# kimkyeonghun/MSA

Measured on AMD Instinct MI355X. Metric: train-step samples/sec, higher is better.
Workload: dtype bf16; 1 GPU; MMBertForPretraining train step, 3 passes S=50/550/550, 12-layer d=768 heads=12 vocab=30522, T=50 A=500 V=500, dropout on, AdamW; per_gpu_batch=16, global_batch=16, parallelism=dp1, scores_dtype=bf16, mlm_backward=labelled rows only (exact: unlabelled rows have zero CE gradient), deterministic=True

## Files before the change

### include/mmbert_hip.h

```cpp
#ifndef MMBERT_HIP_H
#define MMBERT_HIP_H
#include <stddef.h>
#include <stdint.h>

#ifdef __cplusplus
extern "C" {
#endif

typedef struct ihipStream_t* mmbert_stream_t;

#define MMBERT_EPI_BIAS 1
#define MMBERT_EPI_GELU 2
#define MMBERT_EPI_RESID 4
#define MMBERT_EPI_GELU_BWD 8
#define MMBERT_EPI_OUT_F32 16

int mmbert_gemm_nt(mmbert_stream_t stream, const void* A, int lda, const void* B, int ldb, void* C, int ldc,
                   int M, int N, int K, int epi, const float* bias, const void* R, int ldr, void* aux, int ldaux,
                   const void* U, int ldu, float alpha, const float* alpha_dev,
                   uint32_t drop_stream, uint32_t drop_thr16, float drop_scale, int* tile_queue);

int mmbert_gemm_nt_splitk(mmbert_stream_t stream, const void* A, int lda, const void* B, int ldb, void* C, int ldc,
                          int M, int N, int K, void* workspace, const void* R, int ldr);
size_t mmbert_gemm_nt_splitk_workspace(int M, int N, int K);

void mmbert_gemm_nt_force(int mode);
int mmbert_gemm_nt_describe(int M, int N, int K, int epi, int with_queue, int* out);
void mmbert_gemm_tn_force_splits(int splits);
void mmbert_gemm_tn_force_one_launch(int on);

size_t mmbert_gemm_tn_workspace(int M, int N, int K, int* splits_out);
int mmbert_gemm_tn(mmbert_stream_t stream, const void* A, int lda, const void* B, int ldb, float* W, int ldw,
                   int M, int N, int K, int accumulate, float alpha, const float* alpha_dev, void* slab, float* bias_out);
size_t mmbert_gemm_tn_grouped_workspace(int nprob, const int* N, const int* K, int M, int* splits_out);
int mmbert_gemm_tn_grouped(mmbert_stream_t stream, int nprob, const void* const* A, const int* lda, const void* const* B, const int* ldb,
                           float* const* W, float* const* bias, const int* N, const int* K, int M,
                           int accumulate, float alpha, const float* alpha_dev, void* slab);
int mmbert_gemm_tn_grouped_rows(mmbert_stream_t stream, int nprob, const void* const* A, const int* lda, const void* const* B, const int* ldb,
                                float* const* W, float* const* bias, const int* N, const int* K, const int* M,
                                int accumulate, const int* accumulate_each, float alpha, const float* alpha_dev, void* slab);

int mmbert_colsum(mmbert_stream_t stream, const void* X, int ldx, int M, int N, float* out, float alpha, const float* alpha_dev);

uint32_t mmbert_rng_stream(uint64_t seed, uint32_t site);
uint32_t mmbert_dropout_thr16(float p);
int mmbert_dropout_mask(mmbert_stream_t stream, uint8_t* out, size_t n, uint32_t rng_stream, uint32_t thr16);

int mmbert_mlm_mask(mmbert_stream_t stream, int64_t* ids, int64_t* labels, size_t n, uint32_t rng_stream, uint32_t select_thr16,
                    uint32_t replace_thr16, int64_t special0, int64_t special1, int64_t special2, int64_t mask_id);

int mmbert_ln_fwd(mmbert_stream_t stream, const void* x, int ldx, const int* in_rows, void* y, int ldy, const int* out_rows,
                  int M, int H, const float* gamma, const float* beta, float eps, float* mean, float* rstd,
                  uint32_t dstream, uint32_t dthr, float dscale, int drop_row0);
int mmbert_ln_bwd(mmbert_stream_t stream, const void* dy, int lddy, const int* dy_rows, const void* x, int ldx, const int* x_rows,
                  const float* mean, const float* rstd, const float* gamma, int M, int H,
                  void* dx, int lddx, const int* dx_rows, void* dx2, int lddx2, float* dgamma, float* dbeta, float* dbias2,
                  uint32_t post_stream, uint32_t post_thr, float post_scale,
                  uint32_t pre_stream, uint32_t pre_thr, float pre_scale,
                  float* partial_ws , const int* drop_rows,
                  int defer_reduce ,
                  int dy_row_limit );
size_t mmbert_ln_bwd_workspace(int M, int H);
int mmbert_ln_bwd_reduce(mmbert_stream_t stream, int items, const float* const* partial_ws, float* const* dgamma, float* const* dbeta,
                         float* const* dbias2, int M, int H);
int mmbert_ln_bwd_reduce_rows(mmbert_stream_t stream, int items, const float* const* partial_ws, float* const* dgamma, float* const* dbeta,
                              float* const* dbias2, const int* M, int H);

int mmbert_embed_gather(mmbert_stream_t stream, const int64_t* ids, const int64_t* tts, const float* word, const float* type,
                        const float* pos, int n, int T, int H, int V, void* out, int ldo);
int mmbert_embed_scatter(mmbert_stream_t stream, const int64_t* ids, const int64_t* tts, const void* d, int ldd, int n, int T, int H, int V,
                         float* gword, float* gtype, float* gpos, float* type_slab);

int mmbert_pair_proj_fwd(mmbert_stream_t stream, const void* feat, int feat_f64, int B, int P, int D, const float* W, const float* bias, int H,
                         void* out, int ldo, int T);
int mmbert_pair_proj_bwd(mmbert_stream_t stream, const void* feat, int feat_f64, int B, int P, int D, const void* J, const void* dJ, int ld, int T,
                         float* dW, float* db, int H, void* workspace );
size_t mmbert_pair_proj_bwd_workspace(int B, int P, int D, int H);

int mmbert_attn_tile_rows(int which);
int mmbert_attn_kv_len(mmbert_stream_t stream, const float* key_bias, const int* bias_start, const int* seq_len, int nseq, int* kv_len);
int mmbert_attn_fwd(mmbert_stream_t stream, const void* qkv, void* ctx, float* lse, const float* key_bias, const int* bias_start, int H, int heads,
                    const int* seq_start, const int* seq_len, const unsigned* elem_base, const int* tile_seq, const int* tile_r0, int ntiles,
                    uint32_t dstream, uint32_t dthr, float dscale, const int* kv_len, const int* tile_qshift, const int* tile_qend);
int mmbert_attn_fwd_first(mmbert_stream_t stream, const void* qkv, void* ctx, const float* key_bias, const int* bias_start, int H, int heads,
                          const int* seq_start, const int* seq_len, const int* q_row, int nseq, const int* kv_len);
int mmbert_attn_probs_first(mmbert_stream_t stream, const void* qkv, float* probs, int ld, const float* key_bias, const int* bias_start, int H, int heads,
                            const int* seq_start, const int* seq_len, const int* q_row, int nseq, const int* kv_len );
int mmbert_attn_bwd(mmbert_stream_t stream, const void* qkv, const void* ctx, const void* dctx, void* dqkv, const float* lse, float* delta,
                    const float* key_bias, const int* bias_start, int H, int heads, const int* seq_start, const int* seq_len, const unsigned* elem_base,
                    const int* qtile_seq, const int* qtile_r0, int nqtiles,
                    const int* tile_seq, const int* tile_r0, int ntiles,
                    uint32_t dstream, uint32_t dthr, float dscale, const int* kv_len,
                    const int* qtile_qshift, const int* qtile_qend, int split,
                    const int* q_limit);
int mmbert_attn_q_limit(mmbert_stream_t stream, const int* rows, int n, const int* seq_start, int nseq, int* q_limit);
int mmbert_attn_dropout_mask(mmbert_stream_t stream, uint8_t* out, int S, unsigned elem_base, int head, uint32_t rng_stream, uint32_t thr16);

int mmbert_ce_fwd(mmbert_stream_t stream, const void* logits, int ldv, int V, const int64_t* labels, int M,
                  const int* seg_bounds, int nseg, float* inv_count, float* loss_sum, float* row_lse,
                  int logits_f32 ,
                  float* row_loss );
int mmbert_ce_bwd(mmbert_stream_t stream, const void* logits, int ldv, int V, const int64_t* labels, int M,
                  const int* seg_bounds, int nseg, const float* inv_count, const float* gscale, const float* row_lse, void* dlogits, int ldd,
                  const int* rows , int nrows,
                  int logits_f32 );
int mmbert_vocab_topk(mmbert_stream_t stream, const void* logits, int ldv, int V, int M, int logits_f32, int k,
                      const int64_t* labels ,
                      int32_t* top_ids , float* top_logprob , float* row_lse ,
                      float* label_logprob , int32_t* label_rank );
int mmbert_split_rows(mmbert_stream_t stream, const int64_t* row_seq, const int64_t* row_pos, const int* start_a, const int* start_b,
                      const int* valid, int mode, int M, int rows_a, int64_t* perm, int64_t* inv, const int* rank,
                      int* perm32 , int* inv32);

int mmbert_split_layout(mmbert_stream_t stream, const int* seq_len, const int* valid, int nseq, int tile_rows, int xs, int nf_max, int nq_max,
                        int* out);

int mmbert_prologue(mmbert_stream_t stream, int nseg, const void* const* seg_ptr, const long long* seg_stride_b, const long long* seg_stride_p,
                    const int* seg_dtype, const int* seg_pass, const int* seg_offset, const int* seg_len,
                    int npass, const int* pass_len, int B, const int64_t* labels, int vocab,
                    float* key_bias, int* kv_len, int* valid, int* seq_cnt, int* idx, int* words, int* rank, float* key_bias_perm);

int mmbert_rows_to_block(mmbert_stream_t stream, const int64_t* ids, const void* rows, int rows_bf16, int ldr, int n, int H,
                         const int64_t* uni, int U, int V, float* block);

int mmbert_pack_i64(mmbert_stream_t stream, int nseg, const int64_t* const* src, const long long* dst_offset, const long long* count,
                    const long long* fill, int64_t* out);

int mmbert_active_rows(mmbert_stream_t stream, const int64_t* labels, int M, int V, int* idx, int* count);

int mmbert_heads_gate_fwd(mmbert_stream_t stream, const float* P, const float* Apre, const float* const* vw3, const float* const* vb3, int B, int H, float* g, float* C);
int mmbert_heads_loss_fwd(mmbert_stream_t stream, const float* P, const float* XP, const float* rel, const int64_t* ap, const float* lo, const float* sent,
                          int B, int H, float beta, int tanh_lo, float* out5, float* dXP, float* dPc, float* drel, float* dlo, float* nce_part,
                          const float* mlm, int nmlm, float alpha, float* loss_out , float* aux_out );
int mmbert_heads_scale(mmbert_stream_t stream, float* x, size_t n, const float* s);
int mmbert_heads_seed(mmbert_stream_t stream, const float* src, size_t n, const float* s, float* dst, float* zero, size_t nzero, float* dmlm, int nmlm, float coef);
int mmbert_heads_gate_bwd(mmbert_stream_t stream, const float* dC, const float* P, const float* Apre, const float* g, const float* const* vw3, const float* dPc,
                          int B, int H, float* dP, float* dApre, float* E, float* dg);
int mmbert_heads_tanh(mmbert_stream_t stream, float* x, size_t n);
int mmbert_heads_tanh_bwd(mmbert_stream_t stream, const float* dP, const float* P, float* dpre, size_t n);
int mmbert_heads_colsum(mmbert_stream_t stream, int nseg, const float* const* src, float* const* dst, const int* rows, const int* cols, const int* ld);

typedef struct {
    int B, H, tanh_lo, nmlm;
    float alpha, beta;
    const float* first; const void* y; const int64_t* first_rows; int ldy, ncls;
    const int64_t* ap; const int64_t* ap2; const float* sent; const float* mlm;
    const float *Wp, *bp, *Wal, *bal, *Wsr, *bsr, *Wat, *bat, *vw[3], *vb[3], *Wc1, *bc1, *Wc2, *bc2, *Wq[3], *bq[3];
    float *loss, *aux, *out5, *logits, *t_rel, *rel;
    float* ws;
    const float* dloss; float* dfirst; float* dmlm;
    float *gWp, *gbp, *gWal, *gbal, *gWat, *gbat, *gvw[3], *gvb[3], *gWc1, *gbc1, *gWc2, *gbc2, *gWq[3], *gbq[3];
    unsigned* sync;
    const int64_t* sent_cls; int64_t* pred;
} mmbert_heads_step;
int mmbert_heads_step_struct_size(void);
size_t mmbert_heads_step_workspace(int B, int H);
int mmbert_heads_step_fwd(mmbert_stream_t stream, const mmbert_heads_step* p);
int mmbert_heads_step_bwd(mmbert_stream_t stream, const mmbert_heads_step* p);
int mmbert_heads_step_fwd_levels(mmbert_stream_t stream, const mmbert_heads_step* p, int lo, int hi);
int mmbert_heads_step_bwd_levels(mmbert_stream_t stream, const mmbert_heads_step* p, int lo, int hi);
int mmbert_heads_predict(mmbert_stream_t stream, const mmbert_heads_step* p);
int mmbert_heads_step_outputs(int B, int H, size_t* pooled_offset, size_t* fused_offset);
int mmbert_heads_step_dmlm(mmbert_stream_t stream, const mmbert_heads_step* p);

typedef struct { const float* X; const float* W; int ldx, ldw, inner, row0, rows, w_inner_major; } mmbert_skinny_src;
typedef struct { float* Y; const float* bias; int ldy, M, N, nsrc, act, accumulate; mmbert_skinny_src src[4]; } mmbert_skinny_op;
typedef struct { const float* dY; const float* X; float* dW; float* db; int ldy, ldx, ldw, M, N, K; } mmbert_skinny_wgrad_op;
int mmbert_skinny_mm(mmbert_stream_t stream, int nops, const mmbert_skinny_op* ops);
size_t mmbert_skinny_mm_workspace(int nops, const mmbert_skinny_op* ops);
int mmbert_skinny_mm_ordered(mmbert_stream_t stream, int nops, const mmbert_skinny_op* ops, void* workspace);
int mmbert_skinny_wgrad(mmbert_stream_t stream, int nops, const mmbert_skinny_wgrad_op* ops);

typedef struct { uint32_t stream, thr16; float scale; } mmbert_drop;
typedef struct {
    const float* key_bias; const int* bias_start; const int* seq_start; const int* seq_len; const unsigned* elem_base;
    const int* ftile_seq; const int* ftile_r0; const int* ftile_qshift; const int* ftile_qend;
    const int* qtile_seq; const int* qtile_r0; const int* qtile_qshift; const int* qtile_qend;
    const int* tile_seq; const int* tile_r0;
    const int* kv_len;
    int nftiles, nqtiles, ntiles, split, heads, pad_;
} mmbert_attn_layout;
typedef struct {
    const void* x;
    const void* Wqkv; const void* Wo; const void* W1; const void* W2;
    const float* bqkv; const float* bo; const float* b1; const float* b2; const float* ln1_g; const float* ln1_b; const float* ln2_g; const float* ln2_b;
    void* qkv; void* actx; float* lse; void* z1; void* y1; float* m1; float* r1; void* u ; void* g; void* z2; void* y2; float* m2; float* r2;
    const int* y2_rows;
    int* tile_queue;
    mmbert_drop att, h1, h2;
    int rows, H, I, ldx, ldy2; float ln_eps;
} mmbert_layer_fwd_args;
typedef struct {
    const void* dy; const int* dy_rows;
    const void* z2; const float* m2; const float* r2; const float* ln2_g; float* g_ln2_g; float* g_ln2_b; float* ln2_ws;
    const void* z1; const float* m1; const float* r1; const float* ln1_g; float* g_ln1_g; float* g_ln1_b; float* ln1_ws;
    const void* u; const void* qkv; const void* actx; const float* lse;
    const void* W2T; const void* W1T; const void* WoT; const void* WqkvT;
    void* dz2; void* dz2d ; void* du; void* dy1; void* dz1; void* dz1d ; void* dctx; void* dqkv; float* delta; void* dx;
    int* tile_queue;
    mmbert_drop att, h1, h2;
    int rows, H, I, lddy;
} mmbert_layer_bwd_args;
int mmbert_layer_fwd(mmbert_stream_t stream, const mmbert_attn_layout* layout, const mmbert_layer_fwd_args* a);
int mmbert_layer_bwd(mmbert_stream_t stream, const mmbert_attn_layout* layout, const mmbert_layer_bwd_args* a);
int mmbert_layer_struct_sizes(int* out );

void mmbert_set_deterministic(int on);
int mmbert_get_deterministic(void);
int mmbert_id_runs_sum_rows(mmbert_stream_t stream, const void* src, int src_bf16, int lds, const int64_t* ids, int n,
                            int H, int V, const int64_t* uni, int U, float* dst, int ldd);

int mmbert_adamw(mmbert_stream_t stream, float* p, float* g, float* m, float* v, void* p_bf16, const uint8_t* flags, size_t n,
                 double lr, double beta1, double beta2, double eps, double wd, int step, double gscale, int mode, int zero_grad);

int mmbert_adamw_devscale(mmbert_stream_t stream, float* p, float* g, float* m, float* v, void* p_bf16, const uint8_t* flags, size_t n,
                          double lr, double beta1, double beta2, double eps, double wd, int step, const float* coef, int mode, int zero_grad);

#define MMBERT_ADAMW_MAX_GROUPS 255
#define MMBERT_ADAMW_MAX_SLOTS 64
int mmbert_adamw_grouped(mmbert_stream_t stream, float* p, float* g, float* m, float* v, void* p_bf16, const uint8_t* flags,
                         const uint8_t* group_of_block, size_t n, const double* hyper, int ngroups, int step, double gscale,
                         const float* coef, int mode, int zero_grad);

#define MMBERT_GRAD_NORM_WORKSPACE 8192
int mmbert_grad_norm(mmbert_stream_t stream, const float* g, size_t n, const int64_t* segs, int nseg, double norm_type, double max_norm,
                     double gscale, void* workspace, float* out);
int mmbert_grad_scale(mmbert_stream_t stream, float* g, size_t n, const int64_t* segs, int nseg, const float* coef);

int mmbert_gelu_bwd(mmbert_stream_t stream, const void* dy, const void* u, void* du, size_t n);

int mmbert_cast_f32_bf16(mmbert_stream_t stream, const float* x, void* y, size_t n);
int mmbert_cast_bf16_f32(mmbert_stream_t stream, const void* x, float* y, size_t n);
int mmbert_transpose_cast(mmbert_stream_t stream, const float* src, void* dst, const void* descs, int ndesc, int total_tiles);
int mmbert_compact_rows(mmbert_stream_t stream, const int* rows32, const int64_t* rows64, int n, const int64_t* extra, int nextra, const int64_t* map,
                        int64_t* out64, int* out32);
int mmbert_compact_rows_inv(mmbert_stream_t stream, const int* rows32, const int64_t* rows64, int n, const int64_t* extra, int nextra, const int64_t* map,
                            int64_t* out64, int* out32, int64_t* inv_stamp, unsigned stamp);
int mmbert_scatter_rows_zero(mmbert_stream_t stream, int nseg, const void* const* src, void* const* dst, const long long* src_pitch,
                             const long long* dst_pitch, const int* row_bytes, const int64_t* inv_stamp, unsigned stamp, int nlist, int nrows);
int mmbert_gather_rows(mmbert_stream_t stream, int nseg, const void* const* src, void* const* dst, const long long* src_pitch, const long long* dst_pitch,
                       const int* row_bytes, const int* idx, int nrows);
int mmbert_transpose_bf16(mmbert_stream_t stream, const void* src, void* dst, const void* descs, int ndesc, int total_tiles);

#ifdef __cplusplus
}
#endif
#endif
```

### msa_amd/_lib.py

```python
from __future__ import annotations

import ctypes as C
import os

HERE = os.path.dirname(os.path.abspath(__file__))
LIB_PATH = os.environ.get("MMBERT_LIB_PATH") or os.path.join(HERE, "libmmbert_hip.so")

P, I, F, D, U32, SZ, U64 = C.c_void_p, C.c_int, C.c_float, C.c_double, C.c_uint32, C.c_size_t, C.c_uint64

SIGNATURES = {
    "mmbert_gemm_nt": (I, [P, P, I, P, I, P, I, I, I, I, I, P, P, I, P, I, P, I, F, P, U32, U32, F, P]),
    "mmbert_gemm_nt_force": (None, [I]),
    "mmbert_gemm_nt_describe": (I, [I, I, I, I, I, P]),
    "mmbert_gemm_nt_splitk": (I, [P, P, I, P, I, P, I, I, I, I, P, P, I]),
    "mmbert_gemm_nt_splitk_workspace": (SZ, [I, I, I]),
    "mmbert_gemm_tn_force_splits": (None, [I]),
    "mmbert_gemm_tn_force_one_launch": (None, [I]),
    "mmbert_gemm_tn_workspace": (SZ, [I, I, I, P]),
    "mmbert_gemm_tn": (I, [P, P, I, P, I, P, I, I, I, I, I, F, P, P, P]),
    "mmbert_gemm_tn_grouped_workspace": (SZ, [I, P, P, I, P]),
    "mmbert_gemm_tn_grouped": (I, [P, I, P, P, P, P, P, P, P, P, I, I, F, P, P]),
    "mmbert_gemm_tn_grouped_rows": (I, [P, I, P, P, P, P, P, P, P, P, P, I, P, F, P, P]),
    "mmbert_colsum": (I, [P, P, I, I, I, P, F, P]),
    "mmbert_rng_stream": (U32, [U64, U32]),
    "mmbert_dropout_thr16": (U32, [F]),
    "mmbert_dropout_mask": (I, [P, P, SZ, U32, U32]),
    "mmbert_mlm_mask": (I, [P, P, P, SZ, U32, U32, U32, C.c_int64, C.c_int64, C.c_int64, C.c_int64]),
    "mmbert_ln_fwd": (I, [P, P, I, P, P, I, P, I, I, P, P, F, P, P, U32, U32, F, I]),
    "mmbert_ln_bwd": (I, [P, P, I, P, P, I, P, P, P, P, I, I, P, I, P, P, I, P, P, P, U32, U32, F, U32, U32, F, P, P, I, I]),
    "mmbert_ln_bwd_reduce": (I, [P, I, P, P, P, P, I, I]),
    "mmbert_ln_bwd_reduce_rows": (I, [P, I, P, P, P, P, P, I]),
    "mmbert_ln_bwd_workspace": (SZ, [I, I]),
    "mmbert_embed_gather": (I, [P, P, P, P, P, P, I, I, I, I, P, I]),
    "mmbert_embed_scatter": (I, [P, P, P, P, I, I, I, I, I, P, P, P, P]),
    "mmbert_pair_proj_fwd": (I, [P, P, I, I, I, I, P, P, I, P, I, I]),
    "mmbert_pair_proj_bwd": (I, [P, P, I, I, I, I, P, P, I, I, P, P, I, P]),
    "mmbert_pair_proj_bwd_workspace": (SZ, [I, I, I, I]),
    "mmbert_attn_tile_rows": (I, [I]),
    "mmbert_attn_kv_len": (I, [P, P, P, P, I, P]),
    "mmbert_attn_fwd": (I, [P, P, P, P, P, P, I, I, P, P, P, P, P, I, U32, U32, F, P, P, P]),
    "mmbert_attn_fwd_first": (I, [P, P, P, P, P, I, I, P, P, P, I, P]),
    "mmbert_attn_probs_first": (I, [P, P, P, I, P, P, I, I, P, P, P, I, P]),
    "mmbert_attn_bwd": (I, [P, P, P, P, P, P, P, P, P, I, I, P, P, P, P, P, I, P, P, I, U32, U32, F, P, P, P, I, P]),
    "mmbert_attn_q_limit": (I, [P, P, I, P, I, P]),
    "mmbert_attn_dropout_mask": (I, [P, P, I, C.c_uint, I, U32, U32]),
    "mmbert_ce_fwd": (I, [P, P, I, I, P, I, P, I, P, P, P, I, P]),
    "mmbert_ce_bwd": (I, [P, P, I, I, P, I, P, I, P, P, P, P, I, P, I, I]),
    "mmbert_vocab_topk": (I, [P, P, I, I, I, I, I, P, P, P, P, P, P]),
    "mmbert_active_rows": (I, [P, P, I, I, P, P]),
    "mmbert_prologue": (I, [P, I, P, P, P, P, P, P, P, I, P, I, P, I, P, P, P, P, P, P, P, P]),
    "mmbert_split_rows": (I, [P, P, P, P, P, P, I, I, I, P, P, P, P, P]),
    "mmbert_heads_gate_fwd": (I, [P, P, P, P, P, I, I, P, P]),
    "mmbert_heads_loss_fwd": (I, [P, P, P, P, P, P, P, I, I, F, I, P, P, P, P, P, P, P, I, F, P, P]),
    "mmbert_heads_scale": (I, [P, P, SZ, P]),
    "mmbert_heads_seed": (I, [P, P, SZ, P, P, P, SZ, P, I, F]),
    "mmbert_heads_gate_bwd": (I, [P, P, P, P, P, P, P, I, I, P, P, P, P]),
    "mmbert_heads_tanh": (I, [P, P, SZ]),
    "mmbert_heads_tanh_bwd": (I, [P, P, P, P, SZ]),
    "mmbert_heads_colsum": (I, [P, I, P, P, P, P, P]),
    "mmbert_skinny_mm": (I, [P, I, P]),
    "mmbert_skinny_mm_workspace": (SZ, [I, P]),
    "mmbert_skinny_mm_ordered": (I, [P, I, P, P]),
    "mmbert_heads_step_struct_size": (I, []),
    "mmbert_heads_step_workspace": (SZ, [I, I]),
    "mmbert_heads_step_fwd": (I, [P, P]),
    "mmbert_heads_step_bwd": (I, [P, P]),
    "mmbert_heads_step_fwd_levels": (I, [P, P, I, I]),
    "mmbert_heads_step_bwd_levels": (I, [P, P, I, I]),
    "mmbert_heads_step_dmlm": (I, [P, P]),
    "mmbert_heads_predict": (I, [P, P]),
    "mmbert_heads_step_outputs": (I, [I, I, P, P]),
    "mmbert_layer_fwd": (I, [P, P, P]),
    "mmbert_layer_bwd": (I, [P, P, P]),
    "mmbert_layer_struct_sizes": (I, [P]),
    "mmbert_set_deterministic": (None, [I]),
    "mmbert_get_deterministic": (I, []),
    "mmbert_id_runs_sum_rows": (I, [P, P, I, I, P, I, I, I, P, I, P, I]),
    "mmbert_skinny_wgrad": (I, [P, I, P]),
    "mmbert_adamw": (I, [P, P, P, P, P, P, P, SZ, D, D, D, D, D, I, D, I, I]),
    "mmbert_adamw_devscale": (I, [P, P, P, P, P, P, P, SZ, D, D, D, D, D, I, P, I, I]),
    "mmbert_adamw_grouped": (I, [P, P, P, P, P, P, P, P, SZ, P, I, I, D, P, I, I]),
    "mmbert_grad_norm": (I, [P, P, SZ, P, I, D, D, D, P, P]),
    "mmbert_grad_scale": (I, [P, P, SZ, P, I, P]),
    "mmbert_gelu_bwd": (I, [P, P, P, P, SZ]),
    "mmbert_cast_f32_bf16": (I, [P, P, P, SZ]),
    "mmbert_cast_bf16_f32": (I, [P, P, P, SZ]),
    "mmbert_transpose_cast": (I, [P, P, P, P, I, I]),
    "mmbert_transpose_bf16": (I, [P, P, P, P, I, I]),
    "mmbert_gather_rows": (I, [P, I, P, P, P, P, P, P, I]),
    "mmbert_compact_rows": (I, [P, P, P, I, P, I, P, P, P]),
    "mmbert_compact_rows_inv": (I, [P, P, P, I, P, I, P, P, P, P, C.c_uint]),
    "mmbert_scatter_rows_zero": (I, [P, I, P, P, P, P, P, P, C.c_uint, I, I]),
    "mmbert_pack_i64": (I, [P, I, P, P, P, P, P]),
    "mmbert_rows_to_block": (I, [P, P, P, I, I, I, I, P, I, I, P]),
    "mmbert_split_layout": (I, [P, P, P, I, I, I, I, I, P]),
}

_lib = None


def load() -> C.CDLL:
    global _lib
    if _lib is not None:
        return _lib
    if not os.path.exists(LIB_PATH):
        raise RuntimeError(
            f"{LIB_PATH} not found: the MI355X kernels are not built and there is no CPU fallback. "
            "Run `python -m msa_amd.build` (needs hipcc) first.")
    lib = C.CDLL(LIB_PATH)
    for name, (res, args) in SIGNATURES.items():
        fn = getattr(lib, name)
        fn.restype = res
        fn.argtypes = args
    _lib = lib
    return lib


def check(code: int, what: str) -> None:
    if code != 0:
        raise RuntimeError(f"{what} failed with code {code} "
                           f"({'invalid argument' if code < 0 else 'hipError_t'})")
```

### msa_amd/csrc/attention.hip

```cpp
#include <cstdlib>
#include "common.h"
#include <type_traits>

#define LOG2E 1.4426950408889634f
#define LN2 0.6931471805599453f

struct AttnArgs {
    const bf16_t* qkv; int ld_qkv;
    bf16_t* ctx;
    const bf16_t* dctx;
    bf16_t* dqkv;
    float* lse;
    float* delta;
    const float* key_bias;
    const int* bias_start;
    const int* kv_len;
    const int* seq_start; const int* seq_len; const unsigned* elem_base;
    const int* tile_seq; const int* tile_r0;
    const int* tile_qshift; const int* tile_qend; int split;
    const int* q_limit;
    int H, heads;
    float scale;
    uint32_t dstream, dthr; float dscale;
    int head_fast;
// ... 799 lines not shown

    for (int k0 = grp; k0 < Skv; k0 += 256) {
        bf16x8 kf[8];
        float b[8];
#pragma unroll
        for (int u = 0; u < 8; ++u) {
            const int k = min(k0 + 32 * u, Skv - 1);
            kf[u] = *(const bf16x8*)(kbase + (size_t)k * a.ld_qkv);
            b[u] = bbase[k];
        }
        float s[8];
#pragma unroll
        for (int u = 0; u < 8; ++u) {
            float d = 0.f;
#pragma unroll
            for (int j = 0; j < 8; ++j) d = __builtin_fmaf(q[j], bf2f(kf[u][j]), d);
            d += __shfl_xor(d, 1, 64); d += __shfl_xor(d, 2, 64); d += __shfl_xor(d, 4, 64);
            const int k = k0 + 32 * u;
            s[u] = k < Skv ? d + b[u] : -INFINITY;
            if (c == 0 && k < Skv && k < a.ld) sc[k] = s[u];
        }
        const float mnew = fmaxf(fmaxf(fmaxf(fmaxf(s[0], s[1]), fmaxf(s[2], s[3])), fmaxf(fmaxf(s[4], s[5]), fmaxf(s[6], s[7]))), st.m);
        st.l *= __builtin_amdgcn_exp2f((st.m - mnew) * LOG2E);
        st.m = mnew;
#pragma unroll
        for (int u = 0; u < 8; ++u) st.l += __builtin_amdgcn_exp2f((s[u] - mnew) * LOG2E);
    }
#pragma unroll
    for (int off = 8; off < 64; off <<= 1) {
        ApState o2;
        o2.m = __shfl_xor(st.m, off, 64); o2.l = __shfl_xor(st.l, off, 64);
        ap_merge(st, o2);
    }
    if (lane == 0) { part[2 * wave] = st.m; part[2 * wave + 1] = st.l; }
    __syncthreads();
    ApState tot;
    tot.m = part[0]; tot.l = part[1];
#pragma unroll
    for (int w = 1; w < 4; ++w) {
        ApState o2;
        o2.m = part[2 * w]; o2.l = part[2 * w + 1];
        ap_merge(tot, o2);
    }
    const float inv = 1.0f / tot.l;
    const int nk = min(Skv, a.ld);
    for (int k = threadIdx.x; k < a.ld; k += 256)
        prow[k] = k < nk ? __builtin_amdgcn_exp2f((sc[k] - tot.m) * LOG2E) * inv : 0.f;
}

__global__ void attn_mask_kernel(uint8_t* out, int S, unsigned elem_base, int head, uint32_t stream, uint32_t thr) {
    const int Spad = (S + 3) & ~3;
    for (int e = blockIdx.x * blockDim.x + threadIdx.x; e < S * S; e += gridDim.x * blockDim.x) {
        const int i = e / S, j = e % S;
        out[e] = mmb_keep(stream, (uint64_t)elem_base + (uint64_t)(head * S + i) * Spad + j, thr) ? 1 : 0;
    }
}

__global__ void attn_kv_len_kernel(const float* __restrict__ key_bias, const int* __restrict__ bias_start, const int* __restrict__ seq_len, int nseq, int* __restrict__ out) {
    const int s = blockIdx.x;
    if (s >= nseq) return;
    const int S = seq_len[s];
    const float* b = key_bias + bias_start[s];
    int last = -1;
    for (int k = threadIdx.x; k < S; k += 64)
        if (b[k] > -10000.0f) last = k;
#pragma unroll
    for (int o = 32; o > 0; o >>= 1) last = max(last, __shfl_xor(last, o, 64));
    if (threadIdx.x == 0) out[s] = last < 0 ? S : last + 1;
}

__global__ void attn_q_limit_kernel(const int* __restrict__ rows, int n, const int* __restrict__ seq_start, int nseq, int* __restrict__ out) {
    const int i = blockIdx.x * blockDim.x + threadIdx.x;
    if (i >= n) return;
    const int r = rows[i];
    int lo = 0, hi = nseq - 1;
    while (lo < hi) {
        const int mid = (lo + hi + 1) >> 1;
        if (seq_start[mid] <= r) lo = mid; else hi = mid - 1;
    }
    atomicMax(out + lo, r - seq_start[lo] + 1);
}
__global__ __launch_bounds__(256) void attn_q_limit_wg_kernel(const int* __restrict__ rows, int n, const int* __restrict__ seq_start, int nseq,
                                                              int* __restrict__ out) {
    __shared__ int lim[1024], st[1024];
    for (int s = threadIdx.x; s < nseq; s += 256) { lim[s] = 0; st[s] = seq_start[s]; }
    __syncthreads();
    for (int i = threadIdx.x; i < n; i += 256) {
        const int r = rows[i];
        int lo = 0, hi = nseq - 1;
        while (lo < hi) {
            const int mid = (lo + hi + 1) >> 1;
            if (st[mid] <= r) lo = mid; else hi = mid - 1;
        }
        atomicMax(&lim[lo], r - st[lo] + 1);
    }
    __syncthreads();
    for (int s = threadIdx.x; s < nseq; s += 256) out[s] = lim[s];
}

extern "C" {

static int fill_args(AttnArgs& a, const void* qkv, int H, int heads, const float* key_bias, const int* bias_start, const int* seq_start, const int* seq_len,
                     const unsigned* elem_base, const int* tile_seq, const int* tile_r0, float* lse,
                     uint32_t dstream, uint32_t dthr, float dscale, const int* kv_len) {
    if (heads <= 0 || H != heads * 64) return -1;
    a.qkv = (const bf16_t*)qkv; a.ld_qkv = 3 * H; a.H = H; a.heads = heads; a.key_bias = key_bias; a.bias_start = bias_start;
    a.seq_start = seq_start; a.seq_len = seq_len; a.elem_base = elem_base; a.tile_seq = tile_seq; a.tile_r0 = tile_r0;
    a.lse = lse; a.scale = 0.125f; a.dstream = dstream; a.dthr = dthr; a.dscale = dscale;
    a.ctx = nullptr; a.dctx = nullptr; a.dqkv = nullptr; a.delta = nullptr; a.kv_len = kv_len;
    a.tile_qshift = nullptr; a.tile_qend = nullptr; a.split = 0; a.q_limit = nullptr;
    a.head_fast = 1;
    return 0;
}

int mmbert_attn_fwd(hipStream_t stream, const void* qkv, void* ctx, float* lse, const float* key_bias, const int* bias_start, int H, int heads,
                    const int* seq_start, const int* seq_len, const unsigned* elem_base, const int* tile_seq, const int* tile_r0, int ntiles,
                    uint32_t dstream, uint32_t dthr, float dscale, const int* kv_len, const int* tile_qshift, const int* tile_qend) {
    if (ntiles <= 0) return 0;
    if ((tile_qshift == nullptr) != (tile_qend == nullptr)) return -1;
    AttnArgs a;
    if (fill_args(a, qkv, H, heads, key_bias, bias_start, seq_start, seq_len, elem_base, tile_seq, tile_r0, lse, dstream, dthr, dscale, kv_len)) return -1;
    a.ctx = (bf16_t*)ctx; a.tile_qshift = tile_qshift; a.tile_qend = tile_qend;
    if (ntiles > 65535) a.head_fast = 0;
    constexpr int extra_lds = 0;
    if (dthr) hipLaunchKernelGGL(attn_fwd_kernel<true>, a.head_fast ? dim3(heads, ntiles) : dim3(ntiles, heads), dim3(256), extra_lds, stream, a);
    else hipLaunchKernelGGL(attn_fwd_kernel<false>, a.head_fast ? dim3(heads, ntiles) : dim3(ntiles, heads), dim3(256), extra_lds, stream, a);
    MMB_CHECK_LAUNCH();
    return 0;
}

int mmbert_attn_fwd_first(hipStream_t stream, const void* qkv, void* ctx, const float* key_bias, const int* bias_start, int H, int heads,
                          const int* seq_start, const int* seq_len, const int* q_row, int nseq, const int* kv_len) {
    if (nseq <= 0) return 0;
    if (heads <= 0 || H != heads * 64 || nseq > 65535 || !qkv || !ctx || !key_bias || !bias_start || !seq_start || !seq_len || !q_row) return -1;
    AttnFirstArgs a;
    a.qkv = (const bf16_t*)qkv; a.ld_qkv = 3 * H; a.ctx = (bf16_t*)ctx; a.key_bias = key_bias; a.bias_start = bias_start; a.kv_len = kv_len;
    a.seq_start = seq_start; a.seq_len = seq_len; a.q_row = q_row; a.H = H; a.scale = 0.125f;
    hipLaunchKernelGGL(attn_fwd_first_kernel, dim3(heads, nseq), dim3(256), 0, stream, a);
    MMB_CHECK_LAUNCH();
    return 0;
}

int mmbert_attn_probs_first(hipStream_t stream, const void* qkv, float* probs, int ld, const float* key_bias, const int* bias_start, int H, int heads,
                            const int* seq_start, const int* seq_len, const int* q_row, int nseq, const int* kv_len) {
    if (nseq <= 0) return 0;
    if (heads <= 0 || H != heads * 64 || nseq > 65535 || ld < 1 || !qkv || !probs || !key_bias || !bias_start || !seq_start || !seq_len || !q_row) return -1;
    if (APF_LDS_BYTES(ld) > APF_LDS_MAX) return -1;
    AttnProbsArgs a;
    a.qkv = (const bf16_t*)qkv; a.ld_qkv = 3 * H; a.probs = probs; a.ld = ld; a.key_bias = key_bias; a.bias_start = bias_start; a.kv_len = kv_len;
    a.seq_start = seq_start; a.seq_len = seq_len; a.q_row = q_row; a.H = H; a.heads = heads; a.scale = 0.125f;
    hipLaunchKernelGGL(attn_probs_first_kernel, dim3(heads, nseq), dim3(256), APF_LDS_BYTES(ld), stream, a);
    MMB_CHECK_LAUNCH();
    return 0;
}

int mmbert_attn_bwd(hipStream_t stream, const void* qkv, const void* ctx, const void* dctx, void* dqkv, const float* lse, float* delta,
                    const float* key_bias, const int* bias_start, int H, int heads, const int* seq_start, const int* seq_len, const unsigned* elem_base,
                    const int* qtile_seq, const int* qtile_r0, int nqtiles, const int* tile_seq, const int* tile_r0, int ntiles,
                    uint32_t dstream, uint32_t dthr, float dscale, const int* kv_len, const int* qtile_qshift, const int* qtile_qend, int split,
                    const int* q_limit) {
    if (ntiles <= 0 || nqtiles <= 0) return 0;
    if ((qtile_qshift == nullptr) != (qtile_qend == nullptr) || (split && !kv_len)) return -1;
    AttnArgs a;
    if (fill_args(a, qkv, H, heads, key_bias, bias_start, seq_start, seq_len, elem_base, tile_seq, tile_r0, (float*)lse, dstream, dthr, dscale, kv_len)) return -1;
    a.ctx = (bf16_t*)ctx; a.dctx = (const bf16_t*)dctx; a.dqkv = (bf16_t*)dqkv; a.delta = delta; a.q_limit = q_limit;
    {
        AttnArgs q = a;
        q.tile_seq = qtile_seq; q.tile_r0 = qtile_r0; q.tile_qshift = qtile_qshift; q.tile_qend = qtile_qend;
        if (nqtiles > 65535) q.head_fast = 0;
        if (dthr) hipLaunchKernelGGL(attn_bwd_dq_kernel<true>, q.head_fast ? dim3(heads, nqtiles) : dim3(nqtiles, heads), dim3(256), 0, stream, q);
        else hipLaunchKernelGGL(attn_bwd_dq_kernel<false>, q.head_fast ? dim3(heads, nqtiles) : dim3(nqtiles, heads), dim3(256), 0, stream, q);
        MMB_CHECK_LAUNCH();
    }
    a.split = split;
    if (ntiles > 65535) a.head_fast = 0;
    if (dthr) hipLaunchKernelGGL(attn_bwd_dkv_kernel<true>, a.head_fast ? dim3(heads, ntiles) : dim3(ntiles, heads), dim3(256), 0, stream, a);
    else hipLaunchKernelGGL(attn_bwd_dkv_kernel<false>, a.head_fast ? dim3(heads, ntiles) : dim3(ntiles, heads), dim3(256), 0, stream, a);
    MMB_CHECK_LAUNCH();
    return 0;
}
// ... 38 lines not shown
```

### msa_amd/csrc/common.h

```cpp
#pragma once
#include <hip/hip_runtime.h>
#include <stdint.h>

#if defined(MMB_EXP_NOMFMA) || defined(MMB_EXP_ALOADS) || defined(MMB_EXP_NOBLOADS) || defined(MMB_EXP_EXEC0) || defined(MMB_EXP_WAVEA) || \
    defined(MMB_EXP_NOFRAGS) || defined(MMB_AB_FREE_HASH)
#error "MMB_EXP_* / MMB_AB_* ablation switches are not part of the product sources (see git tag r3-gemm-ablations)"
#endif

typedef __bf16 bf16_t;
typedef __attribute__((ext_vector_type(8))) __bf16 bf16x8;
typedef __attribute__((ext_vector_type(4))) __bf16 bf16x4;
typedef __attribute__((ext_vector_type(2))) __bf16 bf16x2;
typedef __attribute__((ext_vector_type(4))) short s16x4;
typedef __attribute__((ext_vector_type(4))) float f32x4;
typedef __attribute__((ext_vector_type(16))) float f32x16;

#define MMB_CHECK_LAUNCH() do { hipError_t e_ = hipGetLastError(); if (e_ != hipSuccess) return (int)e_; } while (0)

#include <atomic>
static inline int mmb_allow_lds(const void* fn, int bytes, std::atomic<unsigned long long>& done) {
    int dev = 0;
    if (hipGetDevice(&dev) != hipSuccess) return (int)hipErrorInvalidDevice;
    const unsigned long long bit = 1ull << (dev & 63);
    if (done.load(std::memory_order_acquire) & bit) return 0;
// ... 77 lines not shown

__device__ __forceinline__ float mmb_clamp_abs12(float x) { return __builtin_amdgcn_fmed3f(fabsf(x), 0.0f, 12.0f); }
__device__ __forceinline__ float mmb_relu(float x) { float r; asm("v_max_f32 %0, 0, %1" : "=v"(r) : "v"(x)); return r; }
__device__ __forceinline__ float gelu_erf(float x) {
    const float a = mmb_clamp_abs12(x);
    float q = 0.000488118665642307f;
    q = fmaf(q, a, -0.007198809871008205f);
    q = fmaf(q, a, 0.05214680078704519f);
    q = fmaf(q, a, 0.4595957249475095f);
    q = fmaf(q, a, 1.1510005681479196f);
    const float t = __builtin_amdgcn_exp2f(fmaf(-a, q, -1.0f));
    return fmaf(-a, t, mmb_relu(x));
}
__device__ __forceinline__ float gelu_erf_grad(float x) {
    const float a = mmb_clamp_abs12(x);
    float w = -0.00016849001371319273f;
    w = fmaf(w, a, 0.002318365387269111f);
    w = fmaf(w, a, -0.013920757956130972f);
    w = fmaf(w, a, 0.04993439894451681f);
    w = fmaf(w, a, -0.1258212077485634f);
    w = fmaf(w, a, 0.2479567789223165f);
    w = fmaf(w, a, -0.7976617799265314f);
    w = fmaf(w, a, 0.49999600551278855f);
    const float g = __builtin_amdgcn_exp2f(-0.72134752044448170f * a * a) * w;
    return x > 0.0f ? 1.0f - g : g;
}

__device__ __forceinline__ mmb_f2 gelu_erf2(mmb_f2 x) {
    const mmb_f2 a = {mmb_clamp_abs12(x.x), mmb_clamp_abs12(x.y)};
    mmb_f2 q = (mmb_f2){0.000488118665642307f, 0.000488118665642307f};
    q = q * a + (mmb_f2){-0.007198809871008205f, -0.007198809871008205f};
    q = q * a + (mmb_f2){0.05214680078704519f, 0.05214680078704519f};
    q = q * a + (mmb_f2){0.4595957249475095f, 0.4595957249475095f};
    q = q * a + (mmb_f2){1.1510005681479196f, 1.1510005681479196f};
    const mmb_f2 e = -a * q + (mmb_f2){-1.0f, -1.0f};
    const mmb_f2 t = {__builtin_amdgcn_exp2f(e.x), __builtin_amdgcn_exp2f(e.y)};
    const mmb_f2 r = {mmb_relu(x.x), mmb_relu(x.y)};
    return -a * t + r;
}
__device__ __forceinline__ mmb_f2 gelu_erf_grad2(mmb_f2 x) {
    const mmb_f2 a = {mmb_clamp_abs12(x.x), mmb_clamp_abs12(x.y)};
    mmb_f2 w = (mmb_f2){-0.00016849001371319273f, -0.00016849001371319273f};
    w = w * a + (mmb_f2){0.002318365387269111f, 0.002318365387269111f};
    w = w * a + (mmb_f2){-0.013920757956130972f, -0.013920757956130972f};
    w = w * a + (mmb_f2){0.04993439894451681f, 0.04993439894451681f};
    w = w * a + (mmb_f2){-0.1258212077485634f, -0.1258212077485634f};
    w = w * a + (mmb_f2){0.2479567789223165f, 0.2479567789223165f};
    w = w * a + (mmb_f2){-0.7976617799265314f, -0.7976617799265314f};
    w = w * a + (mmb_f2){0.49999600551278855f, 0.49999600551278855f};
    const mmb_f2 e = ((mmb_f2){-0.72134752044448170f, -0.72134752044448170f} * a) * a;
    const mmb_f2 g = (mmb_f2){__builtin_amdgcn_exp2f(e.x), __builtin_amdgcn_exp2f(e.y)} * w;
    const mmb_f2 og = (mmb_f2){1.0f, 1.0f} - g;
    return (mmb_f2){x.x > 0.0f ? og.x : g.x, x.y > 0.0f ? og.y : g.y};
}

__device__ __forceinline__ void gelu_erf4(mmb_f2& x0, mmb_f2& x1) {
    const mmb_f2 a0 = {mmb_clamp_abs12(x0.x), mmb_clamp_abs12(x0.y)}, a1 = {mmb_clamp_abs12(x1.x), mmb_clamp_abs12(x1.y)};
    mmb_f2 q0 = (mmb_f2){0.000488118665642307f, 0.000488118665642307f}, q1 = q0;
    q0 = q0 * a0 + (mmb_f2){-0.007198809871008205f, -0.007198809871008205f}; q1 = q1 * a1 + (mmb_f2){-0.007198809871008205f, -0.007198809871008205f};
    q0 = q0 * a0 + (mmb_f2){0.05214680078704519f, 0.05214680078704519f};    q1 = q1 * a1 + (mmb_f2){0.05214680078704519f, 0.05214680078704519f};
    q0 = q0 * a0 + (mmb_f2){0.4595957249475095f, 0.4595957249475095f};      q1 = q1 * a1 + (mmb_f2){0.4595957249475095f, 0.4595957249475095f};
    q0 = q0 * a0 + (mmb_f2){1.1510005681479196f, 1.1510005681479196f};      q1 = q1 * a1 + (mmb_f2){1.1510005681479196f, 1.1510005681479196f};
    const mmb_f2 e0 = -a0 * q0 + (mmb_f2){-1.0f, -1.0f}, e1 = -a1 * q1 + (mmb_f2){-1.0f, -1.0f};
    const mmb_f2 r0 = {mmb_relu(x0.x), mmb_relu(x0.y)}, r1 = {mmb_relu(x1.x), mmb_relu(x1.y)};
    const mmb_f2 t0 = {__builtin_amdgcn_exp2f(e0.x), __builtin_amdgcn_exp2f(e0.y)}, t1 = {__builtin_amdgcn_exp2f(e1.x), __builtin_amdgcn_exp2f(e1.y)};
    x0 = -a0 * t0 + r0;
    x1 = -a1 * t1 + r1;
}
__device__ __forceinline__ void gelu_erf_grad4(mmb_f2 x0, mmb_f2 x1, mmb_f2& d0, mmb_f2& d1) {
    const mmb_f2 a0 = {mmb_clamp_abs12(x0.x), mmb_clamp_abs12(x0.y)}, a1 = {mmb_clamp_abs12(x1.x), mmb_clamp_abs12(x1.y)};
    mmb_f2 w0 = (mmb_f2){-0.00016849001371319273f, -0.00016849001371319273f}, w1 = w0;
#define MMB_W_STEP(C) w0 = w0 * a0 + (mmb_f2){C, C}; w1 = w1 * a1 + (mmb_f2){C, C};
    MMB_W_STEP(0.002318365387269111f) MMB_W_STEP(-0.013920757956130972f) MMB_W_STEP(0.04993439894451681f) MMB_W_STEP(-0.1258212077485634f)
    MMB_W_STEP(0.2479567789223165f) MMB_W_STEP(-0.7976617799265314f) MMB_W_STEP(0.49999600551278855f)
#undef MMB_W_STEP
    const mmb_f2 k = {-0.72134752044448170f, -0.72134752044448170f};
    const mmb_f2 e0 = (k * a0) * a0, e1 = (k * a1) * a1;
    const mmb_f2 t0 = {__builtin_amdgcn_exp2f(e0.x), __builtin_amdgcn_exp2f(e0.y)}, t1 = {__builtin_amdgcn_exp2f(e1.x), __builtin_amdgcn_exp2f(e1.y)};
    const mmb_f2 g0 = t0 * w0, g1 = t1 * w1;
    const mmb_f2 o0 = (mmb_f2){1.0f, 1.0f} - g0, o1 = (mmb_f2){1.0f, 1.0f} - g1;
    d0 = (mmb_f2){x0.x > 0.0f ? o0.x : g0.x, x0.y > 0.0f ? o0.y : g0.y};
    d1 = (mmb_f2){x1.x > 0.0f ? o1.x : g1.x, x1.y > 0.0f ? o1.y : g1.y};
}
```

### msa_amd/csrc/rowwise.hip

```cpp
#include "common.h"
#include <cstring>

std::atomic<int> g_mmb_deterministic{0};

__global__ void split_rows_kernel(const int64_t* __restrict__ row_seq, const int64_t* __restrict__ row_pos, const int* __restrict__ start_a,
                                  const int* __restrict__ start_b, const int* __restrict__ valid, int mode, int M, int rows_a,
                                  int64_t* __restrict__ perm, int64_t* __restrict__ inv, const int* __restrict__ rank,
                                  int* __restrict__ perm32, int* __restrict__ inv32) {
    const int i = blockIdx.x * blockDim.x + threadIdx.x;
    if (i >= M) return;
    const int s = (int)row_seq[i], p = rank ? rank[i] : (int)row_pos[i], v = valid[s];
    int n = rows_a;
    bool own = false;
    if (p < v) { n = start_a[s] + p; own = true; }
    else if (mode == 0) { n = start_b[s] + p - v; own = true; }
    else if (mode == 1) { n = start_b[s]; own = p == v; }
    inv[i] = n;
    if (inv32) inv32[i] = n;
    if (own) { perm[n] = i; if (perm32) perm32[n] = i; }
}

#define SL_MAXSEQ 1024
__global__ __launch_bounds__(1024) void split_layout_kernel(const int* __restrict__ lens, const int* __restrict__ valid, int nseq, int rows, int xs,
                                                            int nf_max, int nq_max, int* __restrict__ out) {
// ... 811 lines not shown
            for (int i = 0; i < 4; ++i) av[i] = bf2f(st[u].j[i]) > 0.f ? bf2f(st[u].d[i]) : 0.f;
            float fv[PAIR_NT];
#pragma unroll
            for (int j = 0; j < PAIR_NT; ++j) fv[j] = st[u].f[j];
            load(st[u], r + 16 + 4 * u + g);
#pragma unroll
            for (int j = 0; j < PAIR_NT; ++j) {
                if (j >= njt) continue;
#pragma unroll
                for (int i = 0; i < 4; ++i) acc[j][i] = __builtin_amdgcn_mfma_f32_16x16x4f32(av[i], fv[j], acc[j][i], 0, 0, 0);
            }
        }
    }
    if (wave) {
#pragma unroll
        for (int j = 0; j < PAIR_NT; ++j)
#pragma unroll
            for (int i = 0; i < 4; ++i)
#pragma unroll
                for (int q = 0; q < 4; ++q) red[wave - 1][(j * 4 + i) * 4 + q][lane] = acc[j][i][q];
    }
    __syncthreads();
    if (wave == 0) {
        const int W1 = a.D + 1;
        float* out = a.slab + (size_t)s * a.H * W1;
#pragma unroll
        for (int j = 0; j < PAIR_NT; ++j) {
            const int k = (jt0 + j) * 16 + c;
#pragma unroll
            for (int i = 0; i < 4; ++i)
#pragma unroll
                for (int q = 0; q < 4; ++q) {
                    const int e = (j * 4 + i) * 4 + q;
                    const float v = ((acc[j][i][q] + red[0][e][lane]) + red[1][e][lane]) + red[2][e][lane];
                    const int h = hb + 4 * (4 * g + q) + i;
                    if (j < njt && k < W1 && h < a.H) out[(size_t)h * W1 + k] = v;
                }
        }
    }
#endif
}

__global__ void pair_wgrad_reduce_kernel(const float* __restrict__ slab, int S, int H, int D, float* __restrict__ dW, float* __restrict__ db) {
    const int i = blockIdx.x * blockDim.x + threadIdx.x;
    const int W1 = D + 1;
    if (i >= H * W1) return;
    float t = 0.f;
    int s_ = 0;
    for (; s_ + 8 <= S; s_ += 8) {
        float v[8];
#pragma unroll
        for (int u = 0; u < 8; ++u) v[u] = slab[(size_t)(s_ + u) * H * W1 + i];
#pragma unroll
        for (int u = 0; u < 8; ++u) t += v[u];
    }
    for (; s_ < S; ++s_) t += slab[(size_t)s_ * H * W1 + i];
    const int h = i / W1, k = i - h * W1;
    if (k < D) dW[(size_t)h * D + k] += t; else db[h] += t;
}

__global__ __launch_bounds__(1024) void active_rows_kernel(const int64_t* __restrict__ labels, int M, int V, int* __restrict__ idx, int* __restrict__ count) {
    __shared__ int wsum[16];
    __shared__ int base;
    const int tid = threadIdx.x, lane = tid & 63, w = tid >> 6;
    if (tid == 0) base = 0;
    __syncthreads();
    for (int i0 = 0; i0 < M; i0 += 1024) {
        const int i = i0 + tid;
        const bool act = i < M && labels[i] >= 0 && labels[i] < V;
        const unsigned long long bal = __ballot(act);
        const int before = __popcll(bal & ((1ull << lane) - 1ull));
        if (lane == 0) wsum[w] = __popcll(bal);
        __syncthreads();
        int off = base;
        for (int q = 0; q < w; ++q) off += wsum[q];
        if (act) idx[off + before] = i;
        __syncthreads();
        if (tid == 0) { int t = 0; for (int q = 0; q < 16; ++q) t += wsum[q]; base += t; }
        __syncthreads();
    }
    if (tid == 0) *count = base;
}

__global__ void ce_count_kernel(const int64_t* __restrict__ labels, int M, int V, const int* __restrict__ seg_bounds, int nseg,
                                float* __restrict__ inv_count, float* __restrict__ loss_sum) {
    __shared__ int cnt[4];
    if (threadIdx.x < 4) cnt[threadIdx.x] = 0;
    __syncthreads();
    const int b1 = nseg > 1 ? seg_bounds[1] : 0x7fffffff, b2 = nseg > 2 ? seg_bounds[2] : 0x7fffffff, b3 = nseg > 3 ? seg_bounds[3] : 0x7fffffff;
    int c[4] = {0, 0, 0, 0};
    for (int i0 = threadIdx.x; i0 < M; i0 += (int)blockDim.x * 8) {
        int64_t lab[8];
#pragma unroll
        for (int u = 0; u < 8; ++u) lab[u] = labels[min(i0 + u * (int)blockDim.x, M - 1)];
#pragma unroll
        for (int u = 0; u < 8; ++u) {
            const int i = i0 + u * (int)blockDim.x;
            const int ok = (i < M && lab[u] >= 0 && lab[u] < V) ? 1 : 0;
            const int sg = (i >= b1 ? 1 : 0) + (i >= b2 ? 1 : 0) + (i >= b3 ? 1 : 0);
#pragma unroll
            for (int q = 0; q < 4; ++q) c[q] += (sg == q) ? ok : 0;
        }
    }
#pragma unroll
    for (int q = 0; q < 4; ++q) if (c[q]) atomicAdd(&cnt[q], c[q]);
    __syncthreads();
    if (threadIdx.x < nseg) {
        inv_count[threadIdx.x] = 1.0f / (float)max(cnt[threadIdx.x], 1);
        loss_sum[threadIdx.x] = 0.f;
    }
}

__global__ __launch_bounds__(1024) void ce_loss_sum_ordered_kernel(const float* __restrict__ row_loss, int M, const int* __restrict__ seg_bounds, int nseg,
                                                                   float* __restrict__ loss_sum) {
    __shared__ float red[4][1024];
    const int b1 = nseg > 1 ? seg_bounds[1] : 0x7fffffff, b2 = nseg > 2 ? seg_bounds[2] : 0x7fffffff, b3 = nseg > 3 ? seg_bounds[3] : 0x7fffffff;
    float c[4] = {0.f, 0.f, 0.f, 0.f};
    for (int i0 = threadIdx.x; i0 < M; i0 += 1024 * 8) {
        float v[8];
#pragma unroll
        for (int u = 0; u < 8; ++u) v[u] = row_loss[min(i0 + u * 1024, M - 1)];
#pragma unroll
        for (int u = 0; u < 8; ++u) {
            const int i = i0 + u * 1024;
            const int sg = (i >= b1 ? 1 : 0) + (i >= b2 ? 1 : 0) + (i >= b3 ? 1 : 0);
            const float x = i < M ? v[u] : 0.f;
#pragma unroll
            for (int q = 0; q < 4; ++q) c[q] += (sg == q) ? x : 0.f;
        }
    }
#pragma unroll
    for (int q = 0; q < 4; ++q) red[q][threadIdx.x] = c[q];
    __syncthreads();
    for (int w = 512; w > 0; w >>= 1) {
        if ((int)threadIdx.x < w) {
#pragma unroll
            for (int q = 0; q < 4; ++q) red[q][threadIdx.x] += red[q][threadIdx.x + w];
        }
        __syncthreads();
    }
    if ((int)threadIdx.x < nseg) loss_sum[threadIdx.x] = red[threadIdx.x][0];
}

#define RUNS_MAXN 8192
__global__ __launch_bounds__(1024) void id_runs_sum_rows_kernel(const void* __restrict__ src, int src_bf16, int lds, const int64_t* __restrict__ ids,
                                                                int n, int H, int V, const int64_t* __restrict__ uni, int U,
                                                                float* __restrict__ dst, int ldd) {
    __shared__ int list[RUNS_MAXN];
    __shared__ float red[1024 * 4];
    __shared__ int s_count, s_earlier;
    const int i0 = blockIdx.x, tid = threadIdx.x, nthr = blockDim.x;
    const long long key = ids[i0];
    if (key <= 0 || key >= V) return;
    if (tid == 0) { s_count = 0; s_earlier = 0; }
    __syncthreads();
    int earlier = 0;
    for (int j = tid; j < i0; j += nthr) earlier |= (ids[j] == key) ? 1 : 0;
    if (earlier) s_earlier = 1;
    __syncthreads();
    if (s_earlier) return;
    long long dr = key;
    if (uni) {
        int lo = 0, hi = U - 1;
        while (lo < hi) { const int mid = (lo + hi) >> 1; if (uni[mid] < key) lo = mid + 1; else hi = mid; }
        if (U <= 0 || uni[lo] != key) return;
        dr = lo;
    }
    if (tid < 64) {
        int count = 0;
        for (int base = i0; base < n; base += 64) {
            const int j = base + tid;
            const bool hit = j < n && ids[j] == key;
            const unsigned long long m = __ballot(hit);
            if (hit) list[count + __popcll(m & ((1ull << tid) - 1ull))] = j;
            count += __popcll(m);
        }
        if (tid == 0) s_count = count;
    }
    __syncthreads();
    const int cnt = s_count;
    const int CT = H >> 2, G = nthr / CT;
    const int g = tid / CT, c = tid - g * CT;
    float a[4] = {0.f, 0.f, 0.f, 0.f};
    if (g < G) {
#pragma unroll 4
        for (int k = g; k < cnt; k += G) {
            const size_t r = (size_t)list[k];
            if (src_bf16) {
                const bf16x4 x = *(const bf16x4*)((const bf16_t*)src + r * lds + 4 * c);
#pragma unroll
                for (int q = 0; q < 4; ++q) a[q] += bf2f(x[q]);
            } else {
                const float4 x = *(const float4*)((const float*)src + r * lds + 4 * c);
                a[0] += x.x; a[1] += x.y; a[2] += x.z; a[3] += x.w;
            }
        }
#pragma unroll
        for (int q = 0; q < 4; ++q) red[(g * CT + c) * 4 + q] = a[q];
    }
    __syncthreads();
    if (g == 0) {
        float4* d = (float4*)(dst + (size_t)dr * ldd + 4 * c);
        float4 o = *d;
        float t[4] = {0.f, 0.f, 0.f, 0.f};
        for (int gg = 0; gg < G; ++gg)
#pragma unroll
            for (int q = 0; q < 4; ++q) t[q] += red[(gg * CT + c) * 4 + q];
        o.x += t[0]; o.y += t[1]; o.z += t[2]; o.w += t[3];
        *d = o;
    }
}

__global__ void embed_type_fold_kernel(const float* __restrict__ slab, int T, int H, float* __restrict__ gtype) {
    const int e = blockIdx.x * blockDim.x + threadIdx.x;
    if (e >= 2 * H) return;
    float t = 0.f;
    for (int p = 0; p < T; ++p) t += slab[(size_t)p * 2 * H + e];
    gtype[e] += t;
}

#define CE_MAXC 16
template <int MODE, bool F32>
__global__ __launch_bounds__(256) void ce_row_kernel(const void* __restrict__ logits_, int ldv, int V, const int64_t* __restrict__ labels,
                                                     const int* __restrict__ seg_bounds, int nseg, const float* __restrict__ inv_count,
                                                     float* __restrict__ loss_sum, float* __restrict__ row_lse, const float* __restrict__ gscale,
                                                     bf16_t* __restrict__ dlogits, int ldd, const int* __restrict__ rows, float* __restrict__ row_loss) {
    __shared__ float red[4];
    __shared__ float lab_logit;
    const int i = rows ? rows[blockIdx.x] : blockIdx.x;
    const int64_t lab = labels[i];
    const int tid = threadIdx.x, lane = tid & 63, w = tid >> 6;
    const int nchunk = ldv >> 3;
    if (lab < 0 || lab >= V) {
        if (MODE == 0) { if (tid == 0) { row_lse[i] = 0.f; if (row_loss) row_loss[i] = 0.f; } }
        else {
            bf16_t* drow = dlogits + (size_t)(rows ? blockIdx.x : i) * ldd;
            const bf16x8 z = {0, 0, 0, 0, 0, 0, 0, 0};
            for (int c = tid; c < nchunk; c += 256) *(bf16x8*)(drow + c * 8) = z;
        }
        return;
    }
    int s = 0;
    while (s + 1 < nseg && i >= seg_bounds[s + 1]) ++s;
    bf16x8 v[CE_MAXC];
    if constexpr (F32) {
        const float* row = (const float*)logits_ + (size_t)i * ldv;
#pragma unroll
        for (int c = 0; c < CE_MAXC; ++c) {
            const int ch = c * 256 + tid;
            if (ch < nchunk) {
                const float4 lo = *(const float4*)(row + ch * 8), hi = *(const float4*)(row + ch * 8 + 4);
                v[c] = (bf16x8){f2bf(lo.x), f2bf(lo.y), f2bf(lo.z), f2bf(lo.w), f2bf(hi.x), f2bf(hi.y), f2bf(hi.z), f2bf(hi.w)};
            }
        }
    } else {
        const bf16_t* row = (const bf16_t*)logits_ + (size_t)i * ldv;
#pragma unroll
        for (int c = 0; c < CE_MAXC; ++c) {
            const int ch = c * 256 + tid;
            if (ch < nchunk) v[c] = *(const bf16x8*)(row + ch * 8);
        }
    }
    if (MODE == 0) {
        float mx = -INFINITY;
#pragma unroll
        for (int c = 0; c < CE_MAXC; ++c) {
            const int ch = c * 256 + tid;
            if (ch < nchunk) {
#pragma unroll
                for (int r = 0; r < 8; ++r) if (ch * 8 + r < V) mx = fmaxf(mx, bf2f(v[c][r]));
            }
        }
        mx = wave_max(mx);
        if (lane == 0) red[w] = mx;
        __syncthreads();
        mx = fmaxf(fmaxf(red[0], red[1]), fmaxf(red[2], red[3]));
        __syncthreads();
        float se = 0.f;
#pragma unroll
        for (int c = 0; c < CE_MAXC; ++c) {
            const int ch = c * 256 + tid;
            if (ch < nchunk) {
#pragma unroll
                for (int r = 0; r < 8; ++r) if (ch * 8 + r < V) se += __expf(bf2f(v[c][r]) - mx);
                if ((int)(lab >> 3) == ch) lab_logit = bf2f(v[c][lab & 7]);
            }
        }
        se = wave_sum(se);
        if (lane == 0) red[w] = se;
        __syncthreads();
        if (tid == 0) {
            const float lse = mx + __logf(red[0] + red[1] + red[2] + red[3]);
            row_lse[i] = lse;
            if (row_loss) row_loss[i] = (lse - lab_logit) * inv_count[s];
            else atomicAdd(loss_sum + s, (lse - lab_logit) * inv_count[s]);
        }
    } else {
        const float lse = row_lse[i];
        const float scale = inv_count[s] * gscale[s];
        bf16_t* drow = dlogits + (size_t)(rows ? blockIdx.x : i) * ldd;
#pragma unroll
        for (int c = 0; c < CE_MAXC; ++c) {
            const int ch = c * 256 + tid;
            if (ch < nchunk) {
                bf16x8 o;
#pragma unroll
                for (int r = 0; r < 8; ++r) {
                    const int col = ch * 8 + r;
                    float pr = col < V ? __expf(bf2f(v[c][r]) - lse) : 0.f;
                    if (col == (int)lab) pr -= 1.0f;
                    o[r] = f2bf(pr * scale);
                }
                *(bf16x8*)(drow + ch * 8) = o;
            }
        }
    }
}

typedef uint32_t vt_u32x4 __attribute__((ext_vector_type(4)));

__device__ __forceinline__ uint32_t vt_key(uint32_t h) {
    const uint32_t neg = (uint32_t)((int32_t)h >> 31);
    return h ^ ((neg & 0x7FFF0000u) | 0x80000000u);
}
__device__ __forceinline__ float vt_value(uint32_t word) {
    const uint32_t kk = word & 0xFFFF0000u;
    return __builtin_bit_cast(float, (kk & 0x80000000u) ? (kk ^ 0x80000000u) : (kk ^ 0xFFFF0000u));
}
__device__ __forceinline__ uint32_t vt_wave_max(uint32_t v) {
#pragma unroll
    for (int o = 32; o > 0; o >>= 1) v = max(v, (uint32_t)__shfl_xor((int)v, o, 64));
    return v;
}
template <bool COUNT>
__device__ __forceinline__ uint32_t vt_scan(const uint32_t (&e)[CE_MAXC * 8], uint32_t prev, uint32_t lab_word, int& above) {
    uint32_t best = 0u;
#pragma unroll
    for (int n = 0; n < CE_MAXC * 8; ++n) {
        best = max(best, e[n] - prev);
        if (COUNT) above += e[n] > lab_word ? 1 : 0;
    }
    const uint32_t word = best + prev;
    return word < prev ? word : 0u;
}

template <bool F32>
__global__ __launch_bounds__(256) void vocab_topk_kernel(const void* __restrict__ logits_, int ldv, int V, int k, const int64_t* __restrict__ labels,
                                                         int32_t* __restrict__ top_ids, float* __restrict__ top_logprob, float* __restrict__ row_lse,
                                                         float* __restrict__ label_logprob, int32_t* __restrict__ label_rank) {
    __shared__ float red[4];
    __shared__ float lab_logit;
    __shared__ int red_above[4];
    __shared__ uint32_t red_word[2][4];
    const int i = blockIdx.x;
    const int tid = threadIdx.x, lane = tid & 63, w = tid >> 6;
    const int nchunk = (V + 7) >> 3;
    const int64_t lab = labels ? labels[i] : -1;
    const bool has_lab = lab >= 0 && lab < V;
    const int lab_chunk = has_lab ? (int)(lab >> 3) : -1;
    bf16x8 v[CE_MAXC];
    if constexpr (F32) {
        const float* row = (const float*)logits_ + (size_t)i * ldv;
#pragma unroll
        for (int c = 0; c < CE_MAXC; ++c) {
            const int ch = c * 256 + tid;
            if (ch < nchunk) {
                const float4 lo = *(const float4*)(row + ch * 8), hi = *(const float4*)(row + ch * 8 + 4);
                v[c] = (bf16x8){f2bf(lo.x), f2bf(lo.y), f2bf(lo.z), f2bf(lo.w), f2bf(hi.x), f2bf(hi.y), f2bf(hi.z), f2bf(hi.w)};
            }
        }
    } else {
        const bf16_t* row = (const bf16_t*)logits_ + (size_t)i * ldv;
#pragma unroll
        for (int c = 0; c < CE_MAXC; ++c) {
            const int ch = c * 256 + tid;
            if (ch < nchunk) v[c] = *(const bf16x8*)(row + ch * 8);
        }
    }
    float mx = -INFINITY;
#pragma unroll
    for (int c = 0; c < CE_MAXC; ++c) {
        const int ch = c * 256 + tid;
        if (ch < nchunk) {
#pragma unroll
            for (int r = 0; r < 8; ++r) if (ch * 8 + r < V) mx = fmaxf(mx, bf2f(v[c][r]));
        }
    }
    mx = wave_max(mx);
    if (lane == 0) red[w] = mx;
    __syncthreads();
    mx = fmaxf(fmaxf(red[0], red[1]), fmaxf(red[2], red[3]));
    __syncthreads();
    float se = 0.f;
    {
#pragma clang fp reassociate(off)
#pragma unroll
        for (int c = 0; c < CE_MAXC; ++c) {
            const int ch = c * 256 + tid;
// ... 793 lines not shown
    if (mmb_deterministic() && (gword != nullptr || type_slab == nullptr)) return -4;
    constexpr int slices = 1;
    hipLaunchKernelGGL(embed_scatter_kernel, dim3(T < n ? T : n, slices), dim3(256), 0, stream, ids, tts, (const bf16_t*)d, ldd, n, T, H, V, gword, gtype, gpos, type_slab);
    MMB_CHECK_LAUNCH();
    if (type_slab) {
        hipLaunchKernelGGL(embed_type_fold_kernel, dim3((2 * H + 255) / 256), dim3(256), 0, stream, type_slab, T < n ? T : n, H, gtype);
        MMB_CHECK_LAUNCH();
    }
    return 0;
}

int mmbert_pair_proj_fwd(hipStream_t stream, const void* feat, int feat_f64, int B, int P, int D, const float* W, const float* bias, int H,
                         void* out, int ldo, int T) {
    const int n = B * P;
    if (n <= 0) return 0;
    if (D < 1 || H < 1) return -1;
    const int KC = D < 128 ? (D + 3) & ~3 : 128;
    const int pitch = KC + ((18 - (KC & 15)) & 15);
    const int ops_lds = 192 * pitch * (int)sizeof(float), out_lds = 64 * 136 * (int)sizeof(bf16_t);
    const int lds = ops_lds > out_lds ? ops_lds : out_lds;
    return feat_f64 ? pair_proj_fwd_launch(stream, (const double*)feat, n, P, D, W, bias, H, out, ldo, T, KC, pitch, lds)
                    : pair_proj_fwd_launch(stream, (const float*)feat, n, P, D, W, bias, H, out, ldo, T, KC, pitch, lds);
}

static void pair_bwd_split(int n, int D, int H, int* rows_per_wg, int* S) {
    const int htiles = (H + 63) / 64, zt = ((D + 1 + 15) / 16 + PAIR_NT - 1) / PAIR_NT;
    int want = (mmb_device_cus() + htiles * zt - 1) / (htiles * zt);
    if (want < 1) want = 1;
    int rp = ((n + want - 1) / want + 63) / 64 * 64;
    if (rp < 64) rp = 64;
    *rows_per_wg = rp;
    *S = (n + rp - 1) / rp;
}
size_t mmbert_pair_proj_bwd_workspace(int B, int P, int D, int H) {
    if (B <= 0 || P <= 0 || D < 1 || H < 1) return 0;
    int rp, S;
    pair_bwd_split(B * P, D, H, &rp, &S);
    return (size_t)S * H * (D + 1) * sizeof(float);
}

int mmbert_pair_proj_bwd(hipStream_t stream, const void* feat, int feat_f64, int B, int P, int D, const void* J, const void* dJ, int ld, int T,
                         float* dW, float* db, int H, void* workspace) {
    const int n = B * P;
    if (n <= 0) return 0;
    if (!workspace || (H & 7) || (ld & 7) || D < 1) return -1;
    PairBwdArgs a = {};
    a.feat = feat; a.J = (const bf16_t*)J; a.dJ = (const bf16_t*)dJ; a.slab = (float*)workspace;
    a.n = n; a.P = P; a.D = D; a.T = T; a.H = H; a.ld = ld;
    int S;
    pair_bwd_split(n, D, H, &a.rows_per_wg, &S);
    a.ntiles = (D + 1 + 15) / 16;
    const dim3 grid((H + 63) / 64, S, (a.ntiles + PAIR_NT - 1) / PAIR_NT);
    if (feat_f64) hipLaunchKernelGGL(pair_wgrad_kernel<double>, grid, dim3(256), 0, stream, a);
    else hipLaunchKernelGGL(pair_wgrad_kernel<float>, grid, dim3(256), 0, stream, a);
    MMB_CHECK_LAUNCH();
    hipLaunchKernelGGL(pair_wgrad_reduce_kernel, dim3((H * (D + 1) + 255) / 256), dim3(256), 0, stream, (const float*)workspace, S, H, D, dW, db);
    MMB_CHECK_LAUNCH();
    return 0;
}

int mmbert_ce_fwd(hipStream_t stream, const void* logits, int ldv, int V, const int64_t* labels, int M,
                  const int* seg_bounds, int nseg, float* inv_count, float* loss_sum, float* row_lse, int logits_f32, float* row_loss) {
    if (M <= 0) return 0;
    if (nseg < 1 || nseg > 4 || (ldv & 7) || ldv > CE_MAXC * 256 * 8 || V > ldv) return -1;
    const bool det = mmb_deterministic();
    if (det && !row_loss) return -4;
    if (!det) row_loss = nullptr;
    hipLaunchKernelGGL(ce_count_kernel, dim3(1), dim3(1024), 0, stream, labels, M, V, seg_bounds, nseg, inv_count, loss_sum);
    MMB_CHECK_LAUNCH();
    if (logits_f32)
        hipLaunchKernelGGL((ce_row_kernel<0, true>), dim3(M), dim3(256), 0, stream, logits, ldv, V, labels, seg_bounds, nseg, inv_count, loss_sum,
                           row_lse, (const float*)nullptr, (bf16_t*)nullptr, 0, (const int*)nullptr, row_loss);
    else
        hipLaunchKernelGGL((ce_row_kernel<0, false>), dim3(M), dim3(256), 0, stream, logits, ldv, V, labels, seg_bounds, nseg, inv_count, loss_sum,
                           row_lse, (const float*)nullptr, (bf16_t*)nullptr, 0, (const int*)nullptr, row_loss);
    MMB_CHECK_LAUNCH();
    if (det) {
        hipLaunchKernelGGL(ce_loss_sum_ordered_kernel, dim3(1), dim3(1024), 0, stream, (const float*)row_loss, M, seg_bounds, nseg, loss_sum);
        MMB_CHECK_LAUNCH();
    }
    return 0;
}

int mmbert_vocab_topk(hipStream_t stream, const void* logits, int ldv, int V, int M, int logits_f32, int k, const int64_t* labels,
                      int32_t* top_ids, float* top_logprob, float* row_lse, float* label_logprob, int32_t* label_rank) {
    if (M < 0 || V < 1 || V > CE_MAXC * 256 * 8 || k < 1 || k > 8 || k > V || (ldv & 7) || ldv < V) return -1;
    if (M == 0) return 0;
    if (!logits || !top_ids || !top_logprob || !row_lse) return -1;
    if (labels ? (!label_logprob || !label_rank) : (label_logprob || label_rank)) return -1;
    if (logits_f32)
        hipLaunchKernelGGL(vocab_topk_kernel<true>, dim3(M), dim3(256), 0, stream, logits, ldv, V, k, labels, top_ids, top_logprob, row_lse,
                           label_logprob, label_rank);
    else
        hipLaunchKernelGGL(vocab_topk_kernel<false>, dim3(M), dim3(256), 0, stream, logits, ldv, V, k, labels, top_ids, top_logprob, row_lse,
                           label_logprob, label_rank);
    MMB_CHECK_LAUNCH();
    return 0;
}

void mmbert_set_deterministic(int on) { g_mmb_deterministic.store(on != 0); }
int mmbert_get_deterministic(void) { return g_mmb_deterministic.load(); }

int mmbert_id_runs_sum_rows(hipStream_t stream, const void* src, int src_bf16, int lds, const int64_t* ids, int n,
                            int H, int V, const int64_t* uni, int U, float* dst, int ldd) {
    if (n <= 0) return 0;
    if ((H & 3) || H > 4096 || n > RUNS_MAXN || (lds & 3) || (ldd & 3) || !src || !ids || !dst) return -1;
    const int CT = H >> 2;
    int G = 1024 / CT; if (G > 8) G = 8; if (G < 1) G = 1;
    int threads = G * CT; if (threads < 64) threads = 64;
    hipLaunchKernelGGL(id_runs_sum_rows_kernel, dim3(n), dim3(threads), 0, stream, src, src_bf16, lds, ids, n, H, V, uni, U, dst, ldd);
    MMB_CHECK_LAUNCH();
    return 0;
}

int mmbert_ce_bwd(hipStream_t stream, const void* logits, int ldv, int V, const int64_t* labels, int M,
                  const int* seg_bounds, int nseg, const float* inv_count, const float* gscale, const float* row_lse, void* dlogits, int ldd,
                  const int* rows, int nrows, int logits_f32) {
    if (M <= 0 || (rows && nrows <= 0)) return 0;
    if (nseg < 1 || nseg > 4 || (ldv & 7) || (ldd & 7) || ldv > CE_MAXC * 256 * 8 || V > ldv) return -1;
    if (logits_f32)
        hipLaunchKernelGGL((ce_row_kernel<1, true>), dim3(rows ? nrows : M), dim3(256), 0, stream, logits, ldv, V, labels, seg_bounds, nseg, inv_count,
                           (float*)nullptr, (float*)row_lse, gscale, (bf16_t*)dlogits, ldd, rows, (float*)nullptr);
    else
        hipLaunchKernelGGL((ce_row_kernel<1, false>), dim3(rows ? nrows : M), dim3(256), 0, stream, logits, ldv, V, labels, seg_bounds, nseg, inv_count,
                           (float*)nullptr, (float*)row_lse, gscale, (bf16_t*)dlogits, ldd, rows, (float*)nullptr);
    MMB_CHECK_LAUNCH();
    return 0;
}

int mmbert_split_rows(hipStream_t stream, const int64_t* row_seq, const int64_t* row_pos, const int* start_a, const int* start_b, const int* valid,
                      int mode, int M, int rows_a, int64_t* perm, int64_t* inv, const int* rank, int* perm32, int* inv32) {
    if (M <= 0) return 0;
    if (mode < 0 || mode > 2) return -1;
    hipLaunchKernelGGL(split_rows_kernel, dim3((M + 255) / 256), dim3(256), 0, stream, row_seq, row_pos, start_a, start_b, valid, mode, M, rows_a, perm, inv, rank,
                       perm32, inv32);
    MMB_CHECK_LAUNCH();
    return 0;
}

int mmbert_split_layout(hipStream_t stream, const int* seq_len, const int* valid, int nseq, int tile_rows, int xs, int nf_max, int nq_max, int* out) {
    if (nseq <= 0) return 0;
    if (nseq > SL_MAXSEQ || tile_rows <= 0 || xs <= 0 || !out) return -1;
    hipLaunchKernelGGL(split_layout_kernel, dim3(1), dim3(1024), 0, stream, seq_len, valid, nseq, tile_rows, xs, nf_max, nq_max, out);
    MMB_CHECK_LAUNCH();
    return 0;
}

int mmbert_prologue(hipStream_t stream, int nseg, const void* const* seg_ptr, const long long* seg_stride_b, const long long* seg_stride_p,
                    const int* seg_dtype, const int* seg_pass, const int* seg_offset, const int* seg_len,
                    int npass, const int* pass_len, int B, const int64_t* labels, int vocab,
                    float* key_bias, int* kv_len, int* valid, int* seq_cnt, int* idx, int* words, int* rank, float* key_bias_perm) {
    if (npass <= 0 || B <= 0) return 0;
    if (nseg < 0 || nseg > PRO_MAXSEG || npass > PRO_MAXPASS || ((rank == nullptr) != (key_bias_perm == nullptr))) return -1;
    PrologueArgs a = {};
    for (int q = 0; q < nseg; ++q) {
        if (seg_dtype[q] < 0 || seg_dtype[q] > 6 || seg_pass[q] < 0 || seg_pass[q] >= npass) return -1;
        a.seg[q].ptr = (const char*)seg_ptr[q]; a.seg[q].sb = seg_stride_b[q]; a.seg[q].sp = seg_stride_p[q];
        a.seg[q].dtype = seg_dtype[q]; a.seg[q].pass = seg_pass[q]; a.seg[q].offset = seg_offset[q]; a.seg[q].len = seg_len[q];
    }
    int row = 0, slot = 0;
    for (int p = 0; p < npass; ++p) {
        a.pass_len[p] = pass_len[p]; a.pass_row0[p] = row; a.pass_bias0[p] = slot;
        row += B * pass_len[p]; slot += B * ((pass_len[p] + 127) & ~127);
    }
    a.nseg = nseg; a.npass = npass; a.B = B; a.vocab = vocab; a.labels = labels;
    a.key_bias = key_bias; a.kv_len = kv_len; a.valid = valid; a.seq_cnt = seq_cnt; a.idx = idx; a.words = words;
// ... 144 lines not shown
    return 0;
}

__global__ void compact_rows_kernel(const int* __restrict__ a32, const int64_t* __restrict__ a64, int n, const int64_t* __restrict__ extra, int nextra,
                                    const int64_t* __restrict__ map, int64_t* __restrict__ out64, int* __restrict__ out32,
                                    long long* __restrict__ inv_stamp, long long stamp_hi) {
    const int i = blockIdx.x * blockDim.x + threadIdx.x;
    if (i >= n + nextra) return;
    int64_t r = i < n ? (a32 ? (int64_t)a32[i] : a64[i]) : extra[i - n];
    if (map) r = map[r];
    out64[i] = r;
    out32[i] = (int)r;
    if (inv_stamp) inv_stamp[r] = stamp_hi | (long long)i;
}
static int compact_rows_launch(hipStream_t stream, const int* rows32, const int64_t* rows64, int n, const int64_t* extra, int nextra, const int64_t* map,
                               int64_t* out64, int* out32, long long* inv_stamp, unsigned stamp) {
    if (n < 0 || nextra < 0 || (n > 0 && !rows32 && !rows64) || (nextra > 0 && !extra)) return -1;
    if (n + nextra == 0) return 0;
    hipLaunchKernelGGL(compact_rows_kernel, dim3((n + nextra + 255) / 256), dim3(256), 0, stream, rows32, rows64, n, extra, nextra, map, out64, out32,
                       inv_stamp, (long long)((unsigned long long)stamp << 32));
    MMB_CHECK_LAUNCH();
    return 0;
}
int mmbert_compact_rows(hipStream_t stream, const int* rows32, const int64_t* rows64, int n, const int64_t* extra, int nextra, const int64_t* map,
                        int64_t* out64, int* out32) {
    return compact_rows_launch(stream, rows32, rows64, n, extra, nextra, map, out64, out32, nullptr, 0u);
}
int mmbert_compact_rows_inv(hipStream_t stream, const int* rows32, const int64_t* rows64, int n, const int64_t* extra, int nextra, const int64_t* map,
                            int64_t* out64, int* out32, int64_t* inv_stamp, unsigned stamp) {
    if (!inv_stamp || stamp == 0u) return -1;
    return compact_rows_launch(stream, rows32, rows64, n, extra, nextra, map, out64, out32, (long long*)inv_stamp, stamp);
}

struct ScatterSeg { const char* src; char* dst; long long src_pitch, dst_pitch; int row_bytes; };
struct ScatterArgs { ScatterSeg s[4]; };
__global__ __launch_bounds__(256) void scatter_rows_zero_kernel(const ScatterArgs a, const long long* __restrict__ inv_stamp, long long stamp_hi, int nlist) {
    const ScatterSeg s = a.s[blockIdx.y];
    const int r = blockIdx.x;
    const long long v = inv_stamp[r];
    const int i = (int)(v & 0xffffffffll);
    const bool hit = (v & ~0xffffffffll) == stamp_hi && i < nlist;
    char* dst = s.dst + (long long)r * s.dst_pitch;
    const char* src = s.src + (long long)(hit ? i : 0) * s.src_pitch;
    for (int b = threadIdx.x * 16; b < s.row_bytes; b += 256 * 16) {
        uint4 x = {0u, 0u, 0u, 0u};
        if (hit) x = *(const uint4*)(src + b);
        *(uint4*)(dst + b) = x;
    }
}
int mmbert_scatter_rows_zero(hipStream_t stream, int nseg, const void* const* src, void* const* dst, const long long* src_pitch, const long long* dst_pitch,
                             const int* row_bytes, const int64_t* inv_stamp, unsigned stamp, int nlist, int nrows) {
    if (nseg <= 0 || nrows <= 0) return 0;
    if (nseg > 4 || !inv_stamp || stamp == 0u || nlist < 0) return -1;
    ScatterArgs a = {};
    for (int k = 0; k < nseg; ++k) {
        if (!dst[k] || (nlist > 0 && !src[k]) || row_bytes[k] <= 0 || ((row_bytes[k] | src_pitch[k] | dst_pitch[k]) & 15) ||
            (((uintptr_t)src[k] | (uintptr_t)dst[k]) & 15)) return -1;
        a.s[k].src = (const char*)src[k]; a.s[k].dst = (char*)dst[k]; a.s[k].src_pitch = src_pitch[k]; a.s[k].dst_pitch = dst_pitch[k];
        a.s[k].row_bytes = row_bytes[k];
    }
    hipLaunchKernelGGL(scatter_rows_zero_kernel, dim3(nrows, nseg), dim3(256), 0, stream, a, (const long long*)inv_stamp,
                       (long long)((unsigned long long)stamp << 32), nlist);
    MMB_CHECK_LAUNCH();
    return 0;
}

int mmbert_gather_rows(hipStream_t stream, int nseg, const void* const* src, void* const* dst, const long long* src_pitch, const long long* dst_pitch,
                       const int* row_bytes, const int* idx, int nrows) {
    if (nseg <= 0 || nrows <= 0) return 0;
    if (nseg > 12) return -1;
    GatherArgs a = {};
    for (int k = 0; k < nseg; ++k) {
        if (!src[k] || !dst[k] || row_bytes[k] <= 0 || (row_bytes[k] & 3) || (src_pitch[k] & 3) || (dst_pitch[k] & 3) ||
            ((uintptr_t)src[k] & 3) || ((uintptr_t)dst[k] & 3)) return -1;
        a.s[k].src = (const char*)src[k]; a.s[k].dst = (char*)dst[k]; a.s[k].src_pitch = src_pitch[k]; a.s[k].dst_pitch = dst_pitch[k];
        a.s[k].row_bytes = row_bytes[k];
        a.s[k].vec16 = !((row_bytes[k] | src_pitch[k] | dst_pitch[k]) & 15) && !(((uintptr_t)src[k] | (uintptr_t)dst[k]) & 15);
    }
    hipLaunchKernelGGL(gather_rows_kernel, dim3(nrows, nseg), dim3(256), 0, stream, a, idx);
    MMB_CHECK_LAUNCH();
    return 0;
}

int mmbert_rows_to_block(hipStream_t stream, const int64_t* ids, const void* rows, int rows_bf16, int ldr, int n, int H,
                         const int64_t* uni, int U, int V, float* block) {
    if (n <= 0 || U <= 0) return 0;
    if (!ids || !rows || !uni || !block || H <= 0 || ldr < H) return -1;
    hipLaunchKernelGGL(rows_to_block_kernel, dim3(n), dim3(256), 0, stream, ids, rows, rows_bf16, ldr, n, H, uni, U, V, block);
    MMB_CHECK_LAUNCH();
    return 0;
}

int mmbert_pack_i64(hipStream_t stream, int nseg, const int64_t* const* src, const long long* dst_offset, const long long* count,
                    const long long* fill, int64_t* out) {
    if (nseg <= 0) return 0;
    if (nseg > 12 || !out) return -1;
    PackArgs a = {};
    long long most = 0;
    for (int k = 0; k < nseg; ++k) {
        if (count[k] < 0 || dst_offset[k] < 0) return -1;
        a.s[k].src = src[k]; a.s[k].dst0 = dst_offset[k]; a.s[k].n = count[k]; a.s[k].fill = fill[k];
        most = count[k] > most ? count[k] : most;
    }
    if (most == 0) return 0;
    hipLaunchKernelGGL(pack_i64_kernel, dim3(grid_for((size_t)most, 256, 256), nseg), dim3(256), 0, stream, a, out);
    MMB_CHECK_LAUNCH();
    return 0;
}

int mmbert_mlm_mask(hipStream_t stream, int64_t* ids, int64_t* labels, size_t n, uint32_t rng_stream, uint32_t select_thr16,
                    uint32_t replace_thr16, int64_t special0, int64_t special1, int64_t special2, int64_t mask_id) {
    if (n == 0) return 0;
    if (n >= ((size_t)1 << 32) || select_thr16 > 65536u || replace_thr16 > 65536u) return -1;
    hipLaunchKernelGGL(mlm_mask_kernel, dim3(grid_for(n, 256, 1024)), dim3(256), 0, stream, ids, labels, n, rng_stream, select_thr16,
                       replace_thr16, special0, special1, special2, mask_id);
    MMB_CHECK_LAUNCH();
    return 0;
}

int mmbert_dropout_mask(hipStream_t stream, uint8_t* out, size_t n, uint32_t rng_stream, uint32_t thr16) {
    if (n == 0) return 0;
    hipLaunchKernelGGL(dropout_mask_kernel, dim3(grid_for(n, 256, 4096)), dim3(256), 0, stream, out, n, rng_stream, thr16);
    MMB_CHECK_LAUNCH();
    return 0;
}

}
```

### msa_amd/model.py

```python
from __future__ import annotations

import json
import os
from typing import Optional

import contextlib

import torch
import torch.nn as nn
import torch.nn.functional as F

from . import ops
from .flat import FlatParams

MODALITY_DIMS = {"mosi": (47, 74), "mosei": (35, 74), "ur_funny": (371, 81)}
LN_EPS_JOINT = 1e-5
MASK_NEG = -10000.0


class MMBertConfig:

    def __init__(self, vocab_size=30522, hidden_size=768, num_hidden_layers=12, num_attention_heads=12,
                 intermediate_size=3072, max_position_embeddings=512, type_vocab_size=2,
                 hidden_dropout_prob=0.1, attention_probs_dropout_prob=0.1, layer_norm_eps=1e-12,
# ... 323 lines not shown
                    saved.append((x, qkv, actx, lse, z1, m1, r1, y1, u, g, z2, m2, r2, d_att, d_h1, d_h2))
                x = y2
            return x, saved
        for i in range(nl):
            lw = top._lw[i]
            d_att, d_h1, d_h2 = (ops.make_drop(pa, seed, 8 * i), ops.make_drop(ph, seed, 8 * i + 1), ops.make_drop(ph, seed, 8 * i + 2))
            qkv = ops.gemm_nt(x, lw["Wqkv"], bias=lw["bqkv"])
            actx, lse = ops.attn_fwd(qkv, key_bias, layout, H, drop=d_att, kv_len=kv_len)
            if probe is not None:
                probe(i, qkv)
            z1 = ops.gemm_nt(actx, lw["Wo"], bias=lw["bo"], resid=x, drop=d_h1)
            y1, m1, r1 = ops.ln_fwd(z1, lw["ln1_g"], lw["ln1_b"], cfg.layer_norm_eps, stats=keep)
            u = torch.empty((x.shape[0], cfg.intermediate_size), device=x.device, dtype=torch.bfloat16) if keep else None
            g = ops.gemm_nt(y1, lw["W1"], bias=lw["b1"], gelu=True, aux=u)
            z2 = ops.gemm_nt(g, lw["W2"], bias=lw["b2"], resid=y1, drop=d_h2)
            last = i == L - 1 and y_out is not None
            y2, m2, r2 = ops.ln_fwd(z2, lw["ln2_g"], lw["ln2_b"], cfg.layer_norm_eps, stats=keep,
                                    out=y_out if last else None, out_rows=y_rows if last else None)
            if keep:
                saved.append((x, qkv, actx, lse, z1, m1, r1, y1, u, g, z2, m2, r2, d_att, d_h1, d_h2))
            x = y2
            if top.debug_hidden is not None:
                top.debug_hidden.setdefault("_layers_packed", []).append(None if last else y2.detach())
        return x, saved

    @staticmethod
    def run_top_first(top, x, layout, key_bias, kv_len, q_rows, probe=None):
        cfg = top.config
        H = cfg.hidden_size
        lw = top._lw[cfg.num_hidden_layers - 1]
        qkv = ops.gemm_nt(x, lw["Wqkv"], bias=lw["bqkv"])
        actx = ops.attn_fwd_first(qkv, key_bias, layout, H, q_rows, kv_len=kv_len)
        if probe is not None:
            probe(cfg.num_hidden_layers - 1, qkv)
        del qkv
        xr = ops.gather_rows([x], q_rows)[0]
        z1 = ops.gemm_nt(actx, lw["Wo"], bias=lw["bo"], resid=xr)
        y1, _, _ = ops.ln_fwd(z1, lw["ln1_g"], lw["ln1_b"], cfg.layer_norm_eps, stats=False)
        g = ops.gemm_nt(y1, lw["W1"], bias=lw["b1"], gelu=True)
        z2 = ops.gemm_nt(g, lw["W2"], bias=lw["b2"], resid=y1)
        y2, _, _ = ops.ln_fwd(z2, lw["ln2_g"], lw["ln2_b"], cfg.layer_norm_eps, stats=False)
        return y2

    @staticmethod
    def run_backward(top, layout, key_bias, kv_len, saved, dy, dy_rows, top_rows, compact=None, lnd=None):
        H = top.config.hidden_size
        L = top.config.num_hidden_layers
        top._flat.grads_dirty = True
        top._flat.attach_lazy()
        top._flat.wait_transposes()
        _join_wgrads(top)
        _join_heads(top)
        M_all = saved[0][0].shape[0]
        ra = layout.rows_a if getattr(layout, "split", False) else M_all
        if dy is not None and dy_rows is None and ra < dy.shape[0]:
            dy = dy[:ra]
        own_lnd = lnd is None
        if own_lnd:
            lnd = ops.LnDeferred(2 * L)
        pair_wgrads, held = getattr(top, "pair_wgrads", True), None
        dw = getattr(top, "defer_wgrads", None)
        if dw is None and _DEFER_ENV:
            dw = _DEFER_ENV != "0"
        if dw is None:
            dw = _auto_defer_wgrads(H, top.config.intermediate_size, L, x_dev=saved[0][0].device, rows=ra)
        defer_wgrads, deferred = (top.grad_hook is None and bool(dw)), []
        composite_bwd = getattr(top, "composite_layers", True) and ops.launches_unwrapped()
        AL = tq = None
        for i in reversed(range(L)):
            lw = top._lw[i]
            saved_i = saved[i]
            saved[i] = None
            if ra < M_all:
                saved_i = tuple(t[:ra] if torch.is_tensor(t) else t for t in saved_i)
            x, qkv, actx, lse, z1, m1, r1, y1, u, g, z2, m2, r2, d_att, d_h1, d_h2 = saved_i
            if i == L - 1 and (top_rows is not None or compact is not None):
                R = None
                R32 = None
                if compact is not None:
                    rows_l, rows_f, dy_c = compact
                    rinv = top.__dict__.get("_row_inverse")
                    if rinv is None or rinv.table.numel() < M_all or rinv.table.device != rows_f.device:
                        rinv = top.__dict__["_row_inverse"] = ops.RowInverse(M_all, rows_f.device)
                    R, R32 = ops.compact_rows(rows_l, rows_f, layout.inv if getattr(layout, "split", False) else None, inverse=rinv)
                elif top_rows is not None:
                    Ro = _EncoderFn._sparse_rows(top_rows, None, ra)
                    if Ro is not None:
                        R = layout.inv.index_select(0, Ro) if getattr(layout, "split", False) else Ro
                        src_rows = Ro if dy_rows is not None else R
                        (dy_c,) = ops.gather_rows([dy], src_rows.int())
                if R is not None:
                    dy = _EncoderFn._last_layer_sparse(top, lw, layout, key_bias, kv_len, saved_i, dy_c, R, H, ra, R32, lnd,
                                                       rinv if compact is not None else None, deferred if defer_wgrads else None)
                    if top.grad_hook is not None:
                        lnd.flush()
                    dy_rows = None
                    top._layer_grads_done(i)
                    continue
                if compact is not None:
                    raise RuntimeError("compact output gradient without the sparse top-layer path")
            if composite_bwd:
                dev, bf = z2.device, torch.bfloat16
                I_ = top.config.intermediate_size
                if AL is None:
                    AL = ops.attn_layout_struct(key_bias, layout, backward=True)
                    if kv_len is not None and not getattr(layout, "split", False):
                        AL.kv_len = kv_len.data_ptr()
                    tq = ops._tile_queue(dev)
                dz2, dz1, dy1, dctx, dx_ = (torch.empty((ra, H), device=dev, dtype=bf) for _ in range(5))
                dz2d = torch.empty((ra, H), device=dev, dtype=bf) if d_h2[1] else None
                dz1d = torch.empty((ra, H), device=dev, dtype=bf) if d_h1[1] else None
                du, dqkv = torch.empty((ra, I_), device=dev, dtype=bf), torch.empty((ra, 3 * H), device=dev, dtype=bf)
                delta = torch.empty((ra, layout.heads), device=dev, dtype=torch.float32)
                lnd.reserve(2, ra, H, dev)
                ws2 = lnd.slot(ra, H, dev, lw["g_ln2_g"], lw["g_ln2_b"], None)
                ws1 = lnd.slot(ra, H, dev, lw["g_ln1_g"], lw["g_ln1_b"], None)
                b = lw.get("_bwd_args")
                if b is None:
                    b = lw["_bwd_args"] = ops._LayerBwd()
                    for n in ("W2T", "W1T", "WoT", "WqkvT", "ln2_g", "ln1_g", "g_ln2_g", "g_ln2_b", "g_ln1_g", "g_ln1_b"):
                        assert lw[n].is_contiguous()
                        setattr(b, n, lw[n].data_ptr())
                    b.H, b.I = H, I_
                b.dy, b.lddy, b.dy_rows, b.rows = dy.data_ptr(), dy.stride(0), ops._ptr(dy_rows), ra
                b.z2, b.m2, b.r2, b.ln2_ws, b.z1, b.m1, b.r1, b.ln1_ws = z2.data_ptr(), m2.data_ptr(), r2.data_ptr(), ws2, z1.data_ptr(), m1.data_ptr(), r1.data_ptr(), ws1
                b.u, b.qkv, b.actx, b.lse = u.data_ptr(), qkv.data_ptr(), actx.data_ptr(), lse.data_ptr()
                b.dz2, b.dz2d, b.du, b.dy1, b.dz1, b.dz1d = dz2.data_ptr(), ops._ptr(dz2d), du.data_ptr(), dy1.data_ptr(), dz1.data_ptr(), ops._ptr(dz1d)
                b.dctx, b.dqkv, b.delta, b.dx, b.tile_queue = dctx.data_ptr(), dqkv.data_ptr(), delta.data_ptr(), dx_.data_ptr(), tq
                ops._set_drop(b.att, d_att); ops._set_drop(b.h1, d_h1); ops._set_drop(b.h2, d_h2)
                ops.layer_bwd(AL, b)
                dy_rows = None
                dy = dx_
                if dz2d is None:
                    dz2d = dz2
                if dz1d is None:
                    dz1d = dz1
            else:
              dz2d = torch.empty((ra, H), device=z2.device, dtype=torch.bfloat16) if d_h2[1] else None
              dz2 = ops.ln_bwd(dy, z2, m2, r2, lw["ln2_g"], lw["g_ln2_g"], lw["g_ln2_b"], dx2=dz2d, pre_drop=d_h2, deferred=lnd, dy_rows=dy_rows)
              dy_rows = None
              if dz2d is None:
                  dz2d = dz2
              du = ops.gemm_nt(dz2d, lw["W2T"], gelu_bwd_u=u)
              dy1 = ops.gemm_nt(du, lw["W1T"], resid=dz2)
              dz1d = torch.empty((ra, H), device=z2.device, dtype=torch.bfloat16) if d_h1[1] else None
              dz1 = ops.ln_bwd(dy1, z1, m1, r1, lw["ln1_g"], lw["g_ln1_g"], lw["g_ln1_b"], dx2=dz1d, pre_drop=d_h1, deferred=lnd)
              if dz1d is None:
                  dz1d = dz1
              dctx = ops.gemm_nt(dz1d, lw["WoT"])
              dqkv = ops.attn_bwd(qkv, actx, dctx, lse, key_bias, layout, H, drop=d_att, kv_len=kv_len)
              dy = ops.gemm_nt(dqkv, lw["WqkvT"], resid=dz1)
            probs = [(du, y1, lw["g_W1"], lw["g_b1"]), (dz2d, g, lw["g_W2"], lw["g_b2"]),
                     (dqkv, x, lw["g_Wqkv"], lw["g_bqkv"]), (dz1d, actx, lw["g_Wo"], lw["g_bo"])]
            if defer_wgrads:
                deferred.extend(probs)
                top._layer_grads_done(i)
                continue
            if pair_wgrads:
                if held is None and i > 0:
                    held = (i, probs)
                    continue
                if held is not None:
                    _wgrad(top, held[1] + probs)
                    if top.grad_hook is not None:
                        lnd.flush()
                    top._layer_grads_done(held[0])
                    held = None
                else:
                    _wgrad(top, probs)
            else:
                _wgrad(top, probs)
            if top.grad_hook is not None:
                lnd.flush()
            top._layer_grads_done(i)
        if own_lnd:
            lnd.flush()
        _flush_late_wgrads(top, deferred, deferred=defer_wgrads)
        return dy

    @staticmethod
    def _sparse_rows(top_rows, layout, ra):
        (idx, host, ev), first = top_rows
        n = _active_row_count(top_rows[0])
        r = n + first.numel()
        if 4 * r > ra or int(host[1]) != 0:
            return None
        R = torch.cat((idx[:n].long(), first))
        if layout is not None and getattr(layout, "split", False):
            R = layout.inv.index_select(0, R)
        return R

    @staticmethod
    def _last_layer_sparse(top, lw, layout, key_bias, kv_len, saved_i, dy_c, R, H, ra, R32=None, lnd=None, rinv=None, deferred=None):
        cfg = top.config
        x, qkv, actx, lse, z1, m1, r1, y1, u, g, z2, m2, r2, d_att, d_h1, d_h2 = saved_i
        if R32 is None:
            R32 = R.int()
        m2_c, r2_c, u_c, m1_c, r1_c, y1_c, g_c, actx_c = ops.gather_rows([m2, r2, u, m1, r1, y1, g, actx], R32)
        dy = dy_c
        dz2d_c = torch.empty_like(dy_c) if d_h2[1] else None
        dz2_c = ops.ln_bwd(dy_c, z2, m2_c, r2_c, lw["ln2_g"], lw["g_ln2_g"], lw["g_ln2_b"], x_rows=R32, dx2=dz2d_c, pre_drop=d_h2,
                           drop_rows=R32, deferred=lnd)
        if dz2d_c is None:
            dz2d_c = dz2_c
        du_c = ops.gemm_nt(dz2d_c, lw["W2T"], gelu_bwd_u=u_c)
        dy1_c = ops.gemm_nt_splitk(du_c, lw["W1T"], resid=dz2_c) if du_c.shape[0] <= 1024 else ops.gemm_nt(du_c, lw["W1T"], resid=dz2_c)
        dz1d_c = torch.empty_like(dy_c) if d_h1[1] else None
        dz1_c = ops.ln_bwd(dy1_c, z1, m1_c, r1_c, lw["ln1_g"], lw["g_ln1_g"], lw["g_ln1_b"], x_rows=R32, dx2=dz1d_c, pre_drop=d_h1,
                           drop_rows=R32, deferred=lnd)
        if dz1d_c is None:
            dz1d_c = dz1_c
        dctx_c = ops.gemm_nt(dz1d_c, lw["WoT"])
        if rinv is not None:
            dctx, dz1 = ops.scatter_rows_zero([dctx_c, dz1_c], rinv, ra)
        else:
            dctx = torch.zeros((ra, H), device=dy.device, dtype=torch.bfloat16)
            dctx.index_copy_(0, R, dctx_c)
        qlim = ops.attn_q_limit(R32, layout) if getattr(top, "top_layer_query_limit", True) else None
        dqkv = ops.attn_bwd(qkv, actx, dctx, lse, key_bias, layout, H, drop=d_att, kv_len=kv_len, q_limit=qlim)
        if rinv is None:
            dz1 = torch.zeros((ra, H), device=dy.device, dtype=torch.bfloat16)
            dz1.index_copy_(0, R, dz1_c)
        out = ops.gemm_nt(dqkv, lw["WqkvT"], resid=dz1)
        few = [(du_c, y1_c, lw["g_W1"], lw["g_b1"]), (dz2d_c, g_c, lw["g_W2"], lw["g_b2"]), (dz1d_c, actx_c, lw["g_Wo"], lw["g_bo"])]
        if deferred is not None and getattr(top, "late_wgrads", True):
            deferred.append((dqkv, x, lw["g_Wqkv"], lw["g_bqkv"]))
            for q in few:
                _late_wgrad(top, q, True)
        else:
            _wgrad(top, few)
            _wgrad(top, [(dqkv, x, lw["g_Wqkv"], lw["g_bqkv"])])
        return out


def _trunk_static(plan, B, T, lens, joff, dev):
    key = ("trunk_static", T, tuple(sorted(joff.items())))
    st = plan.get(key)
    if st is None:
        jrows = {}
        for k, lo in joff.items():
            b = torch.arange(B, dtype=torch.int32)[:, None] * lens[k] + torch.arange(T, dtype=torch.int32)[None, :] + lo
            jrows[k] = b.reshape(-1).to(dev)
        groups, k = [], 0
        while k < len(lens):
            k1 = k
            while k1 + 1 < len(lens) and ((k1 + 1) in joff) == (k in joff):
                k1 += 1
            groups.append((k in joff, k, k1 + 1, torch.cat([jrows[q] for q in range(k, k1 + 1)]) if k in joff else None))
            k = k1 + 1
        st = plan[key] = dict(jrows=jrows, groups=groups, arange=torch.arange(len(lens) * B * T, dtype=torch.int32, device=dev))
    return st


class _Trunk:
    __slots__ = ("ids", "tts", "B", "T", "lens", "pair_info", "feats", "feat_versions", "plan", "layout", "split", "key_bias", "kv_len", "seed", "top_rows",
                 "d_emb", "d_joint", "infer", "late_split", "compact", "J_pre", "predict", "attention", "dense")


class _TrunkFn(torch.autograd.Function):

    @staticmethod
    def forward(ctx, anchor, top, t):
        cfg, w = top.config, top._w
        H = cfg.hidden_size
        B, T, lens, plan, split = t.B, t.T, t.lens, t.plan, t.split
        bounds, tokens = plan["bounds"], plan["layout"].tokens
        dev = t.ids.device
        keep = ctx.needs_input_grad[0] and not t.predict
        late = t.layout
        npass = len(lens)
        joint = [k for k in range(npass) if t.pair_info[k] is not None]
        joff, jtot = {}, 0
        for k in joint:
            joff[k] = jtot
            jtot += B * lens[k]
        early = split is not None and not t.late_split and not t.infer
        dropped = split is not None and getattr(split, "dropped", False)
        Mx = split.rows_packed if early else tokens
        pad = 1 if (early and dropped) else 0
        pre = t.J_pre
        t.J_pre = None
        if pre is not None and pre[0].shape[0] == jtot:
            buf = torch.empty((Mx + pad, H), device=dev, dtype=torch.bfloat16)
            X, J = buf[:Mx], pre[0]
        else:
            pre = None
            buf = torch.empty((Mx + pad + jtot, H), device=dev, dtype=torch.bfloat16)
            X, J = buf[:Mx], buf[Mx + pad:]
        st = _trunk_static(plan, B, T, lens, joff, dev)
        e0 = ops.embed_gather(t.ids, t.tts, w["word"], w["type"], w["pos"], T)
        mean0 = torch.empty(npass * B * T, device=dev, dtype=torch.float32)
        rstd0 = torch.empty_like(mean0)
        for is_joint, k0, k1, jr in st["groups"]:
            rows = slice(k0 * B * T, k1 * B * T)
            if is_joint:
                out, orows = J, jr
            elif early:
                out, orows = X, split.inv32[bounds[k0]:bounds[k1]]
            else:
                out, orows = X[bounds[k0]:bounds[k1]], None
            ops.ln_fwd(e0[rows], w["emb_ln_g"], w["emb_ln_b"], cfg.layer_norm_eps, out=out, out_rows=orows, drop=t.d_emb, drop_row0=k0 * B * T,
                       stats=(mean0[rows], rstd0[rows]))
        jstats = {}
        for n, k in enumerate(joint):
            S = lens[k]
            Jk = J[joff[k]:joff[k] + B * S]
            off = T
            if pre is not None:
                torch.cuda.current_stream().wait_event(pre[1][n])
            else:
                for feat, which in zip(t.feats[k], t.pair_info[k][1]):
                    ops.pair_proj_fwd(feat, w[which + "_w"], w[which + "_b"], Jk, T, seq_len=S, offset=off)
                    off += feat.shape[1]
            if early:
                out, orows = X, split.inv32[bounds[k]:bounds[k + 1]]
            else:
                out, orows = X[bounds[k]:bounds[k + 1]], None
            _, m_, r_ = ops.ln_fwd(Jk, w["joint_ln_g"], w["joint_ln_b"], LN_EPS_JOINT, out=out, out_rows=orows, drop=t.d_joint[k])
            jstats[k] = (m_, r_)
        if top.debug_hidden is not None:
            e1 = torch.cat([(J[joff[k]:joff[k] + B * lens[k]].view(B, lens[k], H)[:, :T].reshape(B * T, H) if k in joff else
                             (torch.cat((X, X.new_zeros((1, H)))).index_select(0, split.inv[bounds[k]:bounds[k + 1]]) if early else X[bounds[k]:bounds[k + 1]]))
                            for k in range(npass)])
            xo = torch.cat((X, X.new_zeros((1, H)))).index_select(0, split.inv) if early else X
            top.debug_hidden.update(emb=e1.detach().clone(), x=xo.detach().clone())
            top.debug_hidden.pop("_layers_packed", None)
        if late is not None:
            split = t.split = late()
            t.layout = None
            dropped = split is not None and getattr(split, "dropped", False)
        x = X
        if split is not None and not early:
            x = X.index_select(0, split.perm)
        layout = split if split is not None else plan["layout"]
        y_out = y_rows = None
        if split is not None and not t.infer:
            y_out = (torch.zeros if dropped else torch.empty)((tokens, H), device=dev, dtype=torch.bfloat16)
            y_rows = split.perm32
        if t.predict and not t.dense:
# ... 11 lines not shown
            return _EncoderFn.run_top_first(top, y, layout, t.key_bias, kvl, q_rows, probe=probe)
        y, saved = _EncoderFn.run_forward(top, x, layout, t.key_bias, t.seed, None if split is not None else t.kv_len, keep, y_out, y_rows,
                                          train=False if t.predict else None)
        if split is not None and t.infer:
            y = y.index_select(0, split.inv)
        ctx.top, ctx.t, ctx.saved, ctx.joff, ctx.early = top, t, saved, joff, early
        if keep:
            ctx.save_for_backward(e0, mean0, rstd0, J, *[x_ for k in joint for x_ in jstats[k]])
        return y

    @staticmethod
    def backward(ctx, dy):
        top, t = ctx.top, ctx.t
        cfg, w = top.config, top._w
        H = cfg.hidden_size
        e0, mean0, rstd0, J, *js = ctx.saved_tensors
        B, T, lens, plan, split = t.B, t.T, t.lens, t.plan, t.split
        bounds = plan["bounds"]
        st = _trunk_static(plan, B, T, lens, ctx.joff, e0.device)
        npass = len(lens)
        layout = split if split is not None else plan["layout"]
        compact, t.compact = t.compact, None
        if not any(q[2] is w["g_word_pad"] for q in _late_pending(top)):
            top._flat.settle([w["g_word_pad"]])
        lnd = top._shared_lnd()
        if top.head_grad_hook is not None:
            lnd.flush()
            top.head_grad_hook()
        dy_rows = None
        if compact is None:
            dy = dy.contiguous()
            if split is not None:
                dy_rows = split.perm32[:split.rows_a]
        dx = _EncoderFn.run_backward(top, layout, t.key_bias, None if split is not None else t.kv_len, ctx.saved, dy, dy_rows, t.top_rows,
                                     compact, lnd)
        ctx.saved = None
        top._flat.settle([w["g_word_pad"]])
        if split is not None:
            top.last_backward_row_fraction = float(split.rows_a) / split.tokens
        ra = dx.shape[0]
        inv32 = split.inv32 if split is not None else None
        limit = ra if split is not None else 0
        dJ = torch.empty_like(J)
        de0 = torch.empty_like(e0)
        joint = sorted(ctx.joff)
        for n, k in enumerate(joint):
            S = lens[k]
            lo = ctx.joff[k]
            m_, r_ = js[2 * n], js[2 * n + 1]
            if split is not None:
                ops.ln_bwd(dx, J[lo:lo + B * S], m_, r_, w["joint_ln_g"], w["g_joint_ln_g"], w["g_joint_ln_b"], dx=dJ[lo:lo + B * S],
                           dy_rows=inv32[bounds[k]:bounds[k + 1]], dy_row_limit=limit, post_drop=t.d_joint[k], deferred=lnd)
            else:
                ops.ln_bwd(dx[bounds[k]:bounds[k + 1]], J[lo:lo + B * S], m_, r_, w["joint_ln_g"], w["g_joint_ln_g"], w["g_joint_ln_b"],
                           dx=dJ[lo:lo + B * S], post_drop=t.d_joint[k], deferred=lnd)
        for n, k in enumerate(joint):
            S = lens[k]
            lo = ctx.joff[k]
            off = T
            _check_unchanged(t.feats[k], t.feat_versions[k])
            for feat, which in zip(t.feats[k], t.pair_info[k][1]):
                ops.pair_proj_bwd(feat, J[lo:lo + B * S], dJ[lo:lo + B * S], T, w["g_" + which + "_w"], w["g_" + which + "_b"], seq_len=S, offset=off)
                off += feat.shape[1]
        for is_joint, k0, k1, jr in st["groups"]:
            rows = slice(k0 * B * T, k1 * B * T)
            kw = dict(dx=de0[rows], post_drop=t.d_emb, drop_rows=st["arange"][rows] if t.d_emb[1] else None, deferred=lnd)
            if is_joint:
                ops.ln_bwd(dJ, e0[rows], mean0[rows], rstd0[rows], w["emb_ln_g"], w["g_emb_ln_g"], w["g_emb_ln_b"], dy_rows=jr, **kw)
            elif split is not None:
                ops.ln_bwd(dx, e0[rows], mean0[rows], rstd0[rows], w["emb_ln_g"], w["g_emb_ln_g"], w["g_emb_ln_b"],
                           dy_rows=inv32[bounds[k0]:bounds[k1]], dy_row_limit=limit, **kw)
            else:
                ops.ln_bwd(dx[bounds[k0]:bounds[k1]], e0[rows], mean0[rows], rstd0[rows], w["emb_ln_g"], w["g_emb_ln_g"], w["g_emb_ln_b"], **kw)
        lnd.flush()
        _join_wgrads(top)
        if top.defer_embed_rows:
            ops.embed_scatter(t.ids, t.tts, de0, T, None, w["g_type"], w["g_pos"], vocab=cfg.vocab_size)
            top.__dict__.setdefault("_deferred_embed_rows", []).append((t.ids, de0))
        else:
            ops.embed_scatter(t.ids, t.tts, de0, T, w["g_word"], w["g_type"], w["g_pos"])
        return None, None, None


def mlm_active_rows(labels, vocab, first=None):
    idx, cnt = ops.active_rows(labels, vocab)
    dup = (labels.index_select(0, first) != -100).sum().to(torch.int32).view(1) if first is not None else torch.zeros_like(cnt)
    bad = ((labels != -100) & ((labels < 0) | (labels >= vocab))).sum().to(torch.int32).view(1)
    host = torch.empty(3, dtype=torch.int32, pin_memory=True)
    host.copy_(torch.cat((cnt, dup, bad)), non_blocking=True)
    ev = torch.cuda.Event()
    ev.record()
    return idx, host, ev


def _active_row_count(rows) -> int:
    _idx, host, ev = rows
    ev.synchronize()
    if int(host[2]) != 0:
        raise IndexError(f"masked_labels: {int(host[2])} label(s) are neither -100 nor in [0, vocab_size) -- Target out of bounds")
    return int(host[0])


_ones = {}


class _ScalarLoss(torch.Tensor):

    def mean(self, *args, **kwargs):
        if self.dim() == 0 and not args and not kwargs:
            return self
        return super().mean(*args, **kwargs)

    def backward(self, gradient=None, retain_graph=None, create_graph=False, inputs=None):
        if gradient is None and not create_graph:
            with torch._C.DisableTorchFunctionSubclass():
                if self.dim() == 0:
                    if self._backward_hooks or self.retains_grad or self.grad_fn is None:
                        gradient = torch.ones((), dtype=self.dtype, device=self.device)
                    else:
                        key = (self.dtype, self.device)
                        gradient = _ones.get(key)
                        if gradient is None:
                            gradient = _ones[key] = torch.ones((), dtype=self.dtype, device=self.device)
        return torch.autograd.backward(self, gradient, retain_graph, create_graph, inputs=inputs)


def _scalar_loss(loss):
    return loss.as_subclass(_ScalarLoss) if (torch.is_tensor(loss) and loss.dim() == 0 and type(loss) is torch.Tensor) else loss


_dummies = {}


def _zero_dummy(M, H, dtype, device):
    key = (dtype, str(device))
    z = _dummies.get(key)
    if z is None:
        z = _dummies[key] = torch.zeros((1, 1), dtype=dtype, device=device)
    return z.expand(M, H)


class _MLMHeadFn(torch.autograd.Function):

    @staticmethod
    def forward(ctx, y, anchor, top, labels, seg_bounds_host, seg_bounds, want_scores, rows=None, first_rows=None, trunk=None, leave_rows=False):
        cfg, w = top.config, top._w
        ctx.trunk = trunk
        M, H = y.shape
        V, Vp = cfg.vocab_size, top._flat.vpad
        keep = ctx.needs_input_grad[0]
        y = y.contiguous()
        ctx.compact = False
        ctx.first_rows = first_rows
        first = None
        if first_rows is not None:
            if leave_rows:
                first = torch.empty((first_rows.numel(), H), device=y.device, dtype=torch.float32)
            else:
                first = y.index_select(0, first_rows).float()
        if (not want_scores) and keep and rows is not None and getattr(top, "sparse_mlm_backward", True):
            idx_all, host, ev = rows
            n = _active_row_count(rows)
            if 0 < n and 2 * n <= M:
                sel32 = idx_all[:n]
                sel = sel32.long()
                y_c = y.index_select(0, sel)
                pre_c = torch.empty_like(y_c)
                t0_c = ops.gemm_nt(y_c, w["Wt"], bias=w["bt"], gelu=True, aux=pre_c)
                t_c, mean_c, rstd_c = ops.ln_fwd(t0_c, w["mlm_ln_g"], w["mlm_ln_b"], cfg.layer_norm_eps, stats=True)
                logits_c = ops.gemm_nt(t_c, w["word_h"], bias=w["pred_bias"])
                labels_c = labels.index_select(0, sel)
                nseg = len(seg_bounds_host) - 1
                bounds_c = torch.searchsorted(sel32, seg_bounds.to(sel32.dtype)).to(torch.int32)
                loss, inv, lse = ops.ce_fwd(logits_c, V, labels_c, bounds_c, nseg)
                ctx.top, ctx.nseg, ctx.compact, ctx.M = top, nseg, True, M
                ctx.set_materialize_grads(False)
                ctx.save_for_backward(y_c, pre_c, t0_c, mean_c, rstd_c, t_c, logits_c, labels_c, bounds_c, inv, lse, sel)
                return loss, None, first
        pre = torch.empty_like(y) if keep else None
        t0 = ops.gemm_nt(y, w["Wt"], bias=w["bt"], gelu=True, aux=pre)
        t, mean, rstd = ops.ln_fwd(t0, w["mlm_ln_g"], w["mlm_ln_b"], cfg.layer_norm_eps, stats=keep)
        f32_scores = want_scores and getattr(top, "scores_dtype", torch.bfloat16) == torch.float32
        logits = ops.gemm_nt(t, w["word_h"], bias=w["pred_bias"], out_f32=f32_scores)
        nseg = len(seg_bounds_host) - 1
        loss, inv, lse = ops.ce_fwd(logits, V, labels, seg_bounds, nseg)
        ctx.top, ctx.nseg, ctx.keep_logits, ctx.M = top, nseg, want_scores, M
        ctx.set_materialize_grads(False)
        ctx.rows = None
        if keep and getattr(top, "sparse_mlm_backward", True):
            ctx.rows = rows if rows is not None else mlm_active_rows(labels, V)
        if keep:
            ctx.save_for_backward(y, pre, t0, mean, rstd, t, logits, labels, seg_bounds, inv, lse)
        out_logits = logits if want_scores else None
        if out_logits is not None:
            ctx.mark_non_differentiable(out_logits)
        return loss, out_logits, first

    @staticmethod
    def backward(ctx, dloss, _unused, dfirst=None):
        t = ctx.trunk
        nf = t.top_rows[1].numel() if (t is not None and t.top_rows is not None and dfirst is not None) else 0
        res = _MLMHeadFn._backward(ctx, dloss, extra_rows=nf)
        _join_heads(ctx.top)
        nones = (None,) * 10
        if isinstance(res, tuple):
            sel, dy_all = res
            n = sel.numel()
            dyl = dy_all[:n]
            if nf and _MLMHeadFn._compact_ok(ctx, t, n, dfirst):
                first = t.top_rows[1]
                df = dfirst if dfirst.shape[0] == first.numel() else dfirst.view(-1, first.numel(), dfirst.shape[1]).sum(0)
                dy_all[n:].copy_(df)
                t.compact = (sel, first, dy_all)
                return (_zero_dummy(ctx.M, dyl.shape[1], dyl.dtype, dyl.device),) + nones
            dy = torch.zeros((ctx.M, dyl.shape[1]), device=dyl.device, dtype=dyl.dtype)
            if n:
                dy.index_copy_(0, sel.long(), dyl)
        else:
            dy = res
        if dfirst is not None:
            if dy is None:
                dy = torch.zeros((ctx.M, dfirst.shape[1]), device=dfirst.device, dtype=torch.bfloat16)
            dy.index_add_(0, ctx.first_rows, dfirst.to(dy.dtype))
        return (dy,) + nones

    @staticmethod
    def _compact_ok(ctx, t, n, dfirst):
        (idx, host, ev), first = t.top_rows
        ra = t.split.rows_a if t.split is not None else t.plan["layout"].tokens
        if ctx.first_rows is None or (ctx.first_rows.numel() % first.numel()) != 0:
            return False
        return 4 * (n + first.numel()) <= ra and int(host[1]) == 0 and n == _active_row_count(t.top_rows[0])

    @staticmethod
    def _few_rows_backward(top, dl, t_c, t0_c, pre_c, y_c, mean_c, rstd_c, lnd, late, extra_rows):
        w = top._w
        n = dl.shape[0]
        _late_wgrad(top, (dl, t_c, w["g_word_pad"], w["g_pred_bias"]), late)
        dt = ops.gemm_nt_splitk(dl, w["wordT"])
        dt0 = ops.ln_bwd(dt, t0_c, mean_c, rstd_c, w["mlm_ln_g"], w["g_mlm_ln_g"], w["g_mlm_ln_b"], deferred=lnd)
        dpre = ops.gelu_bwd(dt0, pre_c)
        _late_wgrad(top, (dpre, y_c, w["g_Wt"], w["g_bt"]), late)
        dy_all = torch.empty((n + extra_rows, y_c.shape[1]), device=y_c.device, dtype=torch.bfloat16)
        ops.gemm_nt(dpre, w["WtT"], out=dy_all[:n])
        return dy_all

    @staticmethod
    def _backward(ctx, dloss, extra_rows=0):
        w = ctx.top._w
        V = ctx.top.config.vocab_size
        if dloss is None:
            return None
        ctx.top._flat.grads_dirty = True
        ctx.top._flat.attach_lazy()
        ctx.top._flat.wait_transposes()
        gs = dloss.contiguous().float()
        lnd = ctx.top._shared_lnd() if (ctx.trunk is not None and ctx.needs_input_grad[0]) else None
        late = (ctx.trunk is not None and ctx.needs_input_grad[0] and ctx.top.grad_hook is None and ctx.top.head_grad_hook is None
                and getattr(ctx.top, "late_wgrads", True))
        if ctx.top.__dict__.get("_late_wgrads"):
            _flush_late_wgrads(ctx.top)
        if ctx.compact:
            y_c, pre_c, t0_c, mean_c, rstd_c, t_c, logits_c, labels_c, bounds_c, inv, lse, sel = ctx.saved_tensors
            dl = ops.ce_bwd(logits_c, V, labels_c, bounds_c, ctx.nseg, inv, gs, lse, logits_c)
            return sel, _MLMHeadFn._few_rows_backward(ctx.top, dl, t_c, t0_c, pre_c, y_c, mean_c, rstd_c, lnd, late, extra_rows)
        y, pre, t0, mean, rstd, t, logits, labels, seg_bounds, inv, lse = ctx.saved_tensors
        M = y.shape[0]
        if ctx.rows is not None:
# ... 191 lines not shown

    def _stage_labels(self, passes, label_parts):
        pk = self._pack_inputs(passes, label_parts)
        if pk is not None:
            return pk[2], pk[:2]
        ids = passes[0]["ids"]
        side = self._prologue_stream(ids) if label_parts[0].is_cuda else None
        with (torch.cuda.stream(side) if side is not None else contextlib.nullcontext()):
            labels = torch.cat([l.reshape(-1) for l in label_parts]) if len(label_parts) > 1 else label_parts[0].reshape(-1)
            labels = labels.to(device=ids.device, dtype=torch.long)
        if side is not None:
            labels.record_stream(torch.cuda.current_stream())
        return labels, None

    def _encode(self, passes, labels=None, want_rows=False, rowset=False, packed=None, predict=False, attention=None):
        bert = self._bert()
        dev = passes[0]["ids"].device
        self._ensure_ready(dev)
        if not predict:
            lnd = self.__dict__.get("_lnd")
            if lnd is not None and lnd.items and torch.is_grad_enabled():
                lnd.drop()
            self._drop_leftovers()
        B, T = passes[0]["ids"].shape
        cfg = self.config
        if T > cfg.max_position_embeddings:
            raise ValueError("text length exceeds max_position_embeddings")
        seed = 0 if predict else self._next_seed()
        je = bert.jointEmbeddings
        rowset = bool(rowset and labels is not None and torch.is_grad_enabled() and getattr(self, "skip_padded_backward", True)
                      and getattr(self, "skip_masked_keys", True))
        segs, lens, pair_info = [], [], []
        side = None if predict else self._prologue_stream(passes[0]["ids"])
        with (torch.cuda.stream(side) if side is not None else contextlib.nullcontext()):
            for k, p in enumerate(passes):
                segs.append((self._mask2d(p["mask"], False, dev), k, 0))
                if p.get("pair") is not None:
                    pairs = p["pair"] if isinstance(p["pair"], (tuple, list)) else (p["pair"],)
                    pmasks = p["pair_mask"] if isinstance(p["pair_mask"], (tuple, list)) else (p["pair_mask"],)
                    off = T
                    for f, pm in zip(pairs, pmasks):
                        segs.append((self._mask2d(pm, True, dev), k, off))
                        off += f.shape[1]
                    lens.append(off)
                    pair_info.append((pairs, tuple(je.which(f) for f in pairs)))
                else:
                    lens.append(T)
                    pair_info.append(None)
        plan = self._plan(lens, B, dev)
        if side is None:
            pro = ops.prologue(segs, lens, B, labels, cfg.vocab_size, dev, rowset=rowset)
            nseq = pro.nseq
            host = torch.empty(nseq + 3, dtype=torch.int32, pin_memory=True)
            host.copy_(pro.words, non_blocking=True)
            ev = torch.cuda.Event()
            ev.record()
        else:
            main = torch.cuda.current_stream()
            k = self._pro_calls = getattr(self, "_pro_calls", 0) + 1
            marks = self.__dict__.setdefault("_pro_marks", {})
            if (k - 1) % 2 in marks:
                side.wait_event(marks[(k - 1) % 2])
            nf, ni = ops.prologue_sizes(lens, B, rowset)
            sets = self.__dict__.setdefault("_pro_bufs", {})
            bufs = sets.get(k % 2)
            if bufs is None or bufs[0].numel() < nf or bufs[1].numel() < ni or bufs[0].device != dev:
                bufs = sets[k % 2] = (torch.empty(nf, device=dev, dtype=torch.float32), torch.empty(ni, device=dev, dtype=torch.int32))
                side.wait_stream(main)
            with torch.cuda.stream(side):
                pro = ops.prologue(segs, lens, B, labels, cfg.vocab_size, dev, bufs=bufs, rowset=rowset)
                nseq = pro.nseq
                host = torch.empty(nseq + 3, dtype=torch.int32, pin_memory=True)
                host.copy_(pro.words, non_blocking=True)
                ev = torch.cuda.Event()
                ev.record()
            mark = torch.cuda.Event()
            mark.record(main)
            marks[k % 2] = mark
            main.wait_event(ev)
        key_bias = pro.key_bias
        if not predict:
            self._last_valid_dev = pro.valid
        rows = (pro.idx, host[nseq:], ev) if want_rows else None
        kv_len = pro.kv_len if getattr(self, "skip_masked_keys", True) else None
        infer = (predict or ((not self.training) and (not torch.is_grad_enabled()))) and getattr(self, "dedupe_masked_rows", True)
        if not predict:
            self.last_backward_row_fraction = 1.0
        pending = None
        if kv_len is not None:
            if infer:
                pending = self._request_lengths(plan, kv_len, labels, True, (pair_info, B, T))
            elif labels is not None and torch.is_grad_enabled() and getattr(self, "skip_padded_backward", True):
                pending = (host[:nseq], None, ev)
        if packed is not None:
            ids, tts = packed
        else:
            ids = torch.cat([p["ids"].reshape(-1).long() for p in passes])
            tts = torch.cat([(p["tt"].reshape(-1).long() if p.get("tt") is not None else torch.zeros(B * T, dtype=torch.long, device=dev)) for p in passes])
        if self.embed_ids_hook is not None and torch.is_grad_enabled():
            if packed is not None or side is None:
                early_ids = ids
            else:
                with torch.cuda.stream(side):
                    early_ids = torch.cat([p["ids"].reshape(-1).long() for p in passes])
            self.embed_ids_hook(early_ids, side)
        p_emb = cfg.hidden_dropout_prob if (self.training and not predict) else 0.0
        p_joint = je.dropout_prob if (self.training and je.training and not predict) else 0.0
        t = _Trunk()
        t.compact = None
        t.predict = bool(predict)
        t.dense = predict == "dense"
        t.attention = attention if predict else None
        t.ids, t.tts, t.B, t.T, t.lens, t.pair_info, t.plan = ids, tts, B, T, lens, pair_info, plan
        t.feats = [None if info is None else tuple(_pair_features(f, dev) for f in info[0]) for info in pair_info]
        t.feat_versions = [None if fs is None else tuple(f._version for f in fs) for fs in t.feats]
        t.J_pre = None
        if getattr(self, "pairs_side_stream", True) and dev.type == "cuda" and any(info is not None for info in pair_info):
            w_ = self._w
            jtot = sum(B * lens[k] for k in range(len(lens)) if pair_info[k] is not None)
            J = torch.empty((jtot, cfg.hidden_size), device=dev, dtype=torch.bfloat16)
            evs, lo = [], 0
            main = torch.cuda.current_stream()
            for n, k in enumerate(k for k in range(len(lens)) if pair_info[k] is not None):
                S = lens[k]
                s_ = ops.side_stream("pairs%d" % n, dev)
                s_.wait_stream(main)
                with torch.cuda.stream(s_):
                    off = T
                    for feat, which in zip(t.feats[k], pair_info[k][1]):
                        ops.pair_proj_fwd(feat, w_[which + "_w"], w_[which + "_b"], J[lo:lo + B * S], T, seq_len=S, offset=off)
                        off += feat.shape[1]
                    evs.append(s_.record_event())
                lo += B * S
            t.J_pre = (J, evs)
        t.key_bias, t.kv_len, t.seed, t.infer = key_bias, kv_len, seed, infer
        t.d_emb = ops.make_drop(p_emb, seed, 1000)
        t.d_joint = [ops.make_drop(p_joint, seed, 1001 + k) for k in range(len(lens))]
        t.top_rows = (rows, plan["first"]) if (rows is not None and getattr(self, "sparse_top_layer_backward", True)) else None
        drop = (not infer) and labels is not None and not getattr(self, "return_scores", True)
        rank = pro.rank
        on_device = pending is not None and not infer and not drop and getattr(self, "device_split_layout", True) and len(lens) * B <= 1024
        t.late_split = side is None and not on_device
        t.split = None
        get_split = lambda: self._split_layout(plan, kv_len, pending, infer, drop, rank)
        if not t.late_split:
            t.split = get_split()
            get_split = None
        t.layout = get_split
        y = _TrunkFn.apply(bert.embeddings.LayerNorm.weight, self, t)
        split = t.split
        if predict:
            return y, plan, lens, rows, None
        if self.debug_hidden is not None:
            packed = self.debug_hidden.pop("_layers_packed", [])
            if split is not None:
                pad = getattr(split, "dropped", False)
                packed = [None if q is None else (torch.cat((q, q.new_zeros((1, q.shape[1])))) if pad else q).index_select(0, split.inv) for q in packed]
            self.debug_hidden["layers"] = [y.detach() if q is None else q for q in packed]
        return y, plan, lens, rows, t

    def _request_lengths(self, plan, kv_len, labels, infer=False, pairs=None):
        assert infer
        pair_info, B, T = pairs
        keep, bad = [], torch.zeros((), dtype=torch.int64, device=kv_len.device)
        for k, info in enumerate(pair_info):
            kv = kv_len[k * B:(k + 1) * B]
            if info is None:
                keep.append(torch.full_like(kv, T))
                continue
            kv = kv.clamp(min=T)
            keep.append(kv)
            off = T
            for f in info[0]:
                pos = off + torch.arange(f.shape[1], device=kv.device)[None, :]
                bad = bad + ((pos >= kv[:, None].long()) & (f.to(kv.device) != 0).any(-1)).sum()
                off += f.shape[1]
        kv_len = torch.cat(keep)
        host = torch.empty(kv_len.numel() + 1, dtype=torch.int32, pin_memory=True)
        host.copy_(torch.cat((kv_len, bad.to(torch.int32).view(1))), non_blocking=True)
        ev = torch.cuda.Event()
        ev.record()
        return host[:-1], host[-1:], ev

    def _split_layout(self, plan, kv_len, pending, infer=False, drop=False, rank=None):
        if pending is None:
            return None
        lay = plan["layout"]
        valid_host, flag, ev = pending
        if not infer and not drop and getattr(self, "device_split_layout", True) and len(lay.lens) <= 1024:
            lay2 = ops.DeviceSplitLayout(lay, self._last_valid_dev, kv_len.device, rank=rank, words=(valid_host, ev))
            return lay2
        ev.synchronize()
        if flag is not None and int(flag[0]) != 0:
            return None
        valid = valid_host.numpy().copy()
        if rank is None and int(valid.sum()) > 0.97 * lay.tokens:
            return None
        if infer:
            return ops.SplitLayout(lay, valid, kv_len.device, dedupe=True)
        self.last_backward_row_fraction = float(valid.sum()) / lay.tokens
        lay2 = ops.SplitLayout(lay, valid, kv_len.device, drop=drop, rank=rank)
        lay2.dropped = drop
        return lay2

class MMBertModel(_GpuModelBase):

    def __init__(self, config, _owner=None):
        super().__init__()
        self.config = config
        holder = _make_bert_holder(config)
        self.embeddings, self.encoder, self.pooler = holder.embeddings, holder.encoder, holder.pooler
        self._init_runtime()
        self._owner = _owner
        _hf_init(self, config.initializer_range)

    def set_joint_embeddings(self, dataset):
        self.dataset = dataset
        self.jointEmbeddings = JointEmbeddings(self.config.hidden_size, 0.5, dataset)
        dev = self.embeddings.word_embeddings.weight.device
        self.jointEmbeddings.to(dev)
# ... 283 lines not shown
        logits_out = torch.tanh(lo) if tanh_lo else lo
        ctx.mark_non_differentiable(t_rel, rel, logits_out)
        ctx.set_materialize_grads(False)
        ctx.mark_non_differentiable(aux)
        return loss, aux, logits_out, t_rel, rel

    @staticmethod
    def backward(ctx, d, *_unused):
        if d is None:
            return None, None, None, None, None
        first, P, Apre, g, Cc, T, seeds = ctx.saved_tensors
        top, B = ctx.top, ctx.B
        H = P.shape[1]
        pool, al, at = top.bert.pooler.dense, top.cls.align, top.attn
        vs3 = (top.vt, top.vv, top.vs)
        c1, c2 = top.classifier1_1, top.classifier1_2
        qs = (top.cpc_zt.net, top.cpc_zv.net, top.cpc_za.net)
        n = 3 * B * H
        dev = first.device
        d1 = d.reshape(1).float().contiguous()
        coef = (ctx.alpha / ctx.nmlm) if ctx.nmlm else 0.0
        dfirst, dmlm = _HeadsFn._backward_chain(ctx, top, first, P, Apre, g, Cc, T, seeds, d1, ctx.nmlm, coef)
        return dfirst, None, None, None, dmlm

    @staticmethod
    def _backward_chain(ctx, top, first, P, Apre, g, Cc, T, seeds, d1, nmlm, coef):
        B = ctx.B
        H = P.shape[1]
        pool, al, at = top.bert.pooler.dense, top.cls.align, top.attn
        vs3 = (top.vt, top.vv, top.vs)
        c1, c2 = top.classifier1_1, top.classifier1_2
        qs = (top.cpc_zt.net, top.cpc_zv.net, top.cpc_za.net)
        n = 3 * B * H
        seeds, zb, dmlm = ops.heads_seed(seeds, d1, 7 * B * H, nmlm, coef)
        dXP, dPc = seeds[:n].view(3, B, H), seeds[n:2 * n].view(3 * B, H)
        dlo, drel = seeds[2 * n:2 * n + B].view(B, 1), seeds[2 * n + B:].view(2 * B, 2)
        dT, dC, dfirst = zb[:B * H].view(B, H), zb[B * H:4 * B * H].view(B, 3 * H), zb[4 * B * H:].view(3 * B, H)
        ops.skinny_mm([(dT, None, 0, False, [(dXP[0], qs[0].weight, 1, 0), (dXP[1], qs[1].weight, 1, 0), (dXP[2], qs[2].weight, 1, 0),
                                            (dlo, c2.weight, 1, 0)])])
        ops.skinny_mm([(dC, None, 0, False, [(dT, c1.weight, 1, 0)])])
        dP, dA, E, dg = ops.heads_gate_bwd(dC, P, Apre, g, [v.weight for v in vs3], dPc, B)
        ops.skinny_mm([(dP, None, 0, True, [(dA, at.weight[:, :H], 1, 0), (dA, at.weight[:, H:], 1, 0)])])
        dpre = ops.heads_tanh_bwd(dP, P)
        ops.skinny_mm([(dfirst, None, 0, False, [(dpre, pool.weight, 1, 0), (drel, al.weight, 1, B)])])
        ops.skinny_wgrad([(dXP[m], T, qs[m].weight.grad, qs[m].bias.grad) for m in range(3)]
                         + [(dlo, T, c2.weight.grad, c2.bias.grad), (dT, Cc, c1.weight.grad, c1.bias.grad),
                            (dA, P, at.weight.grad[:, :H], at.bias.grad), (dA, P, at.weight.grad[:, H:], None),
                            (dpre, first, pool.weight.grad, pool.bias.grad), (drel, first[B:], al.weight.grad, al.bias.grad)])
        E3, dg3 = E.view(3, B, H), dg.view(3, B, 1)
        ops.heads_colsum([(E3[m], vs3[m].weight.grad) for m in range(3)] + [(dg3[m], vs3[m].bias.grad) for m in range(3)])
        return dfirst, dmlm


class MMBertForPretraining(_GpuModelBase):

    def __init__(self, config, num_labels=None, _bert=None):
        super().__init__()
        import weakref
        self.config = config
        H = config.hidden_size
        self.bert = _bert if _bert is not None else MMBertModel(config, _owner=weakref.ref(self))
        self.cls = MMBertPreTrainingHeads(config)
        self.cls._owner = weakref.ref(self)
        self.num_labels = 7 if num_labels is None else self._check_num_labels(num_labels)
        self.classifier1_1 = nn.Linear(H * 3, H)
        self.classifier1_2 = nn.Linear(H, 1 if self.num_labels in (1, 7) else self.num_labels)
        self.attn = nn.Linear(H * 2, H)
        self.relu = nn.ReLU()
        self.vt, self.vs, self.vv = nn.Linear(H, 1), nn.Linear(H, 1), nn.Linear(H, 1)
        self.tanh, self.sigmoid = nn.Tanh(), nn.Sigmoid()
        self.dropout = nn.Dropout(0.38)
        self.alpha, self.beta = 1, 1
        self.cpc_zt, self.cpc_zv, self.cpc_za = (CPC(H, H, 1, "Tanh") for _ in range(3))
        self._init_runtime()
        self.return_scores = True
        self.scores_dtype = torch.bfloat16
        self.token_chunk_rows = 4096
        self.fused_heads = os.environ.get("MMBERT_FUSED_HEADS", "1") != "0"
        self.coop_heads = True
        self.late_wgrads = True
        self.wgrad_side_stream = True
        self.heads_side_stream = True
        self.pairs_side_stream = True
        _hf_init(self, config.initializer_range, skip=_bert)
        self.cls.predictions.decoder.weight = self.bert.embeddings.word_embeddings.weight

    @property
    def deterministic(self) -> bool:
        return ops.deterministic()

    @deterministic.setter
    def deterministic(self, on: bool):
        ops.set_deterministic(bool(on))

    @staticmethod
    def _checkpoint_keys(sd):
        out = {}
        for k, v in sd.items():
            if k.endswith("position_ids"):
                continue
            if k.endswith("LayerNorm.gamma"):
                k = k[:-len("gamma")] + "weight"
            elif k.endswith("LayerNorm.beta"):
                k = k[:-len("beta")] + "bias"
            out[k] = v
        if out and not any(k.startswith(("bert.", "cls.")) for k in out) and any(k.startswith(("embeddings.", "encoder.")) for k in out):
            out = {"bert." + k: v for k, v in out.items()}
        return out

    @classmethod
    def from_pretrained(cls, name_or_path, ignore_unexpected=True, num_labels=None, **kw):
        import warnings
        if not os.path.isdir(name_or_path):
            raise OSError(f"{name_or_path}: from_pretrained needs a local checkpoint directory (no network access)")
        with open(os.path.join(name_or_path, "config.json")) as fh:
            cfg = MMBertConfig(**json.load(fh))
        model = cls(cfg, num_labels=num_labels)
        st = os.path.join(name_or_path, "model.safetensors")
        if os.path.exists(st):
            from safetensors.torch import load_file
            sd = load_file(st)
        else:
            sd = torch.load(os.path.join(name_or_path, "pytorch_model.bin"), map_location="cpu")
        sd = cls._checkpoint_keys(sd)
        res = model.load_state_dict(sd, strict=False)
        alias = {"cls.predictions.decoder.weight": "bert.embeddings.word_embeddings.weight", "cls.predictions.decoder.bias": "cls.predictions.bias"}
        alias.update({v: k for k, v in list(alias.items())})
        hf_side = ("bert.embeddings.", "bert.encoder.", "bert.pooler.", "cls.predictions.", "cls.seq_relationship.")
        missing = [k for k in res.missing_keys if k.startswith(hf_side) and alias.get(k) not in sd]
        unexpected = list(res.unexpected_keys)
        model.load_report = dict(missing=missing, unexpected=unexpected)
        core = [k for k in missing if k.startswith(("bert.embeddings.", "bert.encoder."))]
        if core:
            raise ValueError(f"{name_or_path}: the checkpoint has no tensor for {len(core)} encoder parameter(s): {core[:8]}"
                             f"{' ...' if len(core) > 8 else ''} (key names after the legacy renames: see _checkpoint_keys)")
        if unexpected:
            msg = f"{name_or_path}: {len(unexpected)} checkpoint tensor(s) match no parameter of MMBertForPretraining: {unexpected[:8]}{' ...' if len(unexpected) > 8 else ''}"
            if not ignore_unexpected:
                raise ValueError(msg + " (ignore_unexpected=False was requested; the default loads the rest and warns)")
            warnings.warn(msg)
        fresh = [k for k in missing if k.startswith(("cls.", "bert.pooler."))]
        if fresh:
            warnings.warn(f"{name_or_path}: newly initialised (not in the checkpoint): {fresh}")
        return model

    def set_alpha_beta(self, alpha, beta):
        self.alpha, self.beta = alpha, beta

    @staticmethod
    def _check_num_labels(n) -> int:
        if isinstance(n, bool) or int(n) != n or not 1 <= int(n) <= 16:
            raise ValueError(f"num_labels = {n!r}: 1 or 7 (regression, one output) or a class count from 2 to 16 (one 16-wide tile of the heads kernels)")
        return int(n)

    def set_num_labels(self, n):
        n = self._check_num_labels(n)
        width = 1 if n in (1, 7) else n
        old = self.classifier1_2
        if old.out_features != width:
            new = nn.Linear(old.in_features, width)
            _hf_init(new, self.config.initializer_range)
            self.classifier1_2 = new.to(device=old.weight.device, dtype=old.weight.dtype)
            self._flat = None
        self.num_labels = n
        return self

# ... 289 lines not shown
```

### msa_amd/ops.py

```python
from __future__ import annotations

import ctypes
import os
from typing import Optional, Tuple

import numpy as np
import torch

from . import _lib

EPI_BIAS, EPI_GELU, EPI_RESID, EPI_GELU_BWD, EPI_OUT_F32 = 1, 2, 4, 8, 16

SIDE_TRANSPOSES = True
SIDE_STREAM_PRIORITY = "low"
_side_streams = {}


def side_stream(tag: str, device) -> "torch.cuda.Stream":
    key = (tag, str(device), SIDE_STREAM_PRIORITY)
    s = _side_streams.get(key)
    if s is None:
        prio = 0
        if SIDE_STREAM_PRIORITY == "low":
            try:
# ... 527 lines not shown
         self.qtile_qend, self.seq_start, self.kv_len, start_b_dev) = part
        self.nftiles, self.ntiles = nf, nq
        M = base.tokens
        if on_gpu:
            rs_d, rp_d = base.row_tables(device)
            dev_p = torch.empty(n_packed + M, dtype=torch.int64, device=device)
            dev_p32 = torch.empty(n_packed + M, dtype=torch.int32, device=device)
            _lib.check(_lib.load().mmbert_split_rows(_stream(), rs_d.data_ptr(), rp_d.data_ptr(), self.seq_start.data_ptr(), start_b_dev.data_ptr(),
                                                     self.kv_len.data_ptr(), mode, M, self.rows_a, dev_p.data_ptr(), dev_p.data_ptr() + 8 * n_packed,
                                                     _ptr(rank), dev_p32.data_ptr(), dev_p32.data_ptr() + 4 * n_packed),
                       "mmbert_split_rows")
        else:
            dev_p = torch.from_numpy(np.concatenate((perm, inv))).to(device)
            dev_p32 = dev_p.to(torch.int32)
        self.perm, self.inv = dev_p[:n_packed], dev_p[n_packed:]
        self.perm32, self.inv32 = dev_p32[:n_packed], dev_p32[n_packed:]
        self.rows_packed = n_packed
        self.base, self.heads, self.tokens, self.lens = base, base.heads, base.tokens, base.lens
        self.seq_len, self.elem_base, self.bias_start, self.bias_len = base.seq_len, base.elem_base, base.bias_start, base.bias_len
        self.split = True


class DeviceSplitLayout:

    split = True
    dropped = False

    def __init__(self, base: SeqLayout, valid_dev, device, rank=None, words=None):
        lib = _lib.load()
        ns = len(base.lens)
        rows = base._rows_f
        nq_max = sum((n + rows - 1) // rows for n in base.lens)
        nf_max = nq_max + ns
        xs = 8 // int(np.gcd(base.heads, 8))
        buf = torch.empty(4 * nf_max + 4 * nq_max + 3 * ns + 4, device=device, dtype=torch.int32)
        _lib.check(lib.mmbert_split_layout(_stream(), base.seq_len.data_ptr(), valid_dev.data_ptr(), ns, rows, xs, nf_max, nq_max, buf.data_ptr()),
                   "mmbert_split_layout")
        cut = np.cumsum([0, nf_max, nf_max, nf_max, nf_max, nq_max, nq_max, nq_max, nq_max, ns, ns, ns, 4])
        part = [buf[cut[k]:cut[k + 1]] for k in range(12)]
        (self.ftile_seq, self.ftile_r0, self.ftile_qshift, self.ftile_qend, self.tile_seq, self.tile_r0, self.qtile_qshift,
         self.qtile_qend, self.seq_start, self.kv_len, start_b_dev, self.counts) = part
        self.nftiles = nf_max
        M = base.tokens
        rs_d, rp_d = base.row_tables(device)
        dev_p = torch.empty(2 * M, dtype=torch.int64, device=device)
        dev_p32 = torch.empty(2 * M, dtype=torch.int32, device=device)
        _lib.check(lib.mmbert_split_rows(_stream(), rs_d.data_ptr(), rp_d.data_ptr(), self.seq_start.data_ptr(), start_b_dev.data_ptr(),
                                         self.kv_len.data_ptr(), 0, M, 0, dev_p.data_ptr(), dev_p.data_ptr() + 8 * M, _ptr(rank),
                                         dev_p32.data_ptr(), dev_p32.data_ptr() + 4 * M), "mmbert_split_rows")
        self.perm, self.inv = dev_p[:M], dev_p[M:]
        self.perm32, self.inv32 = dev_p32[:M], dev_p32[M:]
        self.rows_packed = M
        self.base, self.heads, self.tokens, self.lens = base, base.heads, base.tokens, base.lens
        self.seq_len, self.elem_base, self.bias_start, self.bias_len = base.seq_len, base.elem_base, base.bias_start, base.bias_len
        self._words, self._host = words, None

    def _resolve(self):
        if self._host is None:
            if self._words is not None:
                host, ev = self._words
                ev.synchronize()
                v = np.minimum(host.numpy().astype(np.int64), np.asarray(self.lens, dtype=np.int64))
            else:
                v = self.kv_len.cpu().numpy().astype(np.int64)
            rows = self.base._rows_f
            self._host = (int(v.sum()), int(((v + rows - 1) // rows).sum()), [int(x) for x in v])
        return self._host

    rows_a = property(lambda self: self._resolve()[0])
    ntiles = property(lambda self: self._resolve()[1])
    valid_host = property(lambda self: self._resolve()[2])


def pad_key_bias(key_bias, layout: "SeqLayout"):
    out = torch.full((layout.bias_len,), NO_KEY, device=key_bias.device, dtype=torch.float32)
    out.index_copy_(0, layout.bias_index, key_bias.float())
    return out


_MASK_DTYPES = {torch.float32: 0, torch.float64: 1, torch.int64: 2, torch.int32: 3, torch.bfloat16: 4, torch.uint8: 5, torch.bool: 5, torch.float16: 6}


class Prologue:
    __slots__ = ("key_bias", "kv_len", "valid", "idx", "words", "nseq", "rank")


def prologue_sizes(pass_lens, B, rowset=False):
    nseq = len(pass_lens) * B
    tokens = sum(B * S for S in pass_lens)
    nf = sum(B * ((S + 127) // 128 * 128) for S in pass_lens)
    ni = 2 * nseq + 3 * nseq + max(tokens, 1) + nseq + 3
    return (2 * nf, ni + max(tokens, 1)) if rowset else (nf, ni)


def prologue(segs, pass_lens, B, labels, vocab, device, bufs=None, rowset=False) -> Prologue:
    lib = _lib.load()
    n, npass = len(segs), len(pass_lens)
    nseq = npass * B
    tokens = sum(B * S for S in pass_lens)
    bias_len, nints = prologue_sizes(pass_lens, B)
    nf_all, ni_all = prologue_sizes(pass_lens, B, rowset)
    out = Prologue()
    out.nseq = nseq
    out.rank = None
    if bufs is not None:
        fl, ints_all = bufs[0][:nf_all], bufs[1][:ni_all]
        assert fl.numel() == nf_all and ints_all.numel() == ni_all and ints_all.dtype == torch.int32 and fl.dtype == torch.float32
    else:
        fl = torch.empty(nf_all, device=device, dtype=torch.float32)
        ints_all = torch.empty(ni_all, device=device, dtype=torch.int32)
    out.key_bias, ints = fl[:bias_len], ints_all[:nints]
    bias_perm = None
    if rowset:
        out.rank, bias_perm = ints_all[nints:], fl[bias_len:]
    out.kv_len, out.valid = ints[:nseq], ints[nseq:2 * nseq]
    seq_cnt = ints[2 * nseq:5 * nseq]
    out.idx = ints[5 * nseq:5 * nseq + max(tokens, 1)]
    out.words = ints[5 * nseq + max(tokens, 1):]
    PA, LA, IA = ctypes.c_void_p * max(n, 1), ctypes.c_longlong * max(n, 1), ctypes.c_int * max(n, 1)
    for m, _, _ in segs:
        assert m.dim() == 2 and m.shape[0] == B and m.device.type == "cuda" and m.dtype in _MASK_DTYPES, (m.shape, m.dtype, m.device)
    es = [m.element_size() for m, _, _ in segs]
    if labels is not None:
        assert labels.dtype == torch.int64 and labels.is_contiguous() and labels.numel() == tokens
    _lib.check(lib.mmbert_prologue(_stream(), n, PA(*[m.data_ptr() for m, _, _ in segs]), LA(*[m.stride(0) * e for (m, _, _), e in zip(segs, es)]),
                                   LA(*[m.stride(1) * e for (m, _, _), e in zip(segs, es)]), IA(*[_MASK_DTYPES[m.dtype] for m, _, _ in segs]),
                                   IA(*[p for _, p, _ in segs]), IA(*[o for _, _, o in segs]), IA(*[m.shape[1] for m, _, _ in segs]),
                                   npass, (ctypes.c_int * npass)(*pass_lens), B, _ptr(labels), int(vocab),
                                   out.key_bias.data_ptr(), out.kv_len.data_ptr(), out.valid.data_ptr(), seq_cnt.data_ptr(), out.idx.data_ptr(),
                                   out.words.data_ptr(), _ptr(out.rank), _ptr(bias_perm)), "mmbert_prologue")
    if rowset:
        out.key_bias = bias_perm
    return out


def attn_kv_len(key_bias_padded, layout: SeqLayout):
    assert key_bias_padded.numel() == layout.bias_len and key_bias_padded.dtype == torch.float32
    out = torch.empty(layout.seq_len.numel(), device=key_bias_padded.device, dtype=torch.int32)
    _lib.check(_lib.load().mmbert_attn_kv_len(_stream(), key_bias_padded.data_ptr(), layout.bias_start.data_ptr(), layout.seq_len.data_ptr(),
                                              out.numel(), out.data_ptr()), "mmbert_attn_kv_len")
    return out


def attn_fwd(qkv, key_bias, layout: SeqLayout, H, *, drop: Drop = None, ctx=None, lse=None, kv_len=None):
    lib = _lib.load()
    M = qkv.shape[0]
    if key_bias.numel() != layout.bias_len or layout.bias_len == M:
        key_bias = pad_key_bias(key_bias, layout) if key_bias.numel() == M else key_bias
    assert qkv.shape[1] == 3 * H and qkv.is_contiguous()
    if getattr(layout, "split", False):
        kv_len = layout.kv_len
    if ctx is None:
        ctx = torch.empty((M, H), device=qkv.device, dtype=torch.bfloat16)
    if lse is None:
        lse = torch.empty((M, layout.heads), device=qkv.device, dtype=torch.float32)
    d = drop or NO_DROP
    _lib.check(lib.mmbert_attn_fwd(_stream(), qkv.data_ptr(), ctx.data_ptr(), lse.data_ptr(), key_bias.data_ptr(), layout.bias_start.data_ptr(), H, layout.heads,
                                   layout.seq_start.data_ptr(), layout.seq_len.data_ptr(), layout.elem_base.data_ptr(),
                                   layout.ftile_seq.data_ptr(), layout.ftile_r0.data_ptr(), layout.nftiles, d[0], d[1], d[2], _ptr(kv_len),
                                   _ptr(getattr(layout, "ftile_qshift", None)), _ptr(getattr(layout, "ftile_qend", None))), "mmbert_attn_fwd")
    return ctx, lse


def attn_fwd_first(qkv, key_bias, layout: SeqLayout, H, q_rows, *, kv_len=None):
    lib = _lib.load()
    M = qkv.shape[0]
    if key_bias.numel() != layout.bias_len or layout.bias_len == M:
        key_bias = pad_key_bias(key_bias, layout) if key_bias.numel() == M else key_bias
    assert qkv.shape[1] == 3 * H and qkv.is_contiguous() and qkv.dtype == torch.bfloat16
    if getattr(layout, "split", False):
        kv_len = layout.kv_len
    ns = layout.seq_len.numel()
    assert q_rows.dtype == torch.int32 and q_rows.is_contiguous() and q_rows.numel() == ns and key_bias.dtype == torch.float32
    ctx = torch.empty((ns, H), device=qkv.device, dtype=torch.bfloat16)
    _lib.check(lib.mmbert_attn_fwd_first(_stream(), qkv.data_ptr(), ctx.data_ptr(), key_bias.data_ptr(), layout.bias_start.data_ptr(), H, layout.heads,
                                         layout.seq_start.data_ptr(), layout.seq_len.data_ptr(), q_rows.data_ptr(), ns, _ptr(kv_len)),
               "mmbert_attn_fwd_first")
    return ctx


def attn_probs_first(qkv, key_bias, layout: SeqLayout, H, q_rows, *, kv_len=None, out=None):
    lib = _lib.load()
    M = qkv.shape[0]
    if key_bias.numel() != layout.bias_len or layout.bias_len == M:
        key_bias = pad_key_bias(key_bias, layout) if key_bias.numel() == M else key_bias
    assert qkv.shape[1] == 3 * H and qkv.is_contiguous() and qkv.dtype == torch.bfloat16
    if getattr(layout, "split", False):
        kv_len = layout.kv_len
    ns = layout.seq_len.numel()
    assert q_rows.dtype == torch.int32 and q_rows.is_contiguous() and q_rows.numel() == ns and key_bias.dtype == torch.float32
    ld = max(max(layout.lens, default=1), 1)
    if out is None:
        out = torch.empty((ns, layout.heads, ld), device=qkv.device, dtype=torch.float32)
    assert out.shape == (ns, layout.heads, ld) and out.dtype == torch.float32 and out.is_contiguous() and out.device == qkv.device
    probs = out
    _lib.check(lib.mmbert_attn_probs_first(_stream(), qkv.data_ptr(), probs.data_ptr(), ld, key_bias.data_ptr(), layout.bias_start.data_ptr(), H,
                                           layout.heads, layout.seq_start.data_ptr(), layout.seq_len.data_ptr(), q_rows.data_ptr(), ns, _ptr(kv_len)),
               "mmbert_attn_probs_first")
    return probs


def attn_q_limit(rows32, layout):
    ns = layout.seq_len.numel()
    out = torch.empty(ns, device=rows32.device, dtype=torch.int32)
    _lib.check(_lib.load().mmbert_attn_q_limit(_stream(), rows32.data_ptr(), rows32.numel(), layout.seq_start.data_ptr(), ns, out.data_ptr()),
               "mmbert_attn_q_limit")
    return out


def attn_bwd(qkv, ctx, dctx, lse, key_bias, layout: SeqLayout, H, *, drop: Drop = None, dqkv=None, kv_len=None, q_limit=None):
    lib = _lib.load()
    M = qkv.shape[0]
    if dqkv is None:
        dqkv = torch.empty_like(qkv)
    delta = torch.empty((M, layout.heads), device=qkv.device, dtype=torch.float32)
    d = drop or NO_DROP
    if key_bias.numel() != layout.bias_len or layout.bias_len == M:
        key_bias = pad_key_bias(key_bias, layout) if key_bias.numel() == M else key_bias
    assert dctx.is_contiguous() and ctx.is_contiguous()
    split = getattr(layout, "split", False)
    if split:
        q_seq, q_r0, nq = layout.tile_seq, layout.tile_r0, layout.ntiles
        kv_len = layout.kv_len
    else:
        q_seq, q_r0, nq = layout.ftile_seq, layout.ftile_r0, layout.nftiles
    _lib.check(lib.mmbert_attn_bwd(_stream(), qkv.data_ptr(), ctx.data_ptr(), dctx.data_ptr(), dqkv.data_ptr(), lse.data_ptr(), delta.data_ptr(),
                                   key_bias.data_ptr(), layout.bias_start.data_ptr(), H, layout.heads, layout.seq_start.data_ptr(), layout.seq_len.data_ptr(),
                                   layout.elem_base.data_ptr(), q_seq.data_ptr(), q_r0.data_ptr(), nq,
                                   layout.tile_seq.data_ptr(), layout.tile_r0.data_ptr(), layout.ntiles,
                                   d[0], d[1], d[2], _ptr(kv_len), _ptr(getattr(layout, "qtile_qshift", None)), _ptr(getattr(layout, "qtile_qend", None)),
                                   1 if split else 0, _ptr(q_limit)), "mmbert_attn_bwd")
    return dqkv


def attn_dropout_mask(S, elem_base, head, drop, device):
    lib = _lib.load()
    out = torch.empty((S, S), device=device, dtype=torch.uint8)
    _lib.check(lib.mmbert_attn_dropout_mask(_stream(), out.data_ptr(), S, elem_base, head, drop[0], drop[1]), "mmbert_attn_dropout_mask")
    return out


def ce_fwd(logits, V, labels, seg_bounds, nseg):
    lib = _lib.load()
    M = logits.shape[0]
    inv = torch.empty(4, device=logits.device, dtype=torch.float32)
    loss = torch.empty(nseg, device=logits.device, dtype=torch.float32)
    lse = torch.empty(M, device=logits.device, dtype=torch.float32)
    assert logits.dtype in (torch.bfloat16, torch.float32)
    row_loss = _ws_f32(M, logits.device) if deterministic() else None
    _lib.check(lib.mmbert_ce_fwd(_stream(), logits.data_ptr(), logits.stride(0), V, labels.data_ptr(), M, seg_bounds.data_ptr(), nseg,
                                 inv.data_ptr(), loss.data_ptr(), lse.data_ptr(), 1 if logits.dtype == torch.float32 else 0, _ptr(row_loss)),
               "mmbert_ce_fwd")
    return loss, inv, lse


def ce_bwd(logits, V, labels, seg_bounds, nseg, inv, gscale, lse, dlogits, rows=None):
    lib = _lib.load()
    M = logits.shape[0]
    _lib.check(lib.mmbert_ce_bwd(_stream(), logits.data_ptr(), logits.stride(0), V, labels.data_ptr(), M, seg_bounds.data_ptr(), nseg,
                                 inv.data_ptr(), gscale.data_ptr(), lse.data_ptr(), dlogits.data_ptr(), dlogits.stride(0),
                                 _ptr(rows), 0 if rows is None else rows.numel(), 1 if logits.dtype == torch.float32 else 0), "mmbert_ce_bwd")
    return dlogits


def vocab_topk(logits, V, k, labels=None):
    lib = _lib.load()
    assert logits.dim() == 2 and logits.dtype in (torch.bfloat16, torch.float32) and logits.stride(1) in (0, 1)
    M, dev = logits.shape[0], logits.device
    k = int(k)
    assert int(V) <= logits.shape[1], f"vocab_topk: V = {V} columns asked of a [{M}, {logits.shape[1]}] tensor"
    assert M == 0 or logits.data_ptr() % 16 == 0, "vocab_topk: the logits must start on a 16-byte boundary (a column-offset view does not)"
    top_ids = torch.empty((M, max(k, 0)), device=dev, dtype=torch.int32)
    top_lp = torch.empty((M, max(k, 0)), device=dev, dtype=torch.float32)
    lse = torch.empty(M, device=dev, dtype=torch.float32)
    lab_lp = lab_rank = None
    if labels is not None:
        assert labels.dtype == torch.int64 and labels.numel() == M and labels.is_contiguous()
        lab_lp = torch.empty(M, device=dev, dtype=torch.float32)
        lab_rank = torch.empty(M, device=dev, dtype=torch.int32)
    ldv = logits.stride(0) if (M > 1 or logits.stride(0) >= logits.shape[1]) else logits.shape[1]
    _lib.check(lib.mmbert_vocab_topk(_stream(), logits.data_ptr(), ldv, int(V), M,
                                     1 if logits.dtype == torch.float32 else 0, k, _ptr(labels), top_ids.data_ptr(), top_lp.data_ptr(),
                                     lse.data_ptr(), _ptr(lab_lp), _ptr(lab_rank)), "mmbert_vocab_topk")
    return (top_ids, top_lp, lse) if labels is None else (top_ids, top_lp, lse, lab_lp, lab_rank)


def active_rows(labels, V):
    lib = _lib.load()
    M = labels.numel()
    idx = torch.empty(max(M, 1), device=labels.device, dtype=torch.int32)
    count = torch.empty(1, device=labels.device, dtype=torch.int32)
    _lib.check(lib.mmbert_active_rows(_stream(), labels.data_ptr(), M, V, idx.data_ptr(), count.data_ptr()), "mmbert_active_rows")
    return idx, count


def adamw(p, g, m, v, p_bf16, flags, *, lr, beta1=0.9, beta2=0.999, eps=1e-6, wd=0.01, step=1, gscale=1.0, mode=0, zero_grad=True):
    lib = _lib.load()
    _lib.check(lib.mmbert_adamw(_stream(), p.data_ptr(), g.data_ptr(), m.data_ptr(), v.data_ptr(), _ptr(p_bf16), flags.data_ptr(), p.numel(),
                                float(lr), float(beta1), float(beta2), float(eps), float(wd), int(step), float(gscale), int(mode),
                                1 if zero_grad else 0), "mmbert_adamw")


def adamw_devscale(p, g, m, v, p_bf16, flags, coef, *, lr, beta1=0.9, beta2=0.999, eps=1e-6, wd=0.01, step=1, mode=0, zero_grad=True):
    lib = _lib.load()
    _lib.check(lib.mmbert_adamw_devscale(_stream(), p.data_ptr(), g.data_ptr(), m.data_ptr(), v.data_ptr(), _ptr(p_bf16), flags.data_ptr(),
                                         p.numel(), float(lr), float(beta1), float(beta2), float(eps), float(wd), int(step), coef.data_ptr(),
                                         int(mode), 1 if zero_grad else 0), "mmbert_adamw_devscale")


ADAMW_MAX_GROUPS, ADAMW_MAX_SLOTS = 255, 64


def adamw_grouped(p, g, m, v, p_bf16, flags, group_of_block, hyper, *, step=1, gscale=1.0, coef=None, mode=0, zero_grad=True):
    hyper = [tuple(float(x) for x in h) for h in hyper]
    assert all(len(h) == 5 for h in hyper) and group_of_block.dtype == torch.uint8 and group_of_block.numel() * 256 >= p.numel()
    arr = (ctypes.c_double * (5 * max(1, len(hyper))))(*[x for h in hyper for x in h])
    _lib.check(_lib.load().mmbert_adamw_grouped(_stream(), p.data_ptr(), g.data_ptr(), m.data_ptr(), v.data_ptr(), _ptr(p_bf16),
                                                flags.data_ptr(), group_of_block.data_ptr(), p.numel(), arr, len(hyper), int(step),
                                                float(gscale), None if coef is None else coef.data_ptr(), int(mode),
                                                1 if zero_grad else 0), "mmbert_adamw_grouped")


GRAD_NORM_WORKSPACE = 8192


def grad_norm(g, segs, nseg, *, max_norm, norm_type=2.0, gscale=1.0, workspace=None, out=None):
    assert g.dtype == torch.float32 and g.is_contiguous() and segs.dtype == torch.int64 and segs.is_contiguous()
    if workspace is None:
        workspace = torch.empty(GRAD_NORM_WORKSPACE // 8, dtype=torch.float64, device=g.device)
    assert workspace.numel() * workspace.element_size() >= GRAD_NORM_WORKSPACE
    if out is None:
        out = torch.empty(3, dtype=torch.float32, device=g.device)
    _lib.check(_lib.load().mmbert_grad_norm(_stream(), g.data_ptr(), g.numel(), segs.data_ptr(), int(nseg), float(norm_type), float(max_norm),
                                            float(gscale), workspace.data_ptr(), out.data_ptr()), "mmbert_grad_norm")
# ... 72 lines not shown
    _lib.check(_lib.load().mmbert_heads_seed(_stream(), seeds.data_ptr(), n, d.data_ptr(), base, base + 4 * n, nzero, base + 4 * (n + nzero), nmlm, float(coef)),
               "mmbert_heads_seed")
    return buf[:n], buf[n:n + nzero], (buf[n + nzero:] if nmlm else None)


def heads_gate_bwd(dC, P, Apre, g, vws, dPc, B):
    H = P.shape[1]
    dP, dA, E = torch.empty_like(P), torch.empty_like(P), torch.empty_like(P)
    dg = torch.empty(3 * B, device=P.device, dtype=torch.float32)
    _lib.check(_lib.load().mmbert_heads_gate_bwd(_stream(), dC.data_ptr(), P.data_ptr(), Apre.data_ptr(), g.data_ptr(), _ptr3(vws), dPc.data_ptr(), B, H,
                                                 dP.data_ptr(), dA.data_ptr(), E.data_ptr(), dg.data_ptr()), "mmbert_heads_gate_bwd")
    return dP, dA, E, dg


def heads_tanh_(x):
    _lib.check(_lib.load().mmbert_heads_tanh(_stream(), x.data_ptr(), x.numel()), "mmbert_heads_tanh")
    return x


def heads_tanh_bwd(dP, P):
    dpre = torch.empty_like(P)
    _lib.check(_lib.load().mmbert_heads_tanh_bwd(_stream(), dP.data_ptr(), P.data_ptr(), dpre.data_ptr(), P.numel()), "mmbert_heads_tanh_bwd")
    return dpre


class RowInverse:

    def __init__(self, nrows, device):
        self.table = torch.zeros(nrows, device=device, dtype=torch.int64)
        self.stamp, self.nlist = 0, 0

    def next(self, nlist):
        self.stamp = self.stamp % 0xFFFFFFF0 + 1
        self.nlist = nlist
        return self.stamp


def compact_rows(rows, extra, row_map=None, inverse: "RowInverse" = None):
    n, ne = rows.numel(), extra.numel()
    out64 = torch.empty(n + ne, device=extra.device, dtype=torch.int64)
    out32 = torch.empty(n + ne, device=extra.device, dtype=torch.int32)
    assert rows.dtype in (torch.int32, torch.int64) and extra.dtype == torch.int64 and rows.is_contiguous() and extra.is_contiguous()
    assert row_map is None or (row_map.dtype == torch.int64 and row_map.is_contiguous())
    r32, r64 = (rows.data_ptr(), None) if rows.dtype == torch.int32 else (None, rows.data_ptr())
    if inverse is None:
        _lib.check(_lib.load().mmbert_compact_rows(_stream(), r32, r64, n, extra.data_ptr(), ne, _ptr(row_map), out64.data_ptr(), out32.data_ptr()), "mmbert_compact_rows")
    else:
        _lib.check(_lib.load().mmbert_compact_rows_inv(_stream(), r32, r64, n, extra.data_ptr(), ne, _ptr(row_map), out64.data_ptr(), out32.data_ptr(),
                                                       inverse.table.data_ptr(), inverse.next(n + ne)), "mmbert_compact_rows_inv")
    return out64, out32


def scatter_rows_zero(srcs, inverse: "RowInverse", nrows):
    n = len(srcs)
    assert 0 < n <= 4 and nrows <= inverse.table.numel() and inverse.stamp != 0
    outs = [torch.empty((nrows, t.shape[1]), device=t.device, dtype=t.dtype) for t in srcs]
    if nrows == 0:
        return outs
    for t in srcs:
        assert t.dim() == 2 and t.stride(1) == 1 and t.shape[0] == inverse.nlist
    LA = ctypes.c_longlong * n
    rb = [t.shape[1] * t.element_size() for t in srcs]
    _lib.check(_lib.load().mmbert_scatter_rows_zero(_stream(), n, _PtrArr[n](*[t.data_ptr() for t in srcs]), _PtrArr[n](*[o.data_ptr() for o in outs]),
                                                    LA(*[t.stride(0) * t.element_size() for t in srcs]), LA(*rb), _IntArr[n](*rb),
                                                    inverse.table.data_ptr(), inverse.stamp, inverse.nlist, nrows), "mmbert_scatter_rows_zero")
    return outs


def gather_rows(srcs, idx32):
    n = len(srcs)
    assert 0 < n <= 12 and idx32.dtype == torch.int32 and idx32.is_contiguous()
    rows = idx32.numel()
    outs = [torch.empty((rows,) + tuple(t.shape[1:]), device=t.device, dtype=t.dtype) for t in srcs]
    if rows == 0:
        return outs
    for t in srcs:
        assert t.dim() in (1, 2) and (t.dim() == 1 or t.stride(1) == 1)
    LA = ctypes.c_longlong * n
    rb = [(t.shape[1] if t.dim() == 2 else 1) * t.element_size() for t in srcs]
    _lib.check(_lib.load().mmbert_gather_rows(_stream(), n, _PtrArr[n](*[t.data_ptr() for t in srcs]), _PtrArr[n](*[o.data_ptr() for o in outs]),
                                              LA(*[t.stride(0) * t.element_size() for t in srcs]), LA(*[b for b in rb]),
                                              _IntArr[n](*rb), idx32.data_ptr(), rows), "mmbert_gather_rows")
    return outs


def pack_i64(segments, total=None):
    LA = ctypes.c_longlong * len(segments)
    srcs, offs, cnts, fills, keep = [], [], [], [], []
    off = 0
    dev = None
    for sg in segments:
        if torch.is_tensor(sg):
            assert sg.dtype == torch.int64 and sg.is_cuda
            t = sg.reshape(-1)
            if not t.is_contiguous():
                t = t.contiguous()
            keep.append(t)
            srcs.append(t.data_ptr()); cnts.append(t.numel()); fills.append(0)
            dev = t.device
        else:
            srcs.append(None); cnts.append(int(sg[0])); fills.append(int(sg[1]))
        offs.append(off)
        off += cnts[-1]
    out = torch.empty(off if total is None else total, device=dev, dtype=torch.int64)
    n = len(segments)
    _lib.check(_lib.load().mmbert_pack_i64(_stream(), n, _PtrArr[n](*srcs), LA(*offs), LA(*cnts), LA(*fills), out.data_ptr()), "mmbert_pack_i64")
    return out, offs


def heads_colsum(pairs):
    n = len(pairs)
    PA, IA = _PtrArr[n], _IntArr[n]
    _lib.check(_lib.load().mmbert_heads_colsum(_stream(), n, PA(*[s.data_ptr() for s, _ in pairs]), PA(*[d.data_ptr() for _, d in pairs]),
                                               IA(*[s.shape[0] for s, _ in pairs]), IA(*[s.shape[1] for s, _ in pairs]),
                                               IA(*[s.stride(0) for s, _ in pairs])), "mmbert_heads_colsum")


_VP, _VP3 = ctypes.c_void_p, ctypes.c_void_p * 3


class _HeadsStep(ctypes.Structure):
    _fields_ = ([("B", ctypes.c_int), ("H", ctypes.c_int), ("tanh_lo", ctypes.c_int), ("nmlm", ctypes.c_int), ("alpha", ctypes.c_float), ("beta", ctypes.c_float),
                 ("first", _VP), ("y", _VP), ("first_rows", _VP), ("ldy", ctypes.c_int), ("ncls", ctypes.c_int), ("ap", _VP), ("ap2", _VP), ("sent", _VP), ("mlm", _VP)]
                + [(n, _VP) for n in ("Wp", "bp", "Wal", "bal", "Wsr", "bsr", "Wat", "bat")] + [("vw", _VP3), ("vb", _VP3)]
                + [(n, _VP) for n in ("Wc1", "bc1", "Wc2", "bc2")] + [("Wq", _VP3), ("bq", _VP3)]
                + [(n, _VP) for n in ("loss", "aux", "out5", "logits", "t_rel", "rel", "ws", "dloss", "dfirst", "dmlm")]
                + [(n, _VP) for n in ("gWp", "gbp", "gWal", "gbal", "gWat", "gbat")] + [("gvw", _VP3), ("gvb", _VP3)]
                + [(n, _VP) for n in ("gWc1", "gbc1", "gWc2", "gbc2")] + [("gWq", _VP3), ("gbq", _VP3)] + [("sync", _VP), ("sent_cls", _VP), ("pred", _VP)])


_heads_sync = {}
_heads_struct_checked = False


def heads_step_struct() -> "_HeadsStep":
    global _heads_struct_checked
    if not _heads_struct_checked:
        n = _lib.load().mmbert_heads_step_struct_size()
        if n != ctypes.sizeof(_HeadsStep):
            raise RuntimeError(f"mmbert_heads_step: the library's struct has {n} bytes, the binding's {ctypes.sizeof(_HeadsStep)}")
        _heads_struct_checked = True
    return _HeadsStep()


def heads_step_sync(device) -> torch.Tensor:
    key = (device, _stream())
    t = _heads_sync.get(key)
    if t is None:
        t = _heads_sync[key] = torch.zeros(4, device=device, dtype=torch.int32)
    return t


def heads_step_workspace(B: int, H: int, device) -> torch.Tensor:
    return torch.empty(_lib.load().mmbert_heads_step_workspace(int(B), int(H)) // 4, device=device, dtype=torch.float32)


def heads_step_fwd(a: "_HeadsStep", lo: int = 1, hi: int = 7):
    _lib.check(_lib.load().mmbert_heads_step_fwd_levels(_stream(), ctypes.addressof(a), lo, hi), "mmbert_heads_step_fwd_levels")


def heads_predict(a: "_HeadsStep"):
    _lib.check(_lib.load().mmbert_heads_predict(_stream(), ctypes.addressof(a)), "mmbert_heads_predict")


def heads_step_outputs(ws: torch.Tensor, B: int, H: int):
    po, fo = ctypes.c_size_t(0), ctypes.c_size_t(0)
# ... 147 lines not shown
```

Baseline: 1231 samples/s.

## Fuse row compaction, gather and query-limit; compute CE forward on labelled rows only

Adds a row-list cross-entropy forward that processes only the labelled rows from the prologue's row index. It computes the per-segment inverse counts in-kernel and reduces the loss deterministically in a second small kernel, in place of a count kernel plus a full-M row pass. It also adds a fused kernel that compacts the row indices, gathers the saved activations for the sparse top-layer backward and computes the attention query limit in one launch instead of three. Both paths are gated by a new fused_seam flag, on by default. The gains are fewer launches and less logits traffic, at the cost of added complexity and shape assumptions such as the ce_rows size checks.

```diff
diff --git a/include/mmbert_hip.h b/include/mmbert_hip.h
--- a/include/mmbert_hip.h
+++ b/include/mmbert_hip.h
@@ -100,6 +100,9 @@
                   const int* seg_bounds, int nseg, float* inv_count, float* loss_sum, float* row_lse,
                   int logits_f32 ,
                   float* row_loss );
+int mmbert_ce_fwd_rows(mmbert_stream_t stream, const void* logits, int ldv, int V, const int64_t* labels, int M,
+                       const int* seg_bounds, int nseg, const int* rows, const int* count, const int* seg_cnt, int per,
+                       float* inv_count, float* loss_sum, float* row_lse, int logits_f32, float* pair_loss);
 int mmbert_ce_bwd(mmbert_stream_t stream, const void* logits, int ldv, int V, const int64_t* labels, int M,
                   const int* seg_bounds, int nseg, const float* inv_count, const float* gscale, const float* row_lse, void* dlogits, int ldd,
                   const int* rows , int nrows,
@@ -240,6 +243,10 @@
                              const long long* dst_pitch, const int* row_bytes, const int64_t* inv_stamp, unsigned stamp, int nlist, int nrows);
 int mmbert_gather_rows(mmbert_stream_t stream, int nseg, const void* const* src, void* const* dst, const long long* src_pitch, const long long* dst_pitch,
                        const int* row_bytes, const int* idx, int nrows);
+int mmbert_compact_gather_rows(mmbert_stream_t stream, const int* rows32, const int64_t* rows64, int n, const int64_t* extra, int nextra,
+                               const int64_t* map, int64_t* out64, int* out32, int64_t* inv_stamp, unsigned stamp,
+                               int nseg, const void* const* src, void* const* dst, const long long* src_pitch, const long long* dst_pitch,
+                               const int* row_bytes, const int* seq_start, int nseq, int* q_limit);
 int mmbert_transpose_bf16(mmbert_stream_t stream, const void* src, void* dst, const void* descs, int ndesc, int total_tiles);
 
 #ifdef __cplusplus
diff --git a/msa_amd/_lib.py b/msa_amd/_lib.py
--- a/msa_amd/_lib.py
+++ b/msa_amd/_lib.py
@@ -45,6 +45,7 @@
     "mmbert_attn_q_limit": (I, [P, P, I, P, I, P]),
     "mmbert_attn_dropout_mask": (I, [P, P, I, C.c_uint, I, U32, U32]),
     "mmbert_ce_fwd": (I, [P, P, I, I, P, I, P, I, P, P, P, I, P]),
+    "mmbert_ce_fwd_rows": (I, [P, P, I, I, P, I, P, I, P, P, P, I, P, P, P, I, P]),
     "mmbert_ce_bwd": (I, [P, P, I, I, P, I, P, I, P, P, P, P, I, P, I, I]),
     "mmbert_vocab_topk": (I, [P, P, I, I, I, I, I, P, P, P, P, P, P]),
     "mmbert_active_rows": (I, [P, P, I, I, P, P]),
@@ -90,6 +91,7 @@
     "mmbert_gather_rows": (I, [P, I, P, P, P, P, P, P, I]),
     "mmbert_compact_rows": (I, [P, P, P, I, P, I, P, P, P]),
     "mmbert_compact_rows_inv": (I, [P, P, P, I, P, I, P, P, P, P, C.c_uint]),
+    "mmbert_compact_gather_rows": (I, [P, P, P, I, P, I, P, P, P, P, C.c_uint, I, P, P, P, P, P, P, I, P]),
     "mmbert_scatter_rows_zero": (I, [P, I, P, P, P, P, P, P, C.c_uint, I, I]),
     "mmbert_pack_i64": (I, [P, I, P, P, P, P, P]),
     "mmbert_rows_to_block": (I, [P, P, P, I, I, I, I, P, I, I, P]),
diff --git a/msa_amd/csrc/attention.hip b/msa_amd/csrc/attention.hip
--- a/msa_amd/csrc/attention.hip
+++ b/msa_amd/csrc/attention.hip
@@ -905,20 +905,7 @@
 }
 __global__ __launch_bounds__(256) void attn_q_limit_wg_kernel(const int* __restrict__ rows, int n, const int* __restrict__ seq_start, int nseq,
                                                               int* __restrict__ out) {
-    __shared__ int lim[1024], st[1024];
-    for (int s = threadIdx.x; s < nseq; s += 256) { lim[s] = 0; st[s] = seq_start[s]; }
-    __syncthreads();
-    for (int i = threadIdx.x; i < n; i += 256) {
-        const int r = rows[i];
-        int lo = 0, hi = nseq - 1;
-        while (lo < hi) {
-            const int mid = (lo + hi + 1) >> 1;
-            if (st[mid] <= r) lo = mid; else hi = mid - 1;
-        }
-        atomicMax(&lim[lo], r - st[lo] + 1);
-    }
-    __syncthreads();
-    for (int s = threadIdx.x; s < nseq; s += 256) out[s] = lim[s];
+    mmb_q_limit_wg([&](int i) { return rows[i]; }, n, seq_start, nseq, out);
 }
 
 extern "C" {
diff --git a/msa_amd/csrc/common.h b/msa_amd/csrc/common.h
--- a/msa_amd/csrc/common.h
+++ b/msa_amd/csrc/common.h
@@ -183,3 +183,21 @@
     d0 = (mmb_f2){x0.x > 0.0f ? o0.x : g0.x, x0.y > 0.0f ? o0.y : g0.y};
     d1 = (mmb_f2){x1.x > 0.0f ? o1.x : g1.x, x1.y > 0.0f ? o1.y : g1.y};
 }
+
+template <typename RowOf>
+__device__ __forceinline__ void mmb_q_limit_wg(RowOf row_of, int n, const int* __restrict__ seq_start, int nseq, int* __restrict__ out) {
+    __shared__ int lim[1024], st[1024];
+    for (int s = threadIdx.x; s < nseq; s += 256) { lim[s] = 0; st[s] = seq_start[s]; }
+    __syncthreads();
+    for (int i = threadIdx.x; i < n; i += 256) {
+        const int r = row_of(i);
+        int lo = 0, hi = nseq - 1;
+        while (lo < hi) {
+            const int mid = (lo + hi + 1) >> 1;
+            if (st[mid] <= r) lo = mid; else hi = mid - 1;
+        }
+        atomicMax(&lim[lo], r - st[lo] + 1);
+    }
+    __syncthreads();
+    for (int s = threadIdx.x; s < nseq; s += 256) out[s] = lim[s];
+}
diff --git a/msa_amd/csrc/rowwise.hip b/msa_amd/csrc/rowwise.hip
--- a/msa_amd/csrc/rowwise.hip
+++ b/msa_amd/csrc/rowwise.hip
@@ -917,6 +917,8 @@
     if (tid == 0) *count = base;
 }
 
+__device__ __forceinline__ float ce_inv_count(int cnt) { return 1.0f / (float)max(cnt, 1); }
+
 __global__ void ce_count_kernel(const int64_t* __restrict__ labels, int M, int V, const int* __restrict__ seg_bounds, int nseg,
                                 float* __restrict__ inv_count, float* __restrict__ loss_sum) {
     __shared__ int cnt[4];
@@ -941,7 +943,7 @@
     for (int q = 0; q < 4; ++q) if (c[q]) atomicAdd(&cnt[q], c[q]);
     __syncthreads();
     if (threadIdx.x < nseg) {
-        inv_count[threadIdx.x] = 1.0f / (float)max(cnt[threadIdx.x], 1);
+        inv_count[threadIdx.x] = ce_inv_count(cnt[threadIdx.x]);
         loss_sum[threadIdx.x] = 0.f;
     }
 }
@@ -975,6 +977,42 @@
         __syncthreads();
     }
     if ((int)threadIdx.x < nseg) loss_sum[threadIdx.x] = red[threadIdx.x][0];
+}
+
+__global__ __launch_bounds__(1024) void ce_loss_sum_rows_kernel(const int* __restrict__ rows, const int* __restrict__ count, int M,
+                                                                const float* __restrict__ pair_loss, const int* __restrict__ seg_bounds, int nseg,
+                                                                float* __restrict__ loss_sum) {
+    __shared__ float red[4][1024];
+    __shared__ int span[2];
+    const int tid = threadIdx.x;
+    const int n = min(*count, M);
+    const int b1 = nseg > 1 ? seg_bounds[1] : 0x7fffffff, b2 = nseg > 2 ? seg_bounds[2] : 0x7fffffff, b3 = nseg > 3 ? seg_bounds[3] : 0x7fffffff;
+#pragma unroll
+    for (int q = 0; q < 4; ++q) red[q][tid] = 0.f;
+    for (int j0 = 0; j0 < n; j0 += 1024) {
+        const int j = j0 + tid, last = min(j0 + 1023, n - 1);
+        const bool in = j < n;
+        const int r = in ? min(max(rows[j], 0), M - 1) : 0;
+        const float x = in ? pair_loss[j] : 0.f;
+        if (tid == 0) span[0] = r >> 10;
+        if (j == last) span[1] = r >> 10;
+        __syncthreads();
+        const int k0 = span[0], k1 = span[1];
+        const int sg = (r >= b1 ? 1 : 0) + (r >= b2 ? 1 : 0) + (r >= b3 ? 1 : 0);
+        for (int k = k0; k <= k1; ++k) {
+            if (in && (r >> 10) == k) red[sg][r & 1023] += x;
+            __syncthreads();
+        }
+    }
+    __syncthreads();
+    for (int w = 512; w > 0; w >>= 1) {
+        if (tid < w) {
+#pragma unroll
+            for (int q = 0; q < 4; ++q) red[q][tid] += red[q][tid + w];
+        }
+        __syncthreads();
+    }
+    if (tid < nseg) loss_sum[tid] = red[tid][0];
 }
 
 #define RUNS_MAXN 8192
@@ -1055,6 +1093,64 @@
 }
 
 #define CE_MAXC 16
+#define CE_ROWS_GRID 1024
+template <bool F32>
+__device__ __forceinline__ void ce_row_load(const void* __restrict__ logits_, int ldv, int i, int tid, int nchunk, bf16x8 (&v)[CE_MAXC]) {
+    if constexpr (F32) {
+        const float* row = (const float*)logits_ + (size_t)i * ldv;
+#pragma unroll
+        for (int c = 0; c < CE_MAXC; ++c) {
+            const int ch = c * 256 + tid;
+            if (ch < nchunk) {
+                const float4 lo = *(const float4*)(row + ch * 8), hi = *(const float4*)(row + ch * 8 + 4);
+                v[c] = (bf16x8){f2bf(lo.x), f2bf(lo.y), f2bf(lo.z), f2bf(lo.w), f2bf(hi.x), f2bf(hi.y), f2bf(hi.z), f2bf(hi.w)};
+            }
+        }
+    } else {
+        const bf16_t* row = (const bf16_t*)logits_ + (size_t)i * ldv;
+#pragma unroll
+        for (int c = 0; c < CE_MAXC; ++c) {
+            const int ch = c * 256 + tid;
+            if (ch < nchunk) v[c] = *(const bf16x8*)(row + ch * 8);
+        }
+    }
+}
+
+__device__ __forceinline__ float ce_row_lse(const bf16x8 (&v)[CE_MAXC], int nchunk, int V, int64_t lab, int tid, float* red, float* lab_logit) {
+    const int lane = tid & 63, w = tid >> 6;
+    float mx = -INFINITY;
+#pragma unroll
+    for (int c = 0; c < CE_MAXC; ++c) {
+        const int ch = c * 256 + tid;
+        if (ch < nchunk) {
+#pragma unroll
+            for (int r = 0; r < 8; ++r) if (ch * 8 + r < V) mx = fmaxf(mx, bf2f(v[c][r]));
+        }
+    }
+    mx = wave_max(mx);
+    if (lane == 0) red[w] = mx;
+    __syncthreads();
+    mx = fmaxf(fmaxf(red[0], red[1]), fmaxf(red[2], red[3]));
+    __syncthreads();
+    float se = 0.f;
+#pragma unroll
+    for (int c = 0; c < CE_MAXC; ++c) {
+        const int ch = c * 256 + tid;
+        if (ch < nchunk) {
+#pragma unroll
+            for (int r = 0; r < 8; ++r) if (ch * 8 + r < V) se += __expf(bf2f(v[c][r]) - mx);
+            if ((int)(lab >> 3) == ch) {
+#pragma unroll
+                for (int r = 0; r < 8; ++r) if ((int)(lab & 7) == r) *lab_logit = bf2f(v[c][r]);
+            }
+        }
+    }
+    se = wave_sum(se);
+    if (lane == 0) red[w] = se;
+    __syncthreads();
+    return mx + __logf(red[0] + red[1] + red[2] + red[3]);
+}
+
 template <int MODE, bool F32>
 __global__ __launch_bounds__(256) void ce_row_kernel(const void* __restrict__ logits_, int ldv, int V, const int64_t* __restrict__ labels,
                                                      const int* __restrict__ seg_bounds, int nseg, const float* __restrict__ inv_count,
@@ -1064,7 +1160,7 @@
     __shared__ float lab_logit;
     const int i = rows ? rows[blockIdx.x] : blockIdx.x;
     const int64_t lab = labels[i];
-    const int tid = threadIdx.x, lane = tid & 63, w = tid >> 6;
+    const int tid = threadIdx.x;
     const int nchunk = ldv >> 3;
     if (lab < 0 || lab >= V) {
         if (MODE == 0) { if (tid == 0) { row_lse[i] = 0.f; if (row_loss) row_loss[i] = 0.f; } }
@@ -1078,54 +1174,10 @@
     int s = 0;
     while (s + 1 < nseg && i >= seg_bounds[s + 1]) ++s;
     bf16x8 v[CE_MAXC];
-    if constexpr (F32) {
-        const float* row = (const float*)logits_ + (size_t)i * ldv;
-#pragma unroll
-        for (int c = 0; c < CE_MAXC; ++c) {
-            const int ch = c * 256 + tid;
-            if (ch < nchunk) {
-                const float4 lo = *(const float4*)(row + ch * 8), hi = *(const float4*)(row + ch * 8 + 4);
-                v[c] = (bf16x8){f2bf(lo.x), f2bf(lo.y), f2bf(lo.z), f2bf(lo.w), f2bf(hi.x), f2bf(hi.y), f2bf(hi.z), f2bf(hi.w)};
-            }
-        }
-    } else {
-        const bf16_t* row = (const bf16_t*)logits_ + (size_t)i * ldv;
-#pragma unroll
-        for (int c = 0; c < CE_MAXC; ++c) {
-            const int ch = c * 256 + tid;
-            if (ch < nchunk) v[c] = *(const bf16x8*)(row + ch * 8);
-        }
-    }
+    ce_row_load<F32>(logits_, ldv, i, tid, nchunk, v);
     if (MODE == 0) {
-        float mx = -INFINITY;
-#pragma unroll
-        for (int c = 0; c < CE_MAXC; ++c) {
-            const int ch = c * 256 + tid;
-            if (ch < nchunk) {
-#pragma unroll
-                for (int r = 0; r < 8; ++r) if (ch * 8 + r < V) mx = fmaxf(mx, bf2f(v[c][r]));
-            }
-        }
-        mx = wave_max(mx);
-        if (lane == 0) red[w] = mx;
-        __syncthreads();
-        mx = fmaxf(fmaxf(red[0], red[1]), fmaxf(red[2], red[3]));
-        __syncthreads();
-        float se = 0.f;
-#pragma unroll
-        for (int c = 0; c < CE_MAXC; ++c) {
-            const int ch = c * 256 + tid;
-            if (ch < nchunk) {
-#pragma unroll
-                for (int r = 0; r < 8; ++r) if (ch * 8 + r < V) se += __expf(bf2f(v[c][r]) - mx);
-                if ((int)(lab >> 3) == ch) lab_logit = bf2f(v[c][lab & 7]);
-            }
-        }
-        se = wave_sum(se);
-        if (lane == 0) red[w] = se;
-        __syncthreads();
+        const float lse = ce_row_lse(v, nchunk, V, lab, tid, red, &lab_logit);
         if (tid == 0) {
-            const float lse = mx + __logf(red[0] + red[1] + red[2] + red[3]);
             row_lse[i] = lse;
             if (row_loss) row_loss[i] = (lse - lab_logit) * inv_count[s];
             else atomicAdd(loss_sum + s, (lse - lab_logit) * inv_count[s]);
@@ -1149,6 +1201,43 @@
                 *(bf16x8*)(drow + ch * 8) = o;
             }
         }
+    }
+}
+
+template <bool F32>
+__global__ __launch_bounds__(256) void ce_rows_fwd_kernel(const void* __restrict__ logits_, int ldv, int V, const int64_t* __restrict__ labels, int M,
+                                                          const int* __restrict__ seg_bounds, int nseg, const int* __restrict__ rows,
+                                                          const int* __restrict__ count, const int* __restrict__ seg_cnt, int per,
+                                                          float* __restrict__ inv_count, float* __restrict__ row_lse, float* __restrict__ pair_loss) {
+    __shared__ float red[4];
+    __shared__ float lab_logit;
+    __shared__ int cnt[4];
+    const int tid = threadIdx.x;
+    const int nchunk = ldv >> 3;
+    const int n = min(*count, M);
+    if (blockIdx.x != 0 && (int)blockIdx.x >= n) return;
+    if (tid < 4) cnt[tid] = 0;
+    __syncthreads();
+    for (int e = tid; e < nseg * per; e += 256) { const int c = seg_cnt[e]; if (c) atomicAdd(&cnt[e / per], c); }
+    __syncthreads();
+    if (blockIdx.x == 0 && tid < nseg) inv_count[tid] = ce_inv_count(cnt[tid]);
+    for (int j = blockIdx.x; j < n; j += gridDim.x) {
+        const int i = rows[j];
+        const int64_t lab = (i >= 0 && i < M) ? labels[i] : -1;
+        if (lab < 0 || lab >= V) {
+            if (tid == 0) pair_loss[j] = 0.f;
+            continue;
+        }
+        int s = 0;
+        while (s + 1 < nseg && i >= seg_bounds[s + 1]) ++s;
+        bf16x8 v[CE_MAXC];
+        ce_row_load<F32>(logits_, ldv, i, tid, nchunk, v);
+        const float lse = ce_row_lse(v, nchunk, V, lab, tid, red, &lab_logit);
+        if (tid == 0) {
+            row_lse[i] = lse;
+            pair_loss[j] = (lse - lab_logit) * ce_inv_count(cnt[s]);
+        }
+        __syncthreads();
     }
 }
 
@@ -2108,6 +2197,25 @@
     return 0;
 }
 
+int mmbert_ce_fwd_rows(hipStream_t stream, const void* logits, int ldv, int V, const int64_t* labels, int M,
+                       const int* seg_bounds, int nseg, const int* rows, const int* count, const int* seg_cnt, int per,
+                       float* inv_count, float* loss_sum, float* row_lse, int logits_f32, float* pair_loss) {
+    if (M <= 0) return 0;
+    if (nseg < 1 || nseg > 4 || (ldv & 7) || ldv > CE_MAXC * 256 * 8 || V > ldv || per < 1) return -1;
+    if (!rows || !count || !seg_cnt || !pair_loss) return -1;
+    const int grid = M < CE_ROWS_GRID ? M : CE_ROWS_GRID;
+    if (logits_f32)
+        hipLaunchKernelGGL(ce_rows_fwd_kernel<true>, dim3(grid), dim3(256), 0, stream, logits, ldv, V, labels, M, seg_bounds, nseg, rows, count,
+                           seg_cnt, per, inv_count, row_lse, pair_loss);
+    else
+        hipLaunchKernelGGL(ce_rows_fwd_kernel<false>, dim3(grid), dim3(256), 0, stream, logits, ldv, V, labels, M, seg_bounds, nseg, rows, count,
+                           seg_cnt, per, inv_count, row_lse, pair_loss);
+    MMB_CHECK_LAUNCH();
+    hipLaunchKernelGGL(ce_loss_sum_rows_kernel, dim3(1), dim3(1024), 0, stream, rows, count, M, (const float*)pair_loss, seg_bounds, nseg, loss_sum);
+    MMB_CHECK_LAUNCH();
+    return 0;
+}
+
 int mmbert_vocab_topk(hipStream_t stream, const void* logits, int ldv, int V, int M, int logits_f32, int k, const int64_t* labels,
                       int32_t* top_ids, float* top_logprob, float* row_lse, float* label_logprob, int32_t* label_rank) {
     if (M < 0 || V < 1 || V > CE_MAXC * 256 * 8 || k < 1 || k > 8 || k > V || (ldv & 7) || ldv < V) return -1;
@@ -2418,6 +2526,60 @@
     return 0;
 }
 
+__global__ __launch_bounds__(256) void compact_gather_rows_kernel(const GatherArgs a, const int* __restrict__ a32, const int64_t* __restrict__ a64, int n,
+                                                                  const int64_t* __restrict__ extra, int nextra, const int64_t* __restrict__ map,
+                                                                  int64_t* __restrict__ out64, int* __restrict__ out32,
+                                                                  long long* __restrict__ inv_stamp, long long stamp_hi,
+                                                                  const int* __restrict__ seq_start, int nseq, int* __restrict__ q_limit) {
+    auto row_of = [&](int i) {
+        int64_t r = i < n ? (a32 ? (int64_t)a32[i] : a64[i]) : extra[i - n];
+        if (map) r = map[r];
+        return r;
+    };
+    const int i = blockIdx.x;
+    if (i == n + nextra) {
+        if (blockIdx.y == 0) mmb_q_limit_wg([&](int j) { return (int)row_of(j); }, n + nextra, seq_start, nseq, q_limit);
+        return;
+    }
+    const int64_t r = row_of(i);
+    if (blockIdx.y == 0 && threadIdx.x == 0) {
+        out64[i] = r;
+        out32[i] = (int)r;
+        if (inv_stamp) inv_stamp[r] = stamp_hi | (long long)i;
+    }
+    const GatherSeg s = a.s[blockIdx.y];
+    const char* src = s.src + r * s.src_pitch;
+    char* dst = s.dst + (long long)i * s.dst_pitch;
+    if (s.vec16) {
+        for (int b = threadIdx.x * 16; b < s.row_bytes; b += 256 * 16) *(uint4*)(dst + b) = *(const uint4*)(src + b);
+    } else {
+        for (int b = threadIdx.x * 4; b < s.row_bytes; b += 256 * 4) *(uint32_t*)(dst + b) = *(const uint32_t*)(src + b);
+    }
+}
+
+int mmbert_compact_gather_rows(hipStream_t stream, const int* rows32, const int64_t* rows64, int n, const int64_t* extra, int nextra, const int64_t* map,
+                               int64_t* out64, int* out32, int64_t* inv_stamp, unsigned stamp,
+                               int nseg, const void* const* src, void* const* dst, const long long* src_pitch, const long long* dst_pitch,
+                               const int* row_bytes, const int* seq_start, int nseq, int* q_limit) {
+    if (n < 0 || nextra < 0 || (n > 0 && !rows32 && !rows64) || (nextra > 0 && !extra) || !out64 || !out32) return -1;
+    if (nseg < 1 || nseg > 12 || (inv_stamp && stamp == 0u)) return -1;
+    if (q_limit && (!seq_start || nseq < 1 || nseq > 1024)) return -1;
+    const int nlist = n + nextra;
+    if (nlist == 0 && !q_limit) return 0;
+    GatherArgs a = {};
+    for (int k = 0; k < nseg; ++k) {
+        if (!src[k] || !dst[k] || row_bytes[k] <= 0 || (row_bytes[k] & 3) || (src_pitch[k] & 3) || (dst_pitch[k] & 3) ||
+            ((uintptr_t)src[k] & 3) || ((uintptr_t)dst[k] & 3)) return -1;
+        a.s[k].src = (const char*)src[k]; a.s[k].dst = (char*)dst[k]; a.s[k].src_pitch = src_pitch[k]; a.s[k].dst_pitch = dst_pitch[k];
+        a.s[k].row_bytes = row_bytes[k];
+        a.s[k].vec16 = !((row_bytes[k] | src_pitch[k] | dst_pitch[k]) & 15) && !(((uintptr_t)src[k] | (uintptr_t)dst[k]) & 15);
+    }
+    hipLaunchKernelGGL(compact_gather_rows_kernel, dim3(nlist + (q_limit ? 1 : 0), nseg), dim3(256), 0, stream, a, rows32, rows64, n, extra, nextra, map,
+                       out64, out32, (long long*)inv_stamp, (long long)((unsigned long long)stamp << 32), seq_start, nseq, q_limit);
+    MMB_CHECK_LAUNCH();
+    return 0;
+}
+
 int mmbert_rows_to_block(hipStream_t stream, const int64_t* ids, const void* rows, int rows_bf16, int ldr, int n, int H,
                          const int64_t* uni, int U, int V, float* block) {
     if (n <= 0 || U <= 0) return 0;
diff --git a/msa_amd/model.py b/msa_amd/model.py
--- a/msa_amd/model.py
+++ b/msa_amd/model.py
@@ -429,7 +429,11 @@
                     rinv = top.__dict__.get("_row_inverse")
                     if rinv is None or rinv.table.numel() < M_all or rinv.table.device != rows_f.device:
                         rinv = top.__dict__["_row_inverse"] = ops.RowInverse(M_all, rows_f.device)
-                    R, R32 = ops.compact_rows(rows_l, rows_f, layout.inv if getattr(layout, "split", False) else None, inverse=rinv)
+                    rmap = layout.inv if getattr(layout, "split", False) else None
+                    if _seam(top, "D") and layout.seq_len.numel() <= 1024:
+                        R = (rows_l, rows_f, rmap)
+                    else:
+                        R, R32 = ops.compact_rows(rows_l, rows_f, rmap, inverse=rinv)
                 elif top_rows is not None:
                     Ro = _EncoderFn._sparse_rows(top_rows, None, ra)
                     if Ro is not None:
@@ -541,9 +545,15 @@
     def _last_layer_sparse(top, lw, layout, key_bias, kv_len, saved_i, dy_c, R, H, ra, R32=None, lnd=None, rinv=None, deferred=None):
         cfg = top.config
         x, qkv, actx, lse, z1, m1, r1, y1, u, g, z2, m2, r2, d_att, d_h1, d_h2 = saved_i
-        if R32 is None:
-            R32 = R.int()
-        m2_c, r2_c, u_c, m1_c, r1_c, y1_c, g_c, actx_c = ops.gather_rows([m2, r2, u, m1, r1, y1, g, actx], R32)
+        want_qlim = getattr(top, "top_layer_query_limit", True)
+        qlim = None
+        if isinstance(R, tuple):
+            R, R32, (m2_c, r2_c, u_c, m1_c, r1_c, y1_c, g_c, actx_c), qlim = ops.compact_gather_rows(
+                R[0], R[1], R[2], rinv, [m2, r2, u, m1, r1, y1, g, actx], layout if want_qlim else None)
+        else:
+            if R32 is None:
+                R32 = R.int()
+            m2_c, r2_c, u_c, m1_c, r1_c, y1_c, g_c, actx_c = ops.gather_rows([m2, r2, u, m1, r1, y1, g, actx], R32)
         dy = dy_c
         dz2d_c = torch.empty_like(dy_c) if d_h2[1] else None
         dz2_c = ops.ln_bwd(dy_c, z2, m2_c, r2_c, lw["ln2_g"], lw["g_ln2_g"], lw["g_ln2_b"], x_rows=R32, dx2=dz2d_c, pre_drop=d_h2,
@@ -563,7 +573,8 @@
         else:
             dctx = torch.zeros((ra, H), device=dy.device, dtype=torch.bfloat16)
             dctx.index_copy_(0, R, dctx_c)
-        qlim = ops.attn_q_limit(R32, layout) if getattr(top, "top_layer_query_limit", True) else None
+        if qlim is None and want_qlim:
+            qlim = ops.attn_q_limit(R32, layout)
         dqkv = ops.attn_bwd(qkv, actx, dctx, lse, key_bias, layout, H, drop=d_att, kv_len=kv_len, q_limit=qlim)
         if rinv is None:
             dz1 = torch.zeros((ra, H), device=dy.device, dtype=torch.bfloat16)
@@ -601,7 +612,7 @@
 
 class _Trunk:
     __slots__ = ("ids", "tts", "B", "T", "lens", "pair_info", "feats", "feat_versions", "plan", "layout", "split", "key_bias", "kv_len", "seed", "top_rows",
-                 "d_emb", "d_joint", "infer", "late_split", "compact", "J_pre", "predict", "attention", "dense")
+                 "d_emb", "d_joint", "infer", "late_split", "compact", "J_pre", "predict", "attention", "dense", "ce_rows")
 
 
 class _TrunkFn(torch.autograd.Function):
@@ -779,6 +790,11 @@
         return None, None, None
 
 
+def _seam(top, item):
+    v = getattr(top, "fused_seam", True)
+    return (item in v) if isinstance(v, str) else bool(v)
+
+
 def mlm_active_rows(labels, vocab, first=None):
     idx, cnt = ops.active_rows(labels, vocab)
     dup = (labels.index_select(0, first) != -100).sum().to(torch.int32).view(1) if first is not None else torch.zeros_like(cnt)
@@ -880,7 +896,10 @@
         f32_scores = want_scores and getattr(top, "scores_dtype", torch.bfloat16) == torch.float32
         logits = ops.gemm_nt(t, w["word_h"], bias=w["pred_bias"], out_f32=f32_scores)
         nseg = len(seg_bounds_host) - 1
-        loss, inv, lse = ops.ce_fwd(logits, V, labels, seg_bounds, nseg)
+        ce_rows = trunk.ce_rows if (trunk is not None and rows is not None and _seam(top, "A")) else None
+        if ce_rows is not None and (ce_rows[2].numel() != nseg * ce_rows[3] or ce_rows[0].numel() < M):
+            ce_rows = None
+        loss, inv, lse = ops.ce_fwd(logits, V, labels, seg_bounds, nseg, rows=ce_rows)
         ctx.top, ctx.nseg, ctx.keep_logits, ctx.M = top, nseg, want_scores, M
         ctx.set_materialize_grads(False)
         ctx.rows = None
@@ -1238,6 +1257,7 @@
         if not predict:
             self._last_valid_dev = pro.valid
         rows = (pro.idx, host[nseq:], ev) if want_rows else None
+        ce_rows = (pro.idx, pro.words[nseq:nseq + 1], pro.seq_cnt[:nseq], B) if (want_rows and labels is not None) else None
         kv_len = pro.kv_len if getattr(self, "skip_masked_keys", True) else None
         infer = (predict or ((not self.training) and (not torch.is_grad_enabled()))) and getattr(self, "dedupe_masked_rows", True)
         if not predict:
@@ -1292,6 +1312,7 @@
         t.key_bias, t.kv_len, t.seed, t.infer = key_bias, kv_len, seed, infer
         t.d_emb = ops.make_drop(p_emb, seed, 1000)
         t.d_joint = [ops.make_drop(p_joint, seed, 1001 + k) for k in range(len(lens))]
+        t.ce_rows = ce_rows
         t.top_rows = (rows, plan["first"]) if (rows is not None and getattr(self, "sparse_top_layer_backward", True)) else None
         drop = (not infer) and labels is not None and not getattr(self, "return_scores", True)
         rank = pro.rank
@@ -1741,6 +1762,7 @@
         self.wgrad_side_stream = True
         self.heads_side_stream = True
         self.pairs_side_stream = True
+        self.fused_seam = True
         _hf_init(self, config.initializer_range, skip=_bert)
         self.cls.predictions.decoder.weight = self.bert.embeddings.word_embeddings.weight
 
diff --git a/msa_amd/ops.py b/msa_amd/ops.py
--- a/msa_amd/ops.py
+++ b/msa_amd/ops.py
@@ -633,7 +633,7 @@
 
 
 class Prologue:
-    __slots__ = ("key_bias", "kv_len", "valid", "idx", "words", "nseq", "rank")
+    __slots__ = ("key_bias", "kv_len", "valid", "idx", "words", "nseq", "rank", "seq_cnt")
 
 
 def prologue_sizes(pass_lens, B, rowset=False):
@@ -665,7 +665,7 @@
     if rowset:
         out.rank, bias_perm = ints_all[nints:], fl[bias_len:]
     out.kv_len, out.valid = ints[:nseq], ints[nseq:2 * nseq]
-    seq_cnt = ints[2 * nseq:5 * nseq]
+    seq_cnt = out.seq_cnt = ints[2 * nseq:5 * nseq]
     out.idx = ints[5 * nseq:5 * nseq + max(tokens, 1)]
     out.words = ints[5 * nseq + max(tokens, 1):]
     PA, LA, IA = ctypes.c_void_p * max(n, 1), ctypes.c_longlong * max(n, 1), ctypes.c_int * max(n, 1)
@@ -791,16 +791,25 @@
     return out
 
 
-def ce_fwd(logits, V, labels, seg_bounds, nseg):
+def ce_fwd(logits, V, labels, seg_bounds, nseg, rows=None):
     lib = _lib.load()
     M = logits.shape[0]
     inv = torch.empty(4, device=logits.device, dtype=torch.float32)
     loss = torch.empty(nseg, device=logits.device, dtype=torch.float32)
     lse = torch.empty(M, device=logits.device, dtype=torch.float32)
     assert logits.dtype in (torch.bfloat16, torch.float32)
+    f32 = 1 if logits.dtype == torch.float32 else 0
+    if rows is not None and M > 0:
+        lst, count, seg_cnt, per = rows
+        assert lst.dtype == count.dtype == seg_cnt.dtype == torch.int32 and lst.numel() >= M and seg_cnt.numel() >= nseg * per
+        assert lst.is_contiguous() and seg_cnt.is_contiguous()
+        _lib.check(lib.mmbert_ce_fwd_rows(_stream(), logits.data_ptr(), logits.stride(0), V, labels.data_ptr(), M, seg_bounds.data_ptr(), nseg,
+                                          lst.data_ptr(), count.data_ptr(), seg_cnt.data_ptr(), int(per), inv.data_ptr(), loss.data_ptr(),
+                                          lse.data_ptr(), f32, _ws_f32(M, logits.device).data_ptr()), "mmbert_ce_fwd_rows")
+        return loss, inv, lse
     row_loss = _ws_f32(M, logits.device) if deterministic() else None
     _lib.check(lib.mmbert_ce_fwd(_stream(), logits.data_ptr(), logits.stride(0), V, labels.data_ptr(), M, seg_bounds.data_ptr(), nseg,
-                                 inv.data_ptr(), loss.data_ptr(), lse.data_ptr(), 1 if logits.dtype == torch.float32 else 0, _ptr(row_loss)),
+                                 inv.data_ptr(), loss.data_ptr(), lse.data_ptr(), f32, _ptr(row_loss)),
                "mmbert_ce_fwd")
     return loss, inv, lse
 
@@ -1039,6 +1048,33 @@
                                               LA(*[t.stride(0) * t.element_size() for t in srcs]), LA(*[b for b in rb]),
                                               _IntArr[n](*rb), idx32.data_ptr(), rows), "mmbert_gather_rows")
     return outs
+
+
+def compact_gather_rows(rows, extra, row_map, inverse: "RowInverse", srcs, q_limit_layout=None):
+    n, ne, k = rows.numel(), extra.numel(), len(srcs)
+    dev = extra.device
+    out64 = torch.empty(n + ne, device=dev, dtype=torch.int64)
+    out32 = torch.empty(n + ne, device=dev, dtype=torch.int32)
+    assert rows.dtype in (torch.int32, torch.int64) and extra.dtype == torch.int64 and rows.is_contiguous() and extra.is_contiguous()
+    assert row_map is None or (row_map.dtype == torch.int64 and row_map.is_contiguous())
+    assert 0 < k <= 12
+    for t in srcs:
+        assert t.dim() in (1, 2) and (t.dim() == 1 or t.stride(1) == 1)
+    outs = [torch.empty((n + ne,) + tuple(t.shape[1:]), device=t.device, dtype=t.dtype) for t in srcs]
+    qlim, ns, seq_start = None, 0, None
+    if q_limit_layout is not None:
+        seq_start = q_limit_layout.seq_start
+        ns = q_limit_layout.seq_len.numel()
+        qlim = torch.empty(ns, device=dev, dtype=torch.int32)
+    r32, r64 = (rows.data_ptr(), None) if rows.dtype == torch.int32 else (None, rows.data_ptr())
+    LA = ctypes.c_longlong * k
+    rb = [(t.shape[1] if t.dim() == 2 else 1) * t.element_size() for t in srcs]
+    _lib.check(_lib.load().mmbert_compact_gather_rows(
+        _stream(), r32, r64, n, extra.data_ptr(), ne, _ptr(row_map), out64.data_ptr(), out32.data_ptr(),
+        None if inverse is None else inverse.table.data_ptr(), 0 if inverse is None else inverse.next(n + ne),
+        k, _PtrArr[k](*[t.data_ptr() for t in srcs]), _PtrArr[k](*[o.data_ptr() for o in outs]),
+        LA(*[t.stride(0) * t.element_size() for t in srcs]), LA(*rb), _IntArr[k](*rb), _ptr(seq_start), ns, _ptr(qlim)), "mmbert_compact_gather_rows")
+    return out64, out32, outs, qlim
 
 
 def pack_i64(segments, total=None):
```

New measurement: 1230 samples/s, median of 2. About the same (-0.0%).
